# 1812598631/Amos-slam

Hardware: AMD Instinct MI355X
Metric: front-end frames/sec (ORB extract+match+mask) at 640x480 (higher is better)
Workload: dtype u8 (ORB, gate, matcher) + fp32 (mask network); 1 GPU; configs[2]: 640x480 L8 N1000 full front-end: YOLACT-R50 fp32 mask + ORB detect + gate + describe + match; lanes_per_gpu=2, frames_per_launch=64, width=640, height=480, n_features=1000, n_levels=8, ini_th_fast=20, min_th_fast=7, match=frame k vs k-1, N x N best-2, synthetic_stream_seed=stream = rank, frame k seeded 1000*rank+k (amos-slam_amd/synth.py), parallelism=frames sharded 1 ways, one process per GPU, no data-path collective

## Files before the change

### amos-slam_amd/__init__.py

```python
import ctypes as C
import os

import numpy as np

_HERE = os.path.dirname(os.path.abspath(__file__))
LIB_PATH = os.environ.get("AMOS_FRONTEND_LIB", os.path.join(_HERE, "csrc", "libamos_frontend.so"))

KP_DTYPE = np.dtype([("x", "<f4"), ("y", "<f4"), ("size", "<f4"), ("angle", "<f4"),
                     ("response", "<f4"), ("octave", "<i4"), ("class_id", "<i4")])
BEST2_DTYPE = np.dtype([("best_idx", "<i4"), ("best_dist", "<i4"), ("second_idx", "<i4"),
                        ("second_dist", "<i4")])

TH_HIGH, TH_LOW, HISTO_LENGTH = 100, 50, 30

_v, _i, _z, _f, _d, _q, _u = C.c_void_p, C.c_int, C.c_size_t, C.c_float, C.c_double, C.c_longlong, C.c_uint32
PROTOTYPES = {
    "amos_last_error": (C.c_char_p, ()),
    "amos_device_count": (_i, ()),
    "amos_current_device": (_i, ()),
    "amos_build_variant": (C.c_char_p, ()),
    "amos_orb_create": (_i, (_v, _i, _i, _i, _i, _v, _v)),
    "amos_orb_destroy": (None, (_v,)),
    "amos_orb_geometry_probe": (_i, (_v, _i, _i, _i, _i, _v, _v)),
    "amos_orb_tables": (_i, (_v, _v, _v, _v, _v, _v, _v)),
    "amos_orb_tables_host": (_i, (_v, _v, _v, _v, _v, _v, _v)),
    "amos_orb_level_sizes": (_i, (_v, _i, _i, _v, _v)),
    "amos_orb_detect": (_i, (_v, _v, _z, _i, _i)),
    "amos_orb_level_count": (_i, (_v, _i, _i)),
    "amos_orb_level_keypoints": (_i, (_v, _i, _i, _v, _i)),
    "amos_orb_set_level_keypoints": (_i, (_v, _i, _i, _v, _i)),
    "amos_orb_level_layout": (_i, (_v, _v, _v, _v)),
    "amos_orb_fetch_levels": (_i, (_v, _i, _v, _v, _i)),
    "amos_orb_store_levels": (_i, (_v, _i, _v, _v, _i)),
    "amos_orb_gate": (_i, (_v, _v, _z, _v, _z, _v, _i, _v, _i, _v, _i, _v)),
    "amos_orb_closed_mask": (_i, (_v, _v, _z)),
    "amos_orb_describe": (_i, (_v, _v, _v, _i, _v)),
    "amos_orb_extract": (_i, (_v, _v, _z, _i, _i, _v, _v, _i, _v)),
    "amos_orb_level_image": (_i, (_v, _i, _i, _v, _z, _i)),
    "amos_orb_pyramid_images": (_i, (_v, _i, _v, _v, _i)),
    "amos_orb_blurred_image": (_i, (_v, _i, _i, _v, _z)),
    "amos_orb_level_candidates": (_i, (_v, _i, _i, _v, _i)),
    "amos_orb_extract_batch_device": (_i, (_v, _v, _z, _z, _i, _i, _i)),
    "amos_orb_detect_batch_device": (_i, (_v, _v, _z, _z, _i, _i, _i)),
    "amos_orb_gate_batch_device": (_i, (_v, _v, _z, _z)),
    "amos_orb_gate_labels_batch_device": (_i, (_v, _v, _z, _z, _v, _z, _z, _v, _z, _i, _v, _z, _i, _v)),
    "amos_orb_describe_batch_device": (_i, (_v,)),
    "amos_orb_extract_batch_device_color": (_i, (_v, _v, _z, _z, _i, _i, _i, _i, _i)),
    "amos_frame_rgbd_glue_batch_device": (_i, (_v, _v, _i, _f, _z, _z, _f, _f, _f, _f, _f, _v, _v, _v, _v)),
    "amos_frame_stereo_match": (_i, (_v, _v, _f, _f, _v, _v, _i)),
    "amos_frame_stereo_match_batch_device": (_i, (_v, _v, _i, _f, _f, _v, _v, _v, _v)),
    "amos_frame_stereo_match_arrays_device": (_i, (_v, _v, _i, _v, _v, _v, _i, _v, _v, _v, _i, _f, _f, _v, _v, _v, _v)),
    "amos_frame_undistort_batch_device": (_i, (_v, _f, _f, _f, _f, _v, _i, _v)),
    "amos_frame_image_bounds": (_i, (_i, _i, _f, _f, _f, _f, _v, _i, _v)),
    "amos_orb_batch_results_device": (_i, (_v, _v, _v, _v, _v)),
    "amos_orb_batch_fetch": (_i, (_v, _i, _v, _v, _i, _v)),
    "amos_orb_sync": (_i, (_v,)),
    "amos_orb_timing_enable": (_i, (_v, _i)),
    "amos_orb_timing_collect": (_i, (_v, _v, _v)),
    "amos_orb_stream": (_v, (_v,)),
    "amos_match_create": (_i, (_i, _v, _v)),
    "amos_match_destroy": (None, (_v,)),
    "amos_match_sync": (_i, (_v,)),
    "amos_match_stream": (_v, (_v,)),
    "amos_match_distances": (_i, (_v, _v, _i, _v, _i, _v)),
    "amos_match_list_distances": (_i, (_v, _v, _i, _v, _i, _v, _v, _v)),
    "amos_match_list_best2": (_i, (_v, _v, _i, _v, _i, _v, _v, _i, _v)),
    "amos_match_bruteforce_best2": (_i, (_v, _v, _i, _v, _i, _i, _v)),
    "amos_match_set_bruteforce_kernel": (_i, (_v, _i)),
    "amos_match_bruteforce_best2_batch_device": (_i, (_v, _v, _z, _v, _v, _v, _i, _i, _i, _v)),
    "amos_frame_grid_build_batch_device": (_i, (_v, _v, _v, _i, _i, _v, _v)),
    "amos_match_window_best2_batch_device": (_i, (_v, _v, _v)),
    "amos_match_local_points_batch_device": (_i, (_v, _v)),
    "amos_match_local_points": (_i, (_v, _v, _v, _v, _i, _v, _i, _v, _v, _v, _i, _f, _f, _f, _f, _v, _v, _v, _v)),
    "amos_match_motion_model_batch_device": (_i, (_v, _v)),
    "amos_match_motion_model": (_i, (_v, _v, _v, _v, _i, _v, _i, _v, _v, _i, _f, _f, _f, _f, _v, _v, _v, _v)),
    "amos_bow_create": (_i, (_i, _v, _i, _i, _i, _i, _i, _v, _v, _v, _v, _v)),
    "amos_bow_destroy": (None, (_v,)),
    "amos_bow_sync": (_i, (_v,)),
    "amos_bow_stream": (_v, (_v,)),
    "amos_bow_check": (_i, (_i, _i, _i, _i, _i, _v, _v, _v)),
    "amos_bow_transform_batch_device": (_i, (_v, _v, _v, _i, _i, _i, _v, _v, _v, _v, _v, _v, _v, _v, _v, _v)),
    "amos_bow_transform": (_i, (_v, _v, _i, _i, _v, _v, _v, _v, _v, _v, _v, _v)),
    "amos_match_bow_batch_device": (_i, (_v, _v)),
    "amos_match_bow": (_i, (_v, _v, _v, _f, _i, _v, _v)),
    "amos_match_bow_kf_batch_device": (_i, (_v, _v, _f, _i)),
    "amos_match_triangulation_batch_device": (_i, (_v, _v, _v, _v, _v, _i, _i, _i)),
    "amos_match_bow_kf": (_i, (_v, _v, _v, _f, _i, _v, _v)),
    "amos_match_triangulation": (_i, (_v, _v, _v, _i, _v, _v, _v, _i, _i, _i, _v, _v)),
    "amos_mask_pre_create": (_i, (_i, _v, _i, _i, _i, _v)),
    "amos_mask_pre_destroy": (None, (_v,)),
    "amos_mask_pre_stream": (_v, (_v,)),
    "amos_mask_preprocess_batch_device": (_i, (_v, _v, _i, _v)),
    "amos_orb_detect_color_with_mask_pre_batch_device": (_i, (_v, _v, _v, _z, _z, _i, _i, _i, _i, _i, _v)),
    "amos_mask_bias_act_device": (_i, (_v, _v, _v, _v, _z, _i, _i)),
    "amos_mask_bias_relu_maxpool_device": (_i, (_v, _v, _v, _v, _i, _i, _i, _i)),
    "amos_mask_stem_weight_floats": (_i, ()),
    "amos_mask_stem_weights_device": (_i, (_v, _v, _q, _q, _q, _q, _v)),
    "amos_mask_stem_device": (_i, (_v, _v, _q, _q, _q, _q, _v, _v, _v, _i, _i, _i)),
    "amos_mask_conv_supported": (_i, (_i, _i, _i, _i, _i, _i)),
    "amos_mask_conv_device": (_i, (_v, _v, _v, _v, _v, _v, _i, _i, _i, _i, _i, _i, _i, _i, _i, _i)),
    "amos_mask_conv_workspace_bytes": (_z, (_i, _i, _i, _i, _i, _i, _i, _i, _i)),
    "amos_mask_conv_ws_device": (_i, (_v, _v, _v, _v, _v, _v, _i, _i, _i, _i, _i, _i, _i, _i, _i, _i, _v, _z)),
    "amos_mask_conv_tile_mode": (_i, (_i,)),
    "amos_mask_conv_kernel_name": (_i, (_i, _i, _i, _i, _i, _i, _i, _i, _i, _v, _i)),
    "amos_mask_conv_chain_supported": (_i, (_i, _i, _i, _i, _i, _i, _i)),
    "amos_mask_conv_chain_device": (_i, (_v, _v, _v, _v, _v, _v, _v, _v, _i, _i, _i, _i, _i, _i, _i)),
    "amos_mask_conv1x1_supported": (_i, (_i, _i, _i)),
    "amos_mask_winograd_supported": (_i, (_i, _i)),
    "amos_mask_winograd_weight_floats": (_z, (_i, _i)),
    "amos_mask_winograd_weights_device": (_i, (_v, _v, _v, _i, _i)),
    "amos_mask_winograd_conv_device": (_i, (_v, _v, _v, _v, _v, _v, _i, _i, _i, _i, _i, _i)),
    "amos_mask_winograd24_weight_floats": (_z, (_i, _i)),
    "amos_mask_winograd24_weights_device": (_i, (_v, _v, _v, _i, _i)),
    "amos_mask_winograd24_conv_device": (_i, (_v, _v, _v, _v, _v, _v, _i, _i, _i, _i, _i, _i)),
    "amos_mask_winograd24_conv_layout_device": (_i, (_v, _v, _v, _v, _v, _v, _i, _i, _i, _i, _i, _i, _i, _i)),
    "amos_mask_winograd24_persistent_mode": (_i, (_i,)),
    "amos_mask_winograd24_narrow_mode": (_i, (_i,)),
    "amos_mask_conv1x1_device": (_i, (_v, _v, _v, _v, _v, _v, _i, _i, _i, _i, _i, _i, _i)),
    "amos_mask_bilinear_nhwc_device": (_i, (_v, _v, _v, _i, _i, _i, _i, _i, _i, _f, _f)),
    "amos_mask_bilinear_nhwc_act_device": (_i, (_v, _v, _v, _i, _i, _i, _i, _i, _i, _f, _f, _i)),
    "amos_mask_bilinear_x2_mode": (_i, (_i,)),
    "amos_mask_nms_column_max_device": (_i, (_v, _v, _v, _i, _i)),
    "amos_mask_class_scores_device": (_i, (_v, _v, _v, _i, _i, _i, _f)),
    "amos_mask_person_mask_device": (_i, (_v, _v, _v, _v, _i, _i, _i, _i, _i, _i)),
    "amos_mask_head_outputs_device": (_i, (_v, _v, _v, _v, _v, _v, _i, _i, _i, _i, _i, _i, _i, _i)),
    "amos_mask_head_outputs_scores_device": (_i, (_v, _v, _v, _v, _v, _v, _v, _f, _i, _i, _i, _i, _i, _i, _i, _i)),
    "amos_mask_topk_rows_device": (_i, (_v, _v, _v, _v, _i, _i, _i)),
    "amos_mask_topk_rows_sparse_device": (_i, (_v, _v, _v, _v, _i, _i, _i, _f)),
    "amos_mask_post_workspace_bytes": (_z, (_i, _i, _i, _i, _i, _i)),
    "amos_mask_person_masks_device": (_i, (_v, _v, _v, _v, _v, _v, _i, _i, _i, _i, _i, _i, _i, _i, _v, _z, _v, _v)),
    "amos_mask_person_masks_scores_device": (_i, (_v, _v, _v, _v, _v, _v, _i, _i, _i, _i, _i, _i, _i, _i, _v, _z, _v, _v)),
    "amos_mask_coef_at_priors_device": (_i, (_v, _v, _v, _v, _v, _v, _i, _i, _v, _v, _v, _i, _i, _i, _i, _v)),
    "amos_mask_person_masks_at_priors_device": (_i, (_v, _v, _v, _v, _v, _v, _v, _v, _i, _i, _i, _v, _v, _v, _v, _i, _i, _i, _i, _i, _i, _i, _i, _v, _z, _v, _v)),
    "amos_mask_person_masks_scores_at_priors_device": (_i, (_v, _v, _v, _v, _v, _v, _v, _v, _i, _i, _i, _v, _v, _v, _v, _i, _i, _i, _i, _i, _i, _i, _i, _v, _z, _v, _v)),
    "amos_slic_center_count": (_i, (_i, _i, _i, _v, _v)),
    "amos_slic_create": (_i, (_i, _v, _i, _i, _i, _v)),
    "amos_slic_destroy": (None, (_v,)),
    "amos_slic_stream": (_v, (_v,)),
    "amos_slic_run": (_i, (_v, _v, _v, _i, _i, _i, _i, _i, _v, _v, _v)),
    "amos_slic_batch_device": (_i, (_v, _v, _v, _i, _i, _i, _i, _i, _i, _v, _v)),
    "amos_cluster_bgr2lab_batch_device": (_i, (_v, _v, _z, _i, _v)),
    "amos_cluster_kmeans_batch_device": (_i, (_v, _v, _i, _i, _i, _u, _i, _v)),
    "amos_cluster_kmeans": (_i, (_v, _v, _i, _i, _u, _i, _v)),
    "amos_flow_check_device": (_i, (_v, _v, _z, _v, _z, _i, _i, _v, _v, _v, _i, _v)),
    "amos_flow_epipolar_device": (_i, (_v, _v, _v, _v, _v, _i, _v)),
    "amos_flow_scene_flow_device": (_i, (_v, _v, _z, _v, _z, _v, _v, _i, _v, _v)),
    "amos_flow_fundamental_score_device": (_i, (_v, _v, _i, _v, _v, _i, _d, _v, _v, _v)),
    "amos_flow_pnp_score_device": (_i, (_v, _v, _i, _v, _v, _i, _d, _d, _d, _d, _d, _v, _v, _v)),
    "amos_lk_create": (_i, (_i, _v, _i, _i, _i, _i, _v)),
    "amos_lk_destroy": (None, (_v,)),
    "amos_lk_stream": (_v, (_v,)),
    "amos_lk_levels": (_i, (_v,)),
    "amos_lk_track_device": (_i, (_v, _v, _z, _v, _z, _v, _i, _i, _d, _f, _v, _v, _v)),
    "amos_corners_create": (_i, (_i, _v, _i, _i, _v)),
    "amos_corners_destroy": (None, (_v,)),
    "amos_corners_stream": (_v, (_v,)),
    "amos_corners_good_features_device": (_i, (_v, _v, _z, _i, _i, _i, _d, _d, _d, _v, _i, _v, _v)),
    "amos_corners_candidate_count": (_i, (_v, _v)),
    "amos_corners_subpix_device": (_i, (_v, _v, _z, _i, _i, _v, _v, _i, _i, _i, _d)),
    "amos_fmat_create": (_i, (_i, _v, _i, _i, _v)),
    "amos_fmat_destroy": (None, (_v,)),
    "amos_fmat_stream": (_v, (_v,)),
    "amos_fmat_ransac_device": (_i, (_v, _i, _v, _v, _v, _v, _v, _d, _d, _i, _v, _v, _v)),
    "amos_fmat_scene_flow_pair_device": (_i, (_v, _v, _v, _v, _v, _v, _v, _v, _v)),
    "amos_fmat_ransac": (_i, (_v, _i, _v, _v, _d, _d, _i, _v, _v, _v)),
    "amos_pnp_create": (_i, (_i, _v, _i, _i, _v)),
    "amos_pnp_destroy": (None, (_v,)),
    "amos_pnp_stream": (_v, (_v,)),
    "amos_pnp_ransac_device": (_i, (_v, _i, _v, _v, _v, _v, _v, _d, _d, _d, _d, _d, _d, _i, _v, _v, _v)),
    "amos_pnp_scene_flow_device": (_i, (_v, _v, _v, _v, _v, _v, _z, _v, _z, _i, _i, _v, _d, _d, _v, _v, _v)),
    "amos_pnp_ransac": (_i, (_v, _i, _v, _v, _d, _d, _d, _d, _d, _d, _i, _v, _v, _v)),
    "amos_dyna_create": (_i, (_i, _v, _i, _i, _v)),
    "amos_dyna_destroy": (None, (_v,)),
    "amos_dyna_stream": (_v, (_v,)),
    "amos_dyna_results_device": (_i, (_v, _v)),
    "amos_dyna_copy_to_host": (_i, (_v, _v, _v, _z)),
    "amos_dyna_tail_device": (_i, (_v, _i, _v, _v, _v, _v, _v, _v, _v, _v, _v, _z, _v, _z, _i, _i, _v, _d, _d, _v)),
    "amos_dyna_reset_frame_device": (_i, (_v, _i)),
    "amos_dyna_decide_batch_device": (_i, (_v, _i, _v, _z, _z, _i, _i, _v, _z, _i, _i, _v, _z)),
    "amos_dyna_scene_flow_obj_device": (_i, (_v, _i, _v, _v, _v, _v, _v, _z, _v, _z, _i, _i, _v, _z, _v, _z, _v, _d, _d, _v)),
}
EXPORTS = list(PROTOTYPES)


class AmosError(RuntimeError):
    pass


class OrbParams(C.Structure):
    _fields_ = [("n_features", C.c_int32), ("scale_factor", C.c_float), ("n_levels", C.c_int32),
                ("ini_th_fast", C.c_int32), ("min_th_fast", C.c_int32)]


_lib = None


def lib():
    global _lib
    if _lib is None:
        if not os.path.exists(LIB_PATH):
            raise AmosError(f"{LIB_PATH} is missing: build it with `make -C amos-slam_amd/csrc` "
                            "(or __graft_entry__.build()); there is no CPU fallback")
        try:
            import torch
        except ImportError:
            pass
        L = C.CDLL(LIB_PATH)

        def declare(name):
            f = getattr(L, name)
            f.restype, f.argtypes = PROTOTYPES[name]

        declare("amos_build_variant")
        variant = L.amos_build_variant().decode()
        if variant != "default" and os.environ.get("AMOS_ALLOW_EXPERIMENT_BUILD") != "1":
            raise AmosError(f"{LIB_PATH} is an experiment build ({variant}): its results are wrong; unset AMOS_FRONTEND_LIB "
                            "or set AMOS_ALLOW_EXPERIMENT_BUILD=1 for a timing run")
        for name in PROTOTYPES:
            declare(name)
        _lib = L
    return _lib


def _check(rc, what):
    if rc < 0:
        raise AmosError(f"{what} failed (rc={rc}): {lib().amos_last_error().decode()}")
    return rc


def _p(a):
    return a.ctypes.data_as(C.c_void_p) if a is not None else None


def geometry_probe(max_width, max_height, width, height, n_features=1000, scale_factor=1.2, n_levels=8, ini_th=20, min_th=7):
    params = OrbParams(n_features, scale_factor, n_levels, ini_th, min_th)
    need, cap = np.zeros(6, np.int32), np.zeros(6, np.int32)
    rc = lib().amos_orb_geometry_probe(C.byref(params), max_width, max_height, width, height, _p(need), _p(cap))
    return rc, need, cap


def device_count():
    return _check(lib().amos_device_count(), "amos_device_count")


class _Handle:
    _kind = None

    def _open(self, *args):
        self.L = lib()
        h = C.c_void_p()
        _check(getattr(self.L, f"amos_{self._kind}_create")(*args, C.byref(h)), f"amos_{self._kind}_create")
        self.h = h

    def close(self):
        if getattr(self, "h", None):
            getattr(self.L, f"amos_{self._kind}_destroy")(self.h)
            self.h = None

    __del__ = close

    @property
    def stream(self):
        return getattr(self.L, f"amos_{self._kind}_stream")(self.h)


class OrbExtractor(_Handle):

    _kind = "orb"

    def __init__(self, n_features=1000, scale_factor=1.2, n_levels=8, ini_th=20, min_th=7,
                 max_width=640, max_height=480, max_batch=1, device=0, stream=None):
        self.params = OrbParams(n_features, scale_factor, n_levels, ini_th, min_th)
        self.n_levels, self.n_features = n_levels, n_features
        self.max_batch = max_batch
        self._open(C.byref(self.params), max_width, max_height, max_batch, device, stream)
        self.shape = None
        cap = C.c_int(0)
        self.L.amos_orb_batch_results_device(self.h, None, None, None, C.byref(cap))
        self.capacity = cap.value

    def tables(self):
        n = self.n_levels
        sc, isc, s2, is2 = (np.zeros(n, np.float32) for _ in range(4))
        fpl, umax = np.zeros(n, np.int32), np.zeros(16, np.int32)
        _check(self.L.amos_orb_tables(self.h, _p(sc), _p(isc), _p(s2), _p(is2), _p(fpl), _p(umax)), "amos_orb_tables")
        return dict(scale=sc, inv_scale=isc, sigma2=s2, inv_sigma2=is2, features_per_level=fpl, umax=umax)

# ... 278 lines not shown
    return int(lib().amos_mask_bilinear_x2_mode(mode))


def mask_conv1x1_supported(cin, cout, stride):
    return lib().amos_mask_conv1x1_supported(cin, cout, stride) == 0


def mask_conv1x1(stream_ptr, x_ptr, w_ptr, bias_ptr, residual_ptr, y_ptr, batch, in_h, in_w, cin, cout, stride, relu):
    _check(lib().amos_mask_conv1x1_device(stream_ptr, x_ptr, w_ptr, bias_ptr, residual_ptr, y_ptr, batch, in_h, in_w, cin, cout, stride, int(relu)),
           "amos_mask_conv1x1_device")


def mask_conv_supported(cin, cout, kh, kw, stride, pad):
    return lib().amos_mask_conv_supported(cin, cout, kh, kw, stride, pad) == 0


def mask_winograd_supported(cin, cout):
    return lib().amos_mask_winograd_supported(cin, cout) == 0


def mask_winograd_weights(stream_ptr, w_ptr, u_ptr, cin, cout):
    _check(lib().amos_mask_winograd_weights_device(stream_ptr, w_ptr, u_ptr, cin, cout), "amos_mask_winograd_weights_device")


def mask_winograd_conv(stream_ptr, x_ptr, u_ptr, bias_ptr, residual_ptr, y_ptr, batch, h, w, cin, cout, relu):
    _check(lib().amos_mask_winograd_conv_device(stream_ptr, x_ptr, u_ptr, bias_ptr, residual_ptr, y_ptr, batch, h, w, cin, cout, int(relu)),
           "amos_mask_winograd_conv_device")


def mask_winograd24_weights(stream_ptr, w_ptr, u_ptr, cin, cout):
    _check(lib().amos_mask_winograd24_weights_device(stream_ptr, w_ptr, u_ptr, cin, cout), "amos_mask_winograd24_weights_device")


def mask_winograd24_conv(stream_ptr, x_ptr, u_ptr, bias_ptr, residual_ptr, y_ptr, batch, h, w, cin, cout, relu):
    _check(lib().amos_mask_winograd24_conv_device(stream_ptr, x_ptr, u_ptr, bias_ptr, residual_ptr, y_ptr, batch, h, w, cin, cout, int(relu)),
           "amos_mask_winograd24_conv_device")


def mask_winograd24_conv_layout(stream_ptr, x_ptr, u_ptr, bias_ptr, residual_ptr, y_ptr, batch, h, w, cin, cout, relu, in_blocked, out_blocked):
    _check(lib().amos_mask_winograd24_conv_layout_device(stream_ptr, x_ptr, u_ptr, bias_ptr, residual_ptr, y_ptr, batch, h, w, cin, cout, int(relu), int(in_blocked),
                                                         int(out_blocked)), "amos_mask_winograd24_conv_layout_device")


def mask_winograd24_persistent_mode(mode=-2):
    return int(lib().amos_mask_winograd24_persistent_mode(mode))


def mask_winograd24_narrow_mode(mode=-2):
    return int(lib().amos_mask_winograd24_narrow_mode(mode))


def mask_conv_tile_mode(mode=-2):
    return int(lib().amos_mask_conv_tile_mode(mode))


def mask_conv_kernel_name(batch, in_h, in_w, cin, cout, kh, kw, stride, pad):
    buf = C.create_string_buffer(96)
    _check(lib().amos_mask_conv_kernel_name(batch, in_h, in_w, cin, cout, kh, kw, stride, pad, buf, 96), "amos_mask_conv_kernel_name")
    return buf.value.decode()


def mask_conv(stream_ptr, x_ptr, w_ptr, bias_ptr, residual_ptr, y_ptr, batch, in_h, in_w, cin, cout, kh, kw, stride, pad, relu):
    _check(lib().amos_mask_conv_device(stream_ptr, x_ptr, w_ptr, bias_ptr, residual_ptr, y_ptr, batch, in_h, in_w, cin, cout, kh, kw, stride, pad, int(relu)),
           "amos_mask_conv_device")


def mask_conv_chain_supported(batch, in_h, in_w, cin, planes, cout, stride):
    return lib().amos_mask_conv_chain_supported(batch, in_h, in_w, cin, planes, cout, stride) == 0


def mask_conv_chain(stream_ptr, x_ptr, wd_ptr, bd_ptr, yc_ptr, w3_ptr, b3_ptr, y_ptr, batch, in_h, in_w, cin, planes, cout, stride):
    _check(lib().amos_mask_conv_chain_device(stream_ptr, x_ptr, wd_ptr, bd_ptr, yc_ptr, w3_ptr, b3_ptr, y_ptr, batch, in_h, in_w, cin, planes, cout, stride),
           "amos_mask_conv_chain_device")


def mask_conv_workspace_bytes(batch, in_h, in_w, cin, cout, kh, kw, stride, pad):
    return int(lib().amos_mask_conv_workspace_bytes(batch, in_h, in_w, cin, cout, kh, kw, stride, pad))


def mask_conv_ws(stream_ptr, x_ptr, w_ptr, bias_ptr, residual_ptr, y_ptr, batch, in_h, in_w, cin, cout, kh, kw, stride, pad, relu, workspace_ptr, workspace_bytes):
    _check(lib().amos_mask_conv_ws_device(stream_ptr, x_ptr, w_ptr, bias_ptr, residual_ptr, y_ptr, batch, in_h, in_w, cin, cout, kh, kw, stride, pad, int(relu),
                                          workspace_ptr, workspace_bytes), "amos_mask_conv_ws_device")


def mask_bilinear_nhwc(stream_ptr, x_ptr, y_ptr, n, in_h, in_w, out_h, out_w, channels, scale_h, scale_w, relu=False):
    _check(lib().amos_mask_bilinear_nhwc_act_device(stream_ptr, x_ptr, y_ptr, n, in_h, in_w, out_h, out_w, channels, scale_h, scale_w, int(relu)),
           "amos_mask_bilinear_nhwc_act_device")


def mask_class_scores(stream_ptr, conf_ptr, scores_ptr, batch, n_priors, n_classes_with_background, threshold):
    _check(lib().amos_mask_class_scores_device(stream_ptr, conf_ptr, scores_ptr, batch, n_priors, n_classes_with_background, threshold),
           "amos_mask_class_scores_device")


def mask_person_mask(stream_ptr, masks_ptr, flags_ptr, out_ptr, batch, n_det, mask_h, mask_w, out_h, out_w):
    _check(lib().amos_mask_person_mask_device(stream_ptr, masks_ptr, flags_ptr, out_ptr, batch, n_det, mask_h, mask_w, out_h, out_w), "amos_mask_person_mask_device")


def mask_head_outputs(stream_ptr, raw_ptr, bias_ptr, loc_ptr, conf_ptr, coef_ptr, batch, cells, channels_padded, anchors, n_classes_with_background, mask_dim,
                      n_priors_total, prior_offset):
    _check(lib().amos_mask_head_outputs_device(stream_ptr, raw_ptr, bias_ptr, loc_ptr, conf_ptr, coef_ptr, batch, cells, channels_padded, anchors,
                                               n_classes_with_background, mask_dim, n_priors_total, prior_offset), "amos_mask_head_outputs_device")


def mask_head_outputs_scores(stream_ptr, raw_ptr, bias_ptr, loc_ptr, conf_ptr, coef_ptr, scores_ptr, threshold, batch, cells, channels_padded, anchors,
                             n_classes_with_background, mask_dim, n_priors_total, prior_offset):
    _check(lib().amos_mask_head_outputs_scores_device(stream_ptr, raw_ptr, bias_ptr, loc_ptr, conf_ptr, coef_ptr, scores_ptr, threshold, batch, cells,
                                                      channels_padded, anchors, n_classes_with_background, mask_dim, n_priors_total, prior_offset),
           "amos_mask_head_outputs_scores_device")


def mask_person_masks_scores(stream_ptr, loc_ptr, scores_ptr, coef_ptr, priors_ptr, proto_ptr, batch, n_priors, n_classes_with_background, mask_dim, proto_h, proto_w,
                             out_h, out_w, workspace_ptr, workspace_bytes, masks_ptr, found_ptr):
    _check(lib().amos_mask_person_masks_scores_device(stream_ptr, loc_ptr, scores_ptr, coef_ptr, priors_ptr, proto_ptr, batch, n_priors, n_classes_with_background,
                                                      mask_dim, proto_h, proto_w, out_h, out_w, workspace_ptr, workspace_bytes, masks_ptr, found_ptr),
           "amos_mask_person_masks_scores_device")


def mask_topk_rows(stream_ptr, x_ptr, values_ptr, indices_ptr, rows, n, k):
    _check(lib().amos_mask_topk_rows_device(stream_ptr, x_ptr, values_ptr, indices_ptr, rows, n, k), "amos_mask_topk_rows_device")


def mask_topk_rows_sparse(stream_ptr, x_ptr, values_ptr, indices_ptr, rows, n, k, fill):
    _check(lib().amos_mask_topk_rows_sparse_device(stream_ptr, x_ptr, values_ptr, indices_ptr, rows, n, k, fill), "amos_mask_topk_rows_sparse_device")


def mask_post_workspace_bytes(batch, n_priors, n_classes_with_background, mask_dim, proto_h, proto_w):
    return int(lib().amos_mask_post_workspace_bytes(batch, n_priors, n_classes_with_background, mask_dim, proto_h, proto_w))


def mask_person_masks(stream_ptr, loc_ptr, conf_ptr, coef_ptr, priors_ptr, proto_ptr, batch, n_priors, n_classes_with_background, mask_dim, proto_h, proto_w,
                      out_h, out_w, workspace_ptr, workspace_bytes, masks_ptr, found_ptr):
    _check(lib().amos_mask_person_masks_device(stream_ptr, loc_ptr, conf_ptr, coef_ptr, priors_ptr, proto_ptr, batch, n_priors, n_classes_with_background, mask_dim,
                                               proto_h, proto_w, out_h, out_w, workspace_ptr, workspace_bytes, masks_ptr, found_ptr),
           "amos_mask_person_masks_device")


def _coef_levels(level_ptrs, level_hw, level_blocked, anchors):
    n = len(level_ptrs)
    offs, off = [], 0
    for h, w in level_hw:
        offs.append(off)
        off += h * w * anchors
    ints = C.c_int * n
    return ((C.c_void_p * n)(*level_ptrs), ints(*[h for h, _ in level_hw]), ints(*[w for _, w in level_hw]), ints(*[int(bool(f)) for f in level_blocked]),
            ints(*offs), n)


def mask_coef_at_priors(stream_ptr, level_ptrs, level_hw, level_blocked, cin, weight_ptr, bias_ptr, prior_idx_ptr, batch, n_slots, anchors, mask_dim, out_ptr):
    _check(lib().amos_mask_coef_at_priors_device(stream_ptr, *_coef_levels(level_ptrs, level_hw, level_blocked, anchors), cin, weight_ptr, bias_ptr, prior_idx_ptr,
                                                 batch, n_slots, anchors, mask_dim, out_ptr), "amos_mask_coef_at_priors_device")


def mask_person_masks_at_priors(stream_ptr, loc_ptr, scores_ptr, scores_are_class_scores, level_ptrs, level_hw, level_blocked, cin, anchors, mask_weight_ptr,
                                mask_bias_ptr, priors_ptr, proto_ptr, batch, n_priors, n_classes_with_background, mask_dim, proto_h, proto_w, out_h, out_w,
                                workspace_ptr, workspace_bytes, masks_ptr, found_ptr):
    name = "amos_mask_person_masks_scores_at_priors_device" if scores_are_class_scores else "amos_mask_person_masks_at_priors_device"
    _check(getattr(lib(), name)(stream_ptr, loc_ptr, scores_ptr, *_coef_levels(level_ptrs, level_hw, level_blocked, anchors), cin, anchors, mask_weight_ptr,
                                mask_bias_ptr, priors_ptr, proto_ptr, batch, n_priors, n_classes_with_background, mask_dim, proto_h, proto_w, out_h, out_w,
                                workspace_ptr, workspace_bytes, masks_ptr, found_ptr), name)


def mask_nms_column_max(stream_ptr, boxes_ptr, out_ptr, n_lists, k):
    _check(lib().amos_mask_nms_column_max_device(stream_ptr, boxes_ptr, out_ptr, n_lists, k), "amos_mask_nms_column_max_device")


class LkTracker(_Handle):

    _kind = "lk"

    def __init__(self, width=640, height=480, win_size=22, max_level=5, device=0, stream=None):
        self._open(device, stream, width, height, win_size, max_level)
        self.levels = self.L.amos_lk_levels(self.h)

    def track_device(self, d_prev, prev_stride, d_next, next_stride, d_prev_xy, n, d_next_xy, d_status, d_err=None, max_count=20, epsilon=0.01,
                     min_eig=1e-4):
        _check(self.L.amos_lk_track_device(self.h, d_prev, prev_stride, d_next, next_stride, d_prev_xy, n, max_count, epsilon, min_eig, d_next_xy, d_status,
                                           d_err), "amos_lk_track_device")


def image_bounds(width, height, fx, fy, cx, cy, dist_coef):
    dc = np.ascontiguousarray(dist_coef, np.float32)
    out = np.zeros(4, np.float32)
    _check(lib().amos_frame_image_bounds(width, height, fx, fy, cx, cy, _p(dc), len(dc), _p(out)), "amos_frame_image_bounds")
    return tuple(float(v) for v in out)


class WindowSearch(C.Structure):
    _fields_ = [("d_kps", C.c_void_p), ("d_desc", C.c_void_p), ("d_counts", C.c_void_p), ("d_cell_start", C.c_void_p),
                ("d_items", C.c_void_p), ("d_query_uv", C.c_void_p), ("d_query_invz", C.c_void_p), ("d_u_right", C.c_void_p),
                ("d_pairs_q", C.c_void_p), ("d_pairs_t", C.c_void_p), ("scale_factors", C.c_void_p), ("n_pairs", C.c_int32),
                ("capacity", C.c_int32), ("n_levels", C.c_int32), ("mode", C.c_int32), ("init_dist", C.c_int32), ("th", C.c_float),
                ("mbf", C.c_float), ("min_x", C.c_float), ("max_x", C.c_float), ("min_y", C.c_float), ("max_y", C.c_float)]


class MapPoint(C.Structure):
    _fields_ = [("pos", C.c_float * 3), ("normal", C.c_float * 3), ("min_distance", C.c_float), ("max_distance", C.c_float),
                ("flags", C.c_int32), ("desc", C.c_uint8 * 32), ("pad", C.c_uint8 * 12)]


class LocalCamera(C.Structure):
    _fields_ = [("Rcw", C.c_float * 9), ("tcw", C.c_float * 3), ("Ow", C.c_float * 3), ("fx", C.c_float), ("fy", C.c_float),
                ("cx", C.c_float), ("cy", C.c_float), ("mbf", C.c_float), ("view_cos_limit", C.c_float), ("th", C.c_float),
                ("nn_ratio", C.c_float)]


class LocalStats(C.Structure):
    _fields_ = [("n_in_view", C.c_int32), ("n_matches", C.c_int32), ("n_researched", C.c_int32), ("status", C.c_int32)]


MAP_POINT_SKIP, MAP_POINT_HAS_OBS = 1, 2
MAP_POINT_DTYPE = np.dtype([("pos", "<f4", (3,)), ("normal", "<f4", (3,)), ("min_distance", "<f4"), ("max_distance", "<f4"),
                            ("flags", "<i4"), ("desc", "u1", (32,)), ("pad", "u1", (12,))])
LOCAL_CAMERA_DTYPE = np.dtype([("Rcw", "<f4", (9,)), ("tcw", "<f4", (3,)), ("Ow", "<f4", (3,)), ("fx", "<f4"), ("fy", "<f4"), ("cx", "<f4"),
                               ("cy", "<f4"), ("mbf", "<f4"), ("view_cos_limit", "<f4"), ("th", "<f4"), ("nn_ratio", "<f4")])
LOCAL_STATS_DTYPE = np.dtype([("n_in_view", "<i4"), ("n_matches", "<i4"), ("n_researched", "<i4"), ("status", "<i4")])
MAP_QUERY_DTYPE = np.dtype([("proj_x", "<f4"), ("proj_y", "<f4"), ("proj_xr", "<f4"), ("view_cos", "<f4"), ("level", "<i4"),
                            ("has_obs", "<i4"), ("desc", "u1", (32,))])
assert (C.sizeof(MapPoint), C.sizeof(LocalCamera), C.sizeof(LocalStats)) == (MAP_POINT_DTYPE.itemsize, LOCAL_CAMERA_DTYPE.itemsize,
                                                                            LOCAL_STATS_DTYPE.itemsize) == (80, 92, 16)


class LocalSearch(C.Structure):
    _fields_ = [("d_kps", C.c_void_p), ("d_desc", C.c_void_p), ("d_counts", C.c_void_p), ("d_cell_start", C.c_void_p), ("d_items", C.c_void_p),
                ("d_u_right", C.c_void_p), ("d_points", C.c_void_p), ("point_off", C.c_void_p), ("cameras", C.c_void_p),
                ("d_occupied", C.c_void_p), ("scale_factors", C.c_void_p), ("d_query", C.c_void_p), ("d_in_view", C.c_void_p),
                ("d_match", C.c_void_p), ("d_stats", C.c_void_p), ("n_frames", C.c_int32), ("capacity", C.c_int32), ("n_levels", C.c_int32),
                ("min_x", C.c_float), ("max_x", C.c_float), ("min_y", C.c_float), ("max_y", C.c_float)]


class LastPoint(C.Structure):
    _fields_ = [("pos", C.c_float * 3), ("angle", C.c_float), ("octave", C.c_int32), ("flags", C.c_int32), ("desc", C.c_uint8 * 32),
                ("pad", C.c_uint8 * 8)]


class MotionCamera(C.Structure):
    _fields_ = [("Rcw", C.c_float * 9), ("tcw", C.c_float * 3), ("Rlw", C.c_float * 9), ("tlw", C.c_float * 3), ("fx", C.c_float),
                ("fy", C.c_float), ("cx", C.c_float), ("cy", C.c_float), ("mbf", C.c_float), ("mb", C.c_float), ("th", C.c_float),
                ("th_retry", C.c_float), ("retry_below", C.c_int32), ("mono", C.c_int32), ("check_orientation", C.c_int32)]


class MotionStats(C.Structure):
    _fields_ = [("n_projected", C.c_int32), ("n_matches", C.c_int32), ("n_first", C.c_int32), ("pass_", C.c_int32),
                ("n_researched", C.c_int32), ("flags", C.c_int32), ("status", C.c_int32), ("pad", C.c_int32)]


LAST_POINT_SKIP, LAST_POINT_HAS_OBS = 1, 2
MOTION_FORWARD, MOTION_BACKWARD = 1, 2
LAST_POINT_DTYPE = np.dtype([("pos", "<f4", (3,)), ("angle", "<f4"), ("octave", "<i4"), ("flags", "<i4"), ("desc", "u1", (32,)),
                             ("pad", "u1", (8,))])
MOTION_CAMERA_DTYPE = np.dtype([("Rcw", "<f4", (9,)), ("tcw", "<f4", (3,)), ("Rlw", "<f4", (9,)), ("tlw", "<f4", (3,)), ("fx", "<f4"),
                                ("fy", "<f4"), ("cx", "<f4"), ("cy", "<f4"), ("mbf", "<f4"), ("mb", "<f4"), ("th", "<f4"),
                                ("th_retry", "<f4"), ("retry_below", "<i4"), ("mono", "<i4"), ("check_orientation", "<i4")])
MOTION_STATS_DTYPE = np.dtype([("n_projected", "<i4"), ("n_matches", "<i4"), ("n_first", "<i4"), ("pass", "<i4"), ("n_researched", "<i4"),
                               ("flags", "<i4"), ("status", "<i4"), ("pad", "<i4")])
PROJ_QUERY_DTYPE = np.dtype([("u", "<f4"), ("v", "<f4"), ("invz", "<f4"), ("octave", "<i4"), ("angle", "<f4"), ("has_obs", "<i4"),
                             ("desc", "u1", (32,))])
assert (C.sizeof(LastPoint), C.sizeof(MotionCamera), C.sizeof(MotionStats)) == (LAST_POINT_DTYPE.itemsize, MOTION_CAMERA_DTYPE.itemsize,
                                                                                MOTION_STATS_DTYPE.itemsize) == (64, 140, 32)


class MotionSearch(C.Structure):
    _fields_ = [("d_kps", C.c_void_p), ("d_desc", C.c_void_p), ("d_counts", C.c_void_p), ("d_cell_start", C.c_void_p), ("d_items", C.c_void_p),
                ("d_u_right", C.c_void_p), ("d_points", C.c_void_p), ("point_off", C.c_void_p), ("cameras", C.c_void_p),
                ("scale_factors", C.c_void_p), ("d_query", C.c_void_p), ("d_projected", C.c_void_p), ("d_match", C.c_void_p),
                ("d_stats", C.c_void_p), ("n_frames", C.c_int32), ("capacity", C.c_int32), ("n_levels", C.c_int32), ("min_x", C.c_float),
                ("max_x", C.c_float), ("min_y", C.c_float), ("max_y", C.c_float)]


BOW_L1_NORM, BOW_TF_IDF = 0, 0
BOW_MAX_CHILDREN, BOW_MAX_CAPACITY, BOW_NO_WORD, BOW_STATUS_EARLY_LEAF = 32, 16384, 0xFFFFFFFF, 1
BOW_STATS_DTYPE = np.dtype([("n_words", "<i4"), ("n_nodes", "<i4"), ("n_stopped", "<i4"), ("status", "<i4")])
BOW_SEARCH_STATS_DTYPE = np.dtype([("n_queries", "<i4"), ("n_matches", "<i4"), ("n_researched", "<i4"), ("status", "<i4")])
assert BOW_STATS_DTYPE.itemsize == BOW_SEARCH_STATS_DTYPE.itemsize == 16


class BowSearch(C.Structure):
    _fields_ = [("d_kps", C.c_void_p), ("d_desc", C.c_void_p), ("d_counts", C.c_void_p), ("d_n_nodes", C.c_void_p), ("d_node_ids", C.c_void_p),
                ("d_node_off", C.c_void_p), ("d_node_idx", C.c_void_p), ("d_has_point", C.c_void_p), ("d_pairs_kf", C.c_void_p),
                ("d_pairs_f", C.c_void_p), ("d_match", C.c_void_p), ("d_stats", C.c_void_p), ("n_pairs", C.c_int32), ("capacity", C.c_int32),
                ("nn_ratio", C.c_float), ("check_orientation", C.c_int32)]


class KfPairSearch(C.Structure):
    _fields_ = [("d_kps", C.c_void_p), ("d_desc", C.c_void_p), ("d_counts", C.c_void_p), ("d_n_nodes", C.c_void_p), ("d_node_ids", C.c_void_p),
                ("d_node_off", C.c_void_p), ("d_node_idx", C.c_void_p), ("d_has_point", C.c_void_p), ("d_u_right", C.c_void_p),
                ("d_pairs_1", C.c_void_p), ("d_pairs_2", C.c_void_p), ("d_match12", C.c_void_p), ("d_stats", C.c_void_p), ("n_pairs", C.c_int32),
                ("capacity", C.c_int32)]


KF_GEOMETRY_DTYPE = np.dtype([("f12", "<f4", (9,)), ("ex", "<f4"), ("ey", "<f4")])
assert KF_GEOMETRY_DTYPE.itemsize == 44
KF_STATUS_BAD_INDEX, KF_STATUS_BAD_OCTAVE = 1, 2


class BowView(C.Structure):
    _fields_ = [("n", C.c_int32), ("keys", C.c_void_p), ("descriptors", C.c_void_p), ("has_point", C.c_void_p), ("u_right", C.c_void_p),
                ("n_nodes", C.c_int32), ("node_ids", C.c_void_p), ("node_off", C.c_void_p), ("node_idx", C.c_void_p)]


def bow_vocabulary_arrays(parent, is_leaf, desc, weight):
    parent = np.ascontiguousarray(parent, np.int32)
    is_leaf = np.ascontiguousarray(is_leaf, np.uint8)
    desc = np.ascontiguousarray(desc, np.uint8).reshape(-1, 32)
    weight = np.ascontiguousarray(weight, np.float64)
    if not (len(parent) == len(is_leaf) == len(desc) == len(weight)):
        raise ValueError("parent, is_leaf, desc and weight hold one entry per node")
    return parent, is_leaf, desc, weight


# ... 372 lines not shown
```

### amos-slam_amd/csrc/amos_mask_post.hip

```cpp
#include <hip/hip_runtime.h>
#include <stdint.h>

#include "../../include/amos_frontend.h"
#include "amos_common.h"

namespace amos {

constexpr int kScoreTile = 64;
__global__ __launch_bounds__(256) void k_class_scores(const float *__restrict__ conf, float *__restrict__ scores, int P, int C1, float thresh)
{
    extern __shared__ float tile[];
    __shared__ float best[kScoreTile];
    const int b = blockIdx.y, p0 = blockIdx.x * kScoreTile, np = min(kScoreTile, P - p0), pitch = C1 + 1;
    const float *src = conf + ((size_t)b * P + p0) * C1;
    for (int e = threadIdx.x; e < np * C1; e += 256) {
        const int r = e / C1, c = e - r * C1;
        tile[r * pitch + c] = src[e];
    }
    __syncthreads();
    if (threadIdx.x < np) {
        const float *row = tile + threadIdx.x * pitch;
        float m = row[1];
        bool nan = m != m;
        for (int c = 2; c < C1; c++) {
            const float v = row[c];
            nan = nan || v != v;
            m = v > m ? v : m;
        }
        best[threadIdx.x] = nan ? __builtin_nanf("") : m;
    }
    __syncthreads();
    const int C = C1 - 1;
    for (int e = threadIdx.x; e < C * kScoreTile; e += 256) {
        const int c = e / kScoreTile, r = e - c * kScoreTile;
        if (r < np) scores[((size_t)b * C + c) * P + p0 + r] = best[r] > thresh ? tile[r * pitch + c + 1] : -1.f;
    }
}

constexpr int kPmCols = 20, kPmRows = 6, kPmDet = 16, kPmTileH = 16;
__global__ __launch_bounds__(256) void k_person_mask(const float *__restrict__ masks, const uint8_t *__restrict__ flags, uint8_t *__restrict__ out, int n,
                                                    int ph, int pw, int H, int W, float scaleH, float scaleW)
{
    __shared__ float win[kPmDet][kPmRows][kPmCols];
    __shared__ int sList[kPmDet], sCount;
    const int ox = blockIdx.x * 64 + threadIdx.x, b = blockIdx.z, t = threadIdx.y * 64 + threadIdx.x;
    auto src = [](float scale, int o) {
        const float f = __fsub_rn(__fmul_rn(scale, __fadd_rn((float)o, 0.5f)), 0.5f);
        return f < 0.f ? 0.f : f;
    };
    const int ox0 = blockIdx.x * 64, ox1 = min(ox0 + 63, W - 1), oy0 = blockIdx.y * kPmTileH, oy1 = min(oy0 + kPmTileH - 1, H - 1);
    const int wx0 = (int)src(scaleW, ox0), wx1 = min((int)src(scaleW, ox1) + 1, pw - 1), wy0 = (int)src(scaleH, oy0), wy1 = min((int)src(scaleH, oy1) + 1, ph - 1);
    const int wc = wx1 - wx0 + 1, wr = wy1 - wy0 + 1;
    const bool staged = wc <= kPmCols && wr <= kPmRows && n <= kPmDet;
    if (staged) {
        if (t < 64) {
            const bool f = t < n && flags[b * n + t] != 0;
            const unsigned long long m = __ballot(f);
            if (f) sList[__popcll(m & ((1ull << t) - 1ull))] = t;
            if (t == 0) sCount = (int)__popcll(m);
        }
        __syncthreads();
        const int cnt = sCount, per = wr * wc;
        for (int e = t; e < cnt * per; e += 256) {
            const int d = e / per, rem = e - d * per, r = rem / wc, c = rem - r * wc;
            win[d][r][c] = masks[((size_t)b * n + sList[d]) * ph * pw + (size_t)(wy0 + r) * pw + wx0 + c];
        }
        __syncthreads();
    }
    if (ox >= W) return;
    const float fx = src(scaleW, ox);
    const int x0 = (int)fx, x1 = x0 + (x0 < pw - 1 ? 1 : 0);
    const float lx = __fsub_rn(fx, (float)x0), hx = __fsub_rn(1.f, lx);
    for (int ry = threadIdx.y; ry < kPmTileH; ry += 4) {
        const int oy = oy0 + ry;
        if (oy >= H) break;
        const float fy = src(scaleH, oy);
        const int y0 = (int)fy, y1 = y0 + (y0 < ph - 1 ? 1 : 0);
        const float ly = __fsub_rn(fy, (float)y0), hy = __fsub_rn(1.f, ly);
        unsigned count = 0;
        if (staged) {
            const int cnt = sCount, ry0 = y0 - wy0, ry1 = y1 - wy0, cx0 = x0 - wx0, cx1 = x1 - wx0;
            for (int d = 0; d < cnt; d++) {
                const float p = win[d][ry0][cx0], r = win[d][ry0][cx1], s2 = win[d][ry1][cx0], u = win[d][ry1][cx1];
                const float v = __fadd_rn(__fmul_rn(hy, __fadd_rn(__fmul_rn(hx, p), __fmul_rn(lx, r))), __fmul_rn(ly, __fadd_rn(__fmul_rn(hx, s2), __fmul_rn(lx, u))));
                count += v > 0.5f ? 1u : 0u;
            }
        } else {
            for (int i = 0; i < n; i++) {
                if (!flags[b * n + i]) continue;
                const float *m = masks + ((size_t)b * n + i) * ph * pw;
                const float p = m[y0 * pw + x0], r = m[y0 * pw + x1], s2 = m[y1 * pw + x0], u = m[y1 * pw + x1];
                const float v = __fadd_rn(__fmul_rn(hy, __fadd_rn(__fmul_rn(hx, p), __fmul_rn(lx, r))), __fmul_rn(ly, __fadd_rn(__fmul_rn(hx, s2), __fmul_rn(lx, u))));
                count += v > 0.5f ? 1u : 0u;
            }
        }
        out[((size_t)b * H + oy) * W + ox] = (uint8_t)((count * 255u) & 0xffu);
    }
}

constexpr int kHeadCells = 16;
__global__ __launch_bounds__(256) void k_head_outputs(const float *__restrict__ raw, const float *__restrict__ bias, float *__restrict__ loc, float *__restrict__ conf,
                                                     float *__restrict__ coef, int cells, int cpad, int A, int C1, int D, int P, int pOff,
                                                     float *__restrict__ scores, float thresh)
{
    extern __shared__ float sh[];
    const int b = blockIdx.y, c0 = blockIdx.x * kHeadCells, nc = min(kHeadCells, cells - c0);
    const int nLoc = A * 4, nConf = A * C1, nCoef = coef ? A * D : 0;
    const float *src = raw + ((size_t)b * cells + c0) * cpad;
    for (int e = threadIdx.x * 4; e < nc * cpad; e += 256 * 4) {
        float4 v = *reinterpret_cast<const float4 *>(src + e);
        const float4 bb = *reinterpret_cast<const float4 *>(bias + e % cpad);
        v.x = __fadd_rn(v.x, bb.x); v.y = __fadd_rn(v.y, bb.y); v.z = __fadd_rn(v.z, bb.z); v.w = __fadd_rn(v.w, bb.w);
        *reinterpret_cast<float4 *>(sh + e) = v;
    }
    __syncthreads();
    __shared__ float sMax[256], sSum[256];
#define AMOS_HEAD_FOREACH(n, body)                                                             \
    {                                                                                          \
        const int stepCell = 256 / (n), stepR = 256 % (n);                                     \
        int cell = (int)threadIdx.x / (n), r = (int)threadIdx.x - cell * (n);                  \
        for (int e = threadIdx.x; e < nc * (n); e += 256) {                                    \
            body;                                                                              \
            cell += stepCell;                                                                  \
            r += stepR;                                                                        \
            if (r >= (n)) { r -= (n); cell++; }                                                \
        }                                                                                      \
    }
    if ((int)threadIdx.x < nc * A) {
        const int cell = threadIdx.x / A, a = threadIdx.x - cell * A;
        const float *v = sh + cell * cpad + nLoc + a * C1;
        float m = v[0];
        for (int c = 1; c < C1; c++) m = fmaxf(m, v[c]);
        sMax[threadIdx.x] = m;
    }
    __syncthreads();
    const float invC1 = 1.f / (float)C1;
    AMOS_HEAD_FOREACH(nConf, {
        float *v = sh + cell * cpad + nLoc + r;
        int a = (int)((float)r * invC1);
        a -= a * C1 > r ? 1 : 0;
        a += (a + 1) * C1 <= r ? 1 : 0;
        *v = expf(__fsub_rn(*v, sMax[cell * A + a]));
    })
    if (nCoef) AMOS_HEAD_FOREACH(nCoef, {
        float *v = sh + cell * cpad + nLoc + nConf + r;
        *v = tanhf(*v);
    })
    __syncthreads();
    if ((int)threadIdx.x < nc * A) {
        const int cell = threadIdx.x / A, a = threadIdx.x - cell * A;
        const float *v = sh + cell * cpad + nLoc + a * C1;
        float sum = 0.f;
        for (int c = 0; c < C1; c++) sum = __fadd_rn(sum, v[c]);
        sSum[threadIdx.x] = sum;
    }
    __syncthreads();
    const size_t prior0 = (size_t)b * P + pOff + (size_t)c0 * A;
    AMOS_HEAD_FOREACH(nLoc, loc[prior0 * 4 + e] = sh[cell * cpad + r])
    if (nCoef) AMOS_HEAD_FOREACH(nCoef, coef[prior0 * D + e] = sh[cell * cpad + nLoc + nConf + r])
    if (!scores) {
        AMOS_HEAD_FOREACH(nConf, {
            int a = (int)((float)r * invC1);
            a -= a * C1 > r ? 1 : 0;
            a += (a + 1) * C1 <= r ? 1 : 0;
            conf[prior0 * C1 + e] = sh[cell * cpad + nLoc + r] / sSum[cell * A + a];
        })
        return;
    }
    AMOS_HEAD_FOREACH(nConf, {
        int a = (int)((float)r * invC1);
        a -= a * C1 > r ? 1 : 0;
        a += (a + 1) * C1 <= r ? 1 : 0;
        float *v = sh + cell * cpad + nLoc + r;
        *v = *v / sSum[cell * A + a];
    })
    __syncthreads();
    if ((int)threadIdx.x < nc * A) {
        const int cell = threadIdx.x / A, a = threadIdx.x - cell * A;
        const float *v = sh + cell * cpad + nLoc + a * C1;
        float m = v[1];
        bool nan = m != m;
        for (int c = 2; c < C1; c++) {
            const float q = v[c];
            nan = nan || q != q;
            m = q > m ? q : m;
        }
        sMax[threadIdx.x] = nan ? __builtin_nanf("") : m;
    }
    __syncthreads();
    if (conf) AMOS_HEAD_FOREACH(nConf, conf[prior0 * C1 + e] = sh[cell * cpad + nLoc + r])
    {
        const int C = C1 - 1, np = nc * A;
        float *dst = scores + (size_t)b * C * P + pOff + (size_t)c0 * A;
        int c = (int)threadIdx.x / np, pl = (int)threadIdx.x - c * np;
        const int stepC = 256 / np, stepP = 256 % np;
        for (int e = threadIdx.x; e < C * np; e += 256) {
            const int cell = pl / A, a = pl - cell * A;
            dst[(size_t)c * P + pl] = sMax[pl] > thresh ? sh[cell * cpad + nLoc + a * C1 + c + 1] : -1.f;
            c += stepC;
            pl += stepP;
            if (pl >= np) { pl -= np; c++; }
        }
    }
#undef AMOS_HEAD_FOREACH
}


constexpr int kTopkBins = 2048;
__device__ __forceinline__ unsigned topk_key(float f)
{
    const unsigned u = __float_as_uint(f);
    return (u & 0x80000000u) ? ~u : (u | 0x80000000u);
}
__device__ __forceinline__ float topk_value(unsigned key) { return __uint_as_float((key & 0x80000000u) ? (key & 0x7fffffffu) : ~key); }

constexpr int kTopkList = 1024;
__global__ __launch_bounds__(256) void k_topk_rows(const float *__restrict__ x, float *__restrict__ values, long long *__restrict__ indices, int n, int k, float fill)
{
    __shared__ unsigned hist[kTopkBins];
    __shared__ unsigned part[256];
    __shared__ unsigned long long sel[256];
    __shared__ unsigned sPrefix, sMask, sNeed, sCountAbove, sWaveEq[4];
    __shared__ unsigned long long list[kTopkList];
    __shared__ unsigned sLive, sBelow;
    const int t = threadIdx.x, lane = t & 63, wave = t >> 6;
    const float *row = x + (size_t)blockIdx.x * n;
    if (fill == fill) {
        const unsigned fk = topk_key(fill);
        if (t == 0) { sLive = 0; sBelow = 0; }
        __syncthreads();
        const bool vec = (n & 3) == 0 && ((uintptr_t)row & 15) == 0;
        const int nVec = vec ? n : 0;
#define AMOS_TOPK_TAKE(have, v, i)                                                                                        \
        {                                                                                                                 \
            const unsigned key = topk_key(v);                                                                             \
            const bool up = (have) && key > fk;                                                                           \
            const unsigned long long m = __ballot(up);                                                                    \
            if (m) {                                                                                                      \
                unsigned base = 0;                                                                                        \
                if (lane == (int)__builtin_ctzll(m)) base = atomicAdd(&sLive, (unsigned)__popcll(m));                     \
                base = __shfl(base, (int)__builtin_ctzll(m), 64);                                                         \
                const unsigned slot = base + (unsigned)__popcll(m & ((1ull << lane) - 1ull));                             \
                if (up && slot < (unsigned)kTopkList) list[slot] = ((unsigned long long)key << 32) | (unsigned)(0xffffffffu - (unsigned)(i)); \
            }                                                                                                             \
            if ((have) && key < fk) sBelow = 1u;                                                                          \
        }
        for (int i0 = 0; i0 < nVec; i0 += 1024) {
            if (*reinterpret_cast<volatile unsigned *>(&sLive) > (unsigned)kTopkList) break;
            const int i = i0 + 4 * t;
            const bool have = i < n;
            const float4 v = have ? *reinterpret_cast<const float4 *>(row + i) : make_float4(0.f, 0.f, 0.f, 0.f);
            AMOS_TOPK_TAKE(have, v.x, i)
            AMOS_TOPK_TAKE(have, v.y, i + 1)
            AMOS_TOPK_TAKE(have, v.z, i + 2)
            AMOS_TOPK_TAKE(have, v.w, i + 3)
        }
        for (int i0 = nVec; i0 < n; i0 += 256) {
            const int i = i0 + t;
            const bool have = i < n;
            const float v = have ? row[i] : 0.f;
            AMOS_TOPK_TAKE(have, v, i)
        }
#undef AMOS_TOPK_TAKE
        __syncthreads();
        const unsigned live = sLive;
        if (live <= (unsigned)kTopkList && (live >= (unsigned)k || !sBelow)) {
            unsigned n2 = 256;
            while (n2 < live) n2 <<= 1;
            for (unsigned i = live + t; i < n2; i += 256) list[i] = 0ull;
            __syncthreads();
            for (unsigned size = 2; size <= n2; size <<= 1)
                for (unsigned stride = size >> 1; stride > 0; stride >>= 1) {
                    for (unsigned i = t; i < n2 / 2; i += 256) {
                        const unsigned lo = ((i / stride) * stride * 2) + (i % stride), hi = lo + stride;
                        const unsigned long long a = list[lo], b = list[hi];
                        const bool descending = (lo & size) == 0;
                        if (descending ? a < b : a > b) { list[lo] = b; list[hi] = a; }
                    }
                    __syncthreads();
                }
            const unsigned take = live < (unsigned)k ? live : (unsigned)k;
            if ((unsigned)t < take) {
                const unsigned long long v = list[t];
                values[(size_t)blockIdx.x * k + t] = topk_value((unsigned)(v >> 32));
                indices[(size_t)blockIdx.x * k + t] = (long long)(0xffffffffu - (unsigned)(v & 0xffffffffu));
            }
            unsigned have = take;
            for (int i0 = 0; i0 < n && have < (unsigned)k; i0 += 256) {
                const int i = i0 + t;
                const bool eq = i < n && topk_key(row[i]) == fk;
                const unsigned long long m = __ballot(eq);
                if (lane == 0) sWaveEq[wave] = (unsigned)__popcll(m);
                __syncthreads();
                unsigned base = have, total = 0;
                for (int w = 0; w < 4; w++) {
                    const unsigned c = sWaveEq[w];
                    if (w < wave) base += c;
                    total += c;
                }
                const unsigned rank = base + (unsigned)__popcll(m & ((1ull << lane) - 1ull));
                if (eq && rank < (unsigned)k) {
                    values[(size_t)blockIdx.x * k + rank] = fill;
                    indices[(size_t)blockIdx.x * k + rank] = (long long)i;
                }
                have += total;
                __syncthreads();
            }
            return;
        }
        __syncthreads();
// ... 188 lines not shown
        __syncthreads();
        for (unsigned size = 2; size <= n2; size <<= 1)
            for (unsigned stride = size >> 1; stride > 0; stride >>= 1) {
                for (unsigned i = t; i < n2 / 2; i += kTopkLdsThreads) {
                    const unsigned lo = ((i / stride) * stride * 2) + (i % stride), hi = lo + stride;
                    const unsigned long long a = list[lo], b = list[hi];
                    const bool descending = (lo & size) == 0;
                    if (descending ? a < b : a > b) { list[lo] = b; list[hi] = a; }
                }
                __syncthreads();
            }
        const unsigned take = live < (unsigned)k ? live : (unsigned)k;
        if ((unsigned)t < take) {
            const unsigned long long v = list[t];
            values[(size_t)blockIdx.x * k + t] = topk_value((unsigned)(v >> 32));
            indices[(size_t)blockIdx.x * k + t] = (long long)(0xffffffffu - (unsigned)(v & 0xffffffffu));
        }
        unsigned have = take;
        for (int i0 = 0; i0 < n && have < (unsigned)k; i0 += kTopkLdsThreads) {
            const int i = i0 + t;
            const bool eq = i < n && keys[i] == fk;
            const unsigned long long m = __ballot(eq);
            if (lane == 0) sWave[wave] = (unsigned)__popcll(m);
            __syncthreads();
            unsigned base = have, total = 0;
            for (int w = 0; w < kTopkLdsThreads / 64; w++) {
                const unsigned c = sWave[w];
                if (w < wave) base += c;
                total += c;
            }
            const unsigned rank = base + (unsigned)__popcll(m & ((1ull << lane) - 1ull));
            if (eq && rank < (unsigned)k) {
                values[(size_t)blockIdx.x * k + rank] = fill;
                indices[(size_t)blockIdx.x * k + rank] = (long long)i;
            }
            have += total;
            __syncthreads();
        }
        return;
    }
    const int shifts[3] = {21, 10, 0}, widths[3] = {11, 11, 10};
    for (int pass = 0; pass < 3; pass++) {
        const int shift = shifts[pass], bins = 1 << widths[pass];
        for (int b = t; b < kTopkBins; b += kTopkLdsThreads) hist[b] = 0;
        __syncthreads();
        const unsigned prefix = sPrefix, mask = sMask, need = sNeed;
#define AMOS_TOPK_COUNT(in, bin)                                                                                          \
        {     \
            const unsigned long long m = __ballot(in);                                                                    \
            if (m) {                                                                                                      \
                const unsigned b0 = __builtin_amdgcn_readlane((bin), (int)__builtin_ctzll(m));  \
                const bool same = __ballot((in) && (bin) != b0) == 0ull;                                                  \
                if (same) {                                                                                               \
                    if (lane == (int)__builtin_ctzll(m)) atomicAdd(&hist[b0], (unsigned)__popcll(m));                     \
                } else if (in) {                                                                                          \
                    atomicAdd(&hist[(bin)], 1u);                                                                          \
                }                                                                                                         \
            }                                                                                                             \
        }
        for (int i0 = 0; i0 < n; i0 += 4 * kTopkLdsThreads) {
            const int i = i0 + 4 * t;
            const uint4 kk = i < n ? *reinterpret_cast<const uint4 *>(&keys[i]) : make_uint4(0u, 0u, 0u, 0u);
            const bool in0 = i < n && (kk.x & mask) == prefix, in1 = i + 1 < n && (kk.y & mask) == prefix;
            const bool in2 = i + 2 < n && (kk.z & mask) == prefix, in3 = i + 3 < n && (kk.w & mask) == prefix;
            const unsigned b0_ = (kk.x >> shift) & (bins - 1), b1_ = (kk.y >> shift) & (bins - 1), b2_ = (kk.z >> shift) & (bins - 1), b3_ = (kk.w >> shift) & (bins - 1);
            AMOS_TOPK_COUNT(in0, b0_)
            AMOS_TOPK_COUNT(in1, b1_)
            AMOS_TOPK_COUNT(in2, b2_)
            AMOS_TOPK_COUNT(in3, b3_)
        }
#undef AMOS_TOPK_COUNT
        __syncthreads();
        {
            unsigned p = 0;
            for (int b = 0; b < kTopkBins / kTopkLdsThreads; b++) p += hist[(kTopkBins / kTopkLdsThreads) * t + b];
            part[t] = p;
        }
        __syncthreads();
        if (t < 64) {
            unsigned q = 0;
            for (int j = 0; j < kTopkLdsThreads / 64; j++) q += part[(kTopkLdsThreads / 64) * lane + j];
            unsigned suffix = q;
            for (int d = 1; d < 64; d <<= 1) {
                const unsigned o = __shfl_down(suffix, d, 64);
                if (lane + d < 64) suffix += o;
            }
            const unsigned above = suffix - q;
            if (above < need && suffix >= need) {
                unsigned acc = above;
                int bin = 32 * lane + 31;
                for (; bin > 32 * lane; bin--) {
                    const unsigned c = hist[bin];
                    if (acc + c >= need) break;
                    acc += c;
                }
                sPrefix = prefix | ((unsigned)bin << shift);
                sMask = mask | ((unsigned)(bins - 1) << shift);
                sNeed = need - acc;
            }
        }
        __syncthreads();
    }
    const unsigned T = sPrefix, needEq = sNeed, nAbove = (unsigned)k - needEq;
    for (int i0 = 0; i0 < n; i0 += 4 * kTopkLdsThreads) {
        const int i = i0 + 4 * t;
        if (i < n) {
            const uint4 kk = *reinterpret_cast<const uint4 *>(&keys[i]);
            const unsigned key[4] = {kk.x, kk.y, kk.z, kk.w};
#pragma unroll
            for (int e = 0; e < 4; e++)
                if (i + e < n && key[e] > T) sel[atomicAdd(&sCountAbove, 1u)] = ((unsigned long long)key[e] << 32) | (unsigned)(0xffffffffu - (unsigned)(i + e));
        }
    }
    {
        const int chunk = (n + kTopkLdsThreads - 1) / kTopkLdsThreads, lo = min(t * chunk, n), hi = min(lo + chunk, n);
        unsigned cnt = 0;
        for (int i = lo; i < hi; i++) cnt += keys[i] == T ? 1u : 0u;
        unsigned incl = cnt;
        for (int d = 1; d < 64; d <<= 1) {
            const unsigned o = __shfl_up(incl, d, 64);
            if (lane >= d) incl += o;
        }
        if (lane == 63) sWave[wave] = incl;
        __syncthreads();
        unsigned rank = incl - cnt;
        for (int w = 0; w < wave; w++) rank += sWave[w];
        for (int i = lo; i < hi && rank < needEq; i++)
            if (keys[i] == T) {
                sel[nAbove + rank] = ((unsigned long long)T << 32) | (unsigned)(0xffffffffu - (unsigned)i);
                rank++;
            }
    }
    if (t >= k && t < 256) sel[t] = 0ull;
    __syncthreads();
    for (int size = 2; size <= 256; size <<= 1)
        for (int stride = size >> 1; stride > 0; stride >>= 1) {
            unsigned long long a = 0, b = 0;
            if (t < 256) { a = sel[t]; b = sel[t ^ stride]; }
            __syncthreads();
            if (t < 256) {
                const bool descending = (t & size) == 0, lower = (t & stride) == 0;
                const unsigned long long hi = a > b ? a : b, lo = a > b ? b : a;
                sel[t] = (descending == lower) ? hi : lo;
            }
            __syncthreads();
        }
    if (t < k) {
        const unsigned long long v = sel[t];
        values[(size_t)blockIdx.x * k + t] = topk_value((unsigned)(v >> 32));
        indices[(size_t)blockIdx.x * k + t] = (long long)(0xffffffffu - (unsigned)(v & 0xffffffffu));
    }
}



__global__ __launch_bounds__(256) void k_decode_boxes(const float4 *__restrict__ loc, const float4 *__restrict__ priors, float4 *__restrict__ boxes, int P, int total)
{
    const int e = blockIdx.x * 256 + threadIdx.x;
    if (e >= total) return;
    const float4 l = loc[e], p = priors[e % P];
    const float cx = __fadd_rn(p.x, __fmul_rn(__fmul_rn(l.x, 0.1f), p.z)), cy = __fadd_rn(p.y, __fmul_rn(__fmul_rn(l.y, 0.1f), p.w));
    const float sw = __fmul_rn(p.z, expf(__fmul_rn(l.z, 0.2f))), sh = __fmul_rn(p.w, expf(__fmul_rn(l.w, 0.2f)));
    const float x1 = __fsub_rn(cx, __fmul_rn(sw, 0.5f)), y1 = __fsub_rn(cy, __fmul_rn(sh, 0.5f));
    boxes[e] = make_float4(x1, y1, __fadd_rn(x1, sw), __fadd_rn(y1, sh));
}

__global__ __launch_bounds__(256) void k_nms_alive(const float4 *__restrict__ boxes, const long long *__restrict__ idx, const float *__restrict__ scores,
                                                  float *__restrict__ out, int k, int P, int C, float thresh)
{
    __shared__ float4 sb[256];
    __shared__ float sarea[256];
    const int j = threadIdx.x, list = blockIdx.x, b = list / C;
    float4 me = {0.f, 0.f, 0.f, 0.f};
    float myArea = 0.f;
    if (j < k) {
        me = boxes[(size_t)b * P + (size_t)idx[(size_t)list * k + j]];
        myArea = __fmul_rn(__fsub_rn(me.z, me.x), __fsub_rn(me.w, me.y));
        sb[j] = me;
        sarea[j] = myArea;
    }
    __syncthreads();
    if (j >= k) return;
    float best = 0.f;
    bool nan = false;
    for (int i = 0; i < j; i++) {
        const float4 o = sb[i];
        float w = __fsub_rn(fminf(o.z, me.z), fmaxf(o.x, me.x)), h = __fsub_rn(fminf(o.w, me.w), fmaxf(o.y, me.y));
        w = w < 0.f ? 0.f : w;
        h = h < 0.f ? 0.f : h;
        const float inter = __fmul_rn(w, h);
        const float uni = __fsub_rn(__fadd_rn(sarea[i], myArea), inter);
        const float iou = (float)((double)inter / (double)uni);
        nan = nan || iou != iou;
        best = iou > best ? iou : best;
    }
    const float sc = scores[(size_t)list * k + j];
    out[(size_t)list * k + j] = (!nan && best <= thresh && sc > 0.f) ? sc : -1.f;
}

__global__ __launch_bounds__(256) void k_select_display(const float *__restrict__ alive, const long long *__restrict__ idx, const float4 *__restrict__ boxes,
                                                       const float *__restrict__ coef, float *__restrict__ selCoef, float4 *__restrict__ selRect,
                                                       uint8_t *__restrict__ flags, uint8_t *__restrict__ found, int n, int k, int P, int D, int nDisplay,
                                                       float scoreThresh, int personClass, int pw, int ph, int *__restrict__ selPrior)
{
    constexpr int kSelectList = 4096;
    __shared__ unsigned long long list[kSelectList];
    __shared__ unsigned long long sWave[4], sSel[32];
    __shared__ unsigned sCount;
    const int t = threadIdx.x, lane = t & 63, wave = t >> 6, b = blockIdx.x;
    const float *row = alive + (size_t)b * n;
    if (t == 0) sCount = 0;
    __syncthreads();
    for (int i = t; i < n; i += 256) {
        const float v = row[i];
        if (v > scoreThresh) {
            const unsigned slot = atomicAdd(&sCount, 1u);
            if (slot < (unsigned)kSelectList) list[slot] = ((unsigned long long)topk_key(v) << 32) | (unsigned)(0xffffffffu - (unsigned)i);
        }
    }
    __syncthreads();
    const unsigned count = sCount;
    const bool listed = count <= (unsigned)kSelectList;
    unsigned long long prev = ~0ull;
    for (int r = 0; r < nDisplay; r++) {
        unsigned long long best = 0ull;
        if (listed) {
            for (unsigned i = t; i < count; i += 256) {
                const unsigned long long key = list[i];
                best = (key < prev && key > best) ? key : best;
            }
        } else {
            for (int i = t; i < n; i += 256) {
                const float v = row[i];
                const unsigned long long key = v > scoreThresh ? (((unsigned long long)topk_key(v) << 32) | (unsigned)(0xffffffffu - (unsigned)i)) : 0ull;
                best = (key < prev && key > best) ? key : best;
            }
        }
        for (int d = 32; d > 0; d >>= 1) {
            const unsigned long long o = __shfl_xor(best, d, 64);
            best = o > best ? o : best;
        }
        if (lane == 0) sWave[wave] = best;
        __syncthreads();
        unsigned long long m = sWave[0];
        for (int w = 1; w < 4; w++) m = sWave[w] > m ? sWave[w] : m;
        if (t == 0) sSel[r] = m;
        prev = m ? m : 1ull;
        __syncthreads();
    }
    if (t < nDisplay) {
        const unsigned long long key = sSel[t];
        const float score = topk_value((unsigned)(key >> 32));
        const int flat = (int)(0xffffffffu - (unsigned)(key & 0xffffffffu));
        const bool valid = key != 0ull && score > scoreThresh;
        const int cls = valid ? flat / k : 0;
        const long long prior = valid ? idx[(size_t)b * n + flat] : 0;
        const float4 bx = boxes[(size_t)b * P + (size_t)prior];
        const float ax = __fmul_rn(bx.x, (float)pw), bxx = __fmul_rn(bx.z, (float)pw), ay = __fmul_rn(bx.y, (float)ph), by = __fmul_rn(bx.w, (float)ph);
        float4 rc;
        rc.x = fmaxf(__fsub_rn(fminf(ax, bxx), 1.f), 0.f);
        rc.y = fminf(__fadd_rn(fmaxf(ax, bxx), 1.f), (float)pw);
        rc.z = fmaxf(__fsub_rn(fminf(ay, by), 1.f), 0.f);
        rc.w = fminf(__fadd_rn(fmaxf(ay, by), 1.f), (float)ph);
        selRect[(size_t)b * nDisplay + t] = rc;
        flags[(size_t)b * nDisplay + t] = (valid && cls == personClass) ? 1 : 0;
        if (t == 0) found[b] = valid ? 1 : 0;
        if (selPrior) selPrior[(size_t)b * nDisplay + t] = valid ? (int)prior : -1;
        sSel[t] = (unsigned long long)prior;
    }
    if (selPrior) return;
    __syncthreads();
    for (int e = t; e < nDisplay * D; e += 256) {
        const int r = e / D, c = e - r * D;
        selCoef[((size_t)b * nDisplay + r) * D + c] = coef[((size_t)b * P + (size_t)sSel[r]) * D + c];
    }
}

__global__ __launch_bounds__(256) void k_assemble_masks(const float *__restrict__ proto, const float *__restrict__ selCoef, const float4 *__restrict__ selRect,
                                                       const uint8_t *__restrict__ flags, float *__restrict__ masks, int ph, int pw, int D, int nDisplay)
{
    const int n = blockIdx.y, b = blockIdx.z, pix = blockIdx.x * 256 + threadIdx.x;
    if (!flags[(size_t)b * nDisplay + n] || pix >= ph * pw) return;
    const int y = pix / pw, x = pix - y * pw;
    const float4 rc = selRect[(size_t)b * nDisplay + n];
    float v = 0.f;
    if ((float)x >= rc.x && (float)x < rc.y && (float)y >= rc.z && (float)y < rc.w) {
        const float4 *pp = reinterpret_cast<const float4 *>(proto + ((size_t)b * ph * pw + pix) * D);
        const float4 *cc = reinterpret_cast<const float4 *>(selCoef + ((size_t)b * nDisplay + n) * D);
        float acc = 0.f;
        for (int q = 0; q < D / 4; q++) {
            const float4 a = pp[q], c = cc[q];
            acc = __fmaf_rn(a.x, c.x, acc); acc = __fmaf_rn(a.y, c.y, acc); acc = __fmaf_rn(a.z, c.z, acc); acc = __fmaf_rn(a.w, c.w, acc);
        }
        v = 1.f / (1.f + expf(-acc));
    }
    masks[((size_t)b * nDisplay + n) * ph * pw + pix] = v;
}

constexpr int kCoefLevels = 8, kCoefParts = 8;
struct CoefLevels {
    const float *x[kCoefLevels];
    int h[kCoefLevels], w[kCoefLevels], blocked[kCoefLevels], off[kCoefLevels];
    int n;
};
__global__ __launch_bounds__(256) void k_coef_at_priors(CoefLevels lv, int cin, const float *__restrict__ weight, const float *__restrict__ bias,
                                                       const int *__restrict__ idx, int n, int A, int D, float *__restrict__ out)
{
    extern __shared__ __align__(16) float patch[];
    const int slot = blockIdx.x, b = blockIdx.y, t = threadIdx.x;
    const int p = idx[(size_t)b * n + slot];
    float *dst = out + ((size_t)b * n + slot) * D;
    int l = -1;
    for (int i = 0; i < lv.n; i++) l = p >= lv.off[i] ? i : l;
    const int rel = l >= 0 ? p - lv.off[l] : 0, cell = rel / A, a = rel - cell * A;
    if (p < 0 || l < 0 || cell >= lv.h[l] * lv.w[l]) {
        if (t < D) dst[t] = 0.f;
        return;
    }
    const int h = lv.h[l], w = lv.w[l], cy = cell / w, cx = cell - cy * w;
    const float *x = lv.x[l];
    const bool blocked = lv.blocked[l] != 0;
    for (int e = t; e < 9 * cin; e += blockDim.x) {
        const int tap = e / cin, c = e - tap * cin, y = cy + tap / 3 - 1, xx = cx + tap % 3 - 1;
        float v = 0.f;
        if (y >= 0 && y < h && xx >= 0 && xx < w)
            v = blocked ? x[((((size_t)b * (cin / 8) + c / 8) * h + y) * w + xx) * 8 + (c & 7)] : x[(((size_t)b * h + y) * w + xx) * cin + c];
        patch[e] = v;
    }
    __syncthreads();
    const int d = t / kCoefParts, s = t - d * kCoefParts;
    const float4 *wv = reinterpret_cast<const float4 *>(weight + (size_t)(a * D + d) * 9 * cin);
    const float4 *pv = reinterpret_cast<const float4 *>(patch);
    float acc = 0.f;
    for (int q = s; q < 9 * cin / 4; q += kCoefParts) {
        const float4 u = wv[q], v = pv[q];
        acc = __fmaf_rn(u.x, v.x, acc); acc = __fmaf_rn(u.y, v.y, acc); acc = __fmaf_rn(u.z, v.z, acc); acc = __fmaf_rn(u.w, v.w, acc);
    }
    for (int m = 1; m < kCoefParts; m <<= 1) acc = __fadd_rn(acc, __shfl_xor(acc, m, 64));
    if (s == 0) dst[d] = tanhf(__fadd_rn(acc, bias[a * D + d]));
}

}

using namespace amos;

extern "C" {

int amos_mask_class_scores_device(void *stream, const float *d_conf, float *d_scores, int batch, int n_priors, int n_classes_with_background, float threshold)
{
    if (!d_conf || !d_scores || batch < 0 || n_priors < 1 || n_classes_with_background < 2 || n_classes_with_background > 200 || batch > 65535) {
        set_error("amos_mask_class_scores_device: invalid argument (2 <= classes incl. background <= 200)");
        return AMOS_ERR_INVALID;
    }
    if (batch == 0) return AMOS_OK;
    const size_t lds = (size_t)kScoreTile * (n_classes_with_background + 1) * sizeof(float);
    hipLaunchKernelGGL(k_class_scores, dim3((n_priors + kScoreTile - 1) / kScoreTile, batch), dim3(256), lds, (hipStream_t)stream, d_conf, d_scores, n_priors,
                       n_classes_with_background, threshold);
    AMOS_HIP_CHECK(hipGetLastError());
    return AMOS_OK;
}

int amos_mask_person_mask_device(void *stream, const float *d_masks, const uint8_t *d_flags, uint8_t *d_out, int batch, int n_det, int mask_h, int mask_w,
                                 int out_h, int out_w)
{
    if (!d_masks || !d_flags || !d_out || batch < 0 || n_det < 0 || mask_h < 1 || mask_w < 1 || out_h < 1 || out_w < 1 || batch > 65535 || out_h > 16 * 65535) {
        set_error("amos_mask_person_mask_device: invalid argument");
        return AMOS_ERR_INVALID;
    }
    if (batch == 0) return AMOS_OK;
    const float sh = (float)mask_h / (float)out_h, sw = (float)mask_w / (float)out_w;
    hipLaunchKernelGGL(k_person_mask, dim3((out_w + 63) / 64, (out_h + kPmTileH - 1) / kPmTileH, batch), dim3(64, 4), 0, (hipStream_t)stream, d_masks, d_flags, d_out, n_det, mask_h,
                       mask_w, out_h, out_w, sh, sw);
    AMOS_HIP_CHECK(hipGetLastError());
    return AMOS_OK;
}

int amos_mask_head_outputs_device(void *stream, const float *d_raw, const float *d_bias, float *d_loc, float *d_conf, float *d_coef, int batch, int cells,
                                  int channels_padded, int anchors, int n_classes_with_background, int mask_dim, int n_priors_total, int prior_offset)
{
    if (!d_conf) { set_error("amos_mask_head_outputs_device: invalid argument"); return AMOS_ERR_INVALID; }
    return amos_mask_head_outputs_scores_device(stream, d_raw, d_bias, d_loc, d_conf, d_coef, nullptr, 0.f, batch, cells, channels_padded, anchors,
                                                n_classes_with_background, mask_dim, n_priors_total, prior_offset);
}

int amos_mask_head_outputs_scores_device(void *stream, const float *d_raw, const float *d_bias, float *d_loc, float *d_conf, float *d_coef, float *d_scores,
                                         float threshold, int batch, int cells, int channels_padded, int anchors, int n_classes_with_background, int mask_dim,
                                         int n_priors_total, int prior_offset)
{
    const long long used = (long long)anchors * (4 + n_classes_with_background + (d_coef ? mask_dim : 0));
    if (!d_raw || !d_bias || !d_loc || (!d_conf && !d_scores) || (d_scores && n_classes_with_background < 2) || batch < 0 || cells < 1 || anchors < 1 || n_classes_with_background < 1 || mask_dim < 1 ||
        channels_padded % 4 != 0 || used > channels_padded || channels_padded > 1000 || prior_offset < 0 ||
       
        (long long)prior_offset + (long long)cells * anchors > n_priors_total || batch > 65535 || kHeadCells * anchors > 256 ||
        ((uintptr_t)d_raw | (uintptr_t)d_bias) % 16 != 0) {
        set_error("amos_mask_head_outputs_scores_device: invalid argument");
        return AMOS_ERR_INVALID;
    }
    if (batch == 0) return AMOS_OK;
    hipLaunchKernelGGL(k_head_outputs, dim3((cells + kHeadCells - 1) / kHeadCells, batch), dim3(256), (size_t)kHeadCells * channels_padded * sizeof(float),
                       (hipStream_t)stream, d_raw, d_bias, d_loc, d_conf, d_coef, cells, channels_padded, anchors, n_classes_with_background, mask_dim,
                       n_priors_total, prior_offset, d_scores, threshold);
    AMOS_HIP_CHECK(hipGetLastError());
    return AMOS_OK;
}

static DeviceOnce g_topk_lds_once;
static int launch_topk(hipStream_t stream, const float *d_x, float *d_values, long long *d_indices, int rows, int n, int k, float fill)
{
    static const bool ldsAllowed = [] { const char *e = getenv("AMOS_TOPK_LDS"); return !(e && e[0] == '0'); }();
    if (ldsAllowed && n <= kTopkLdsMax && rows <= 256) {
        const int ldsBytes = ((n + 3) & ~3) * (int)sizeof(unsigned);
        AMOS_HIP_CHECK(set_max_dynamic_lds(g_topk_lds_once, reinterpret_cast<const void *>(k_topk_rows_lds), kTopkLdsMax * (int)sizeof(unsigned), stream));
        hipLaunchKernelGGL(k_topk_rows_lds, dim3(rows), dim3(kTopkLdsThreads), ldsBytes, stream, d_x, d_values, d_indices, n, k, fill);
    } else {
        hipLaunchKernelGGL(k_topk_rows, dim3(rows), dim3(256), 0, stream, d_x, d_values, d_indices, n, k, fill);
    }
    AMOS_HIP_CHECK(hipGetLastError());
    return AMOS_OK;
}

int amos_mask_topk_rows_device(void *stream, const float *d_x, float *d_values, long long *d_indices, int rows, int n, int k)
{
    if (!d_x || !d_values || !d_indices || rows < 0 || n < 1 || k < 1 || k > 256 || k > n) {
        set_error("amos_mask_topk_rows_device: invalid argument (1 <= k <= min(256, n))");
        return AMOS_ERR_INVALID;
    }
    if (rows == 0) return AMOS_OK;
    return launch_topk((hipStream_t)stream, d_x, d_values, d_indices, rows, n, k, __builtin_nanf(""));
}

int amos_mask_topk_rows_sparse_device(void *stream, const float *d_x, float *d_values, long long *d_indices, int rows, int n, int k, float fill)
{
    if (!d_x || !d_values || !d_indices || rows < 0 || n < 1 || k < 1 || k > 256 || k > n) {
        set_error("amos_mask_topk_rows_sparse_device: invalid argument (1 <= k <= min(256, n))");
        return AMOS_ERR_INVALID;
    }
    if (rows == 0) return AMOS_OK;
    return launch_topk((hipStream_t)stream, d_x, d_values, d_indices, rows, n, k, fill);
}


namespace {
struct PostLayout {
    size_t boxes, cls, topv, topi, alive, selCoef, selRect, flags, masks, selPrior, total;
};
inline size_t post_align(size_t v) { return (v + 255) & ~(size_t)255; }
PostLayout post_layout(int B, int P, int C1, int D, int ph, int pw)
{
    const size_t C = (size_t)C1 - 1, k = AMOS_MASK_NMS_TOP_K, nd = AMOS_MASK_TOP_K_DISPLAY;
    PostLayout l;
    size_t o = 0;
    l.boxes = o; o += post_align((size_t)B * P * 16);
    l.cls = o; o += post_align((size_t)B * C * P * 4);
    l.topv = o; o += post_align((size_t)B * C * k * 4);
    l.topi = o; o += post_align((size_t)B * C * k * 8);
    l.alive = o; o += post_align((size_t)B * C * k * 4);
    l.selCoef = o; o += post_align((size_t)B * nd * D * 4);
    l.selRect = o; o += post_align((size_t)B * nd * 16);
    l.flags = o; o += post_align((size_t)B * nd);
    l.masks = o; o += post_align((size_t)B * nd * ph * pw * 4);
    l.selPrior = o; o += post_align((size_t)B * nd * 4);
    l.total = o;
    return l;
}
}

size_t amos_mask_post_workspace_bytes(int batch, int n_priors, int n_classes_with_background, int mask_dim, int proto_h, int proto_w)
{
    if (batch < 1 || n_priors < AMOS_MASK_NMS_TOP_K || n_classes_with_background < 2 || mask_dim < 4 || proto_h < 1 || proto_w < 1) return 0;
    return post_layout(batch, n_priors, n_classes_with_background, mask_dim, proto_h, proto_w).total;
}

struct LazyCoef {
    CoefLevels lv;
    int cin, anchors;
    const float *weight, *bias;
};
static int fill_coef_levels(const char *who, CoefLevels &lv, const float *const *d_levels, const int *level_h, const int *level_w, const int *level_blocked,
                            const int *level_offsets, int n_levels, int batch, int cin, int anchors, int mask_dim, const float *d_weight, const float *d_bias);
static int launch_coef_at_priors(hipStream_t st, const CoefLevels &lv, int cin, const float *d_weight, const float *d_bias, const int *d_idx, int batch, int n,
                                 int anchors, int mask_dim, float *d_out);
static int person_masks(void *stream, const float *d_loc, const float *d_conf, const float *d_scores, const float *d_coef, const LazyCoef *lazy, const float *d_priors,
                        const float *d_proto, int batch, int n_priors, int n_classes_with_background, int mask_dim, int proto_h, int proto_w, int out_h, int out_w,
                        void *d_workspace, size_t workspace_bytes, uint8_t *d_masks, uint8_t *d_found);

int amos_mask_person_masks_device(void *stream, const float *d_loc, const float *d_conf, const float *d_coef, const float *d_priors, const float *d_proto,
                                  int batch, int n_priors, int n_classes_with_background, int mask_dim, int proto_h, int proto_w, int out_h, int out_w,
                                  void *d_workspace, size_t workspace_bytes, uint8_t *d_masks, uint8_t *d_found)
{
    if (!d_conf) { set_error("amos_mask_person_masks_device: invalid argument"); return AMOS_ERR_INVALID; }
    return person_masks(stream, d_loc, d_conf, nullptr, d_coef, nullptr, d_priors, d_proto, batch, n_priors, n_classes_with_background, mask_dim, proto_h, proto_w, out_h, out_w,
                        d_workspace, workspace_bytes, d_masks, d_found);
}

int amos_mask_person_masks_scores_device(void *stream, const float *d_loc, const float *d_scores, const float *d_coef, const float *d_priors, const float *d_proto,
                                         int batch, int n_priors, int n_classes_with_background, int mask_dim, int proto_h, int proto_w, int out_h, int out_w,
                                         void *d_workspace, size_t workspace_bytes, uint8_t *d_masks, uint8_t *d_found)
{
    if (!d_scores) { set_error("amos_mask_person_masks_scores_device: invalid argument"); return AMOS_ERR_INVALID; }
    return person_masks(stream, d_loc, nullptr, d_scores, d_coef, nullptr, d_priors, d_proto, batch, n_priors, n_classes_with_background, mask_dim, proto_h, proto_w, out_h, out_w,
                        d_workspace, workspace_bytes, d_masks, d_found);
}

static int fill_coef_levels(const char *who, CoefLevels &lv, const float *const *d_levels, const int *level_h, const int *level_w, const int *level_blocked,
                            const int *level_offsets, int n_levels, int batch, int cin, int anchors, int mask_dim, const float *d_weight, const float *d_bias)
{
    bool ok = d_levels && level_h && level_w && level_blocked && level_offsets && d_weight && d_bias && n_levels >= 1 && n_levels <= kCoefLevels && batch >= 0 &&
              batch <= 65535 && cin >= 8 && cin % 8 == 0 && cin <= 1024 && anchors >= 1 && mask_dim >= 1 && mask_dim * kCoefParts <= 256 &&
              (mask_dim * kCoefParts) % 64 == 0 && (uintptr_t)d_weight % 16 == 0;
    long long next = 0;
    for (int i = 0; ok && i < n_levels; i++) {
        ok = d_levels[i] && level_h[i] >= 1 && level_w[i] >= 1 && level_offsets[i] == next &&
             (long long)batch * level_h[i] * level_w[i] * cin < (1ll << 40);
        next += (long long)level_h[i] * level_w[i] * anchors;
        ok = ok && next < (1ll << 31);
    }
    if (!ok) {
        set_error("%s: invalid argument (1 - %d levels, offsets = the running sum of h x w x anchors, cin %% 8 == 0 and <= 1024, mask_dim x %d a multiple of 64 up to 256)",
                  who, kCoefLevels, kCoefParts);
        return AMOS_ERR_INVALID;
    }
    lv = CoefLevels{};
    lv.n = n_levels;
    for (int i = 0; i < n_levels; i++) {
        lv.x[i] = d_levels[i]; lv.h[i] = level_h[i]; lv.w[i] = level_w[i]; lv.blocked[i] = level_blocked[i]; lv.off[i] = level_offsets[i];
    }
    return AMOS_OK;
}

static int launch_coef_at_priors(hipStream_t st, const CoefLevels &lv, int cin, const float *d_weight, const float *d_bias, const int *d_idx, int batch, int n,
                                 int anchors, int mask_dim, float *d_out)
{
    hipLaunchKernelGGL(k_coef_at_priors, dim3(n, batch), dim3(mask_dim * kCoefParts), (size_t)9 * cin * sizeof(float), st, lv, cin, d_weight, d_bias, d_idx, n, anchors,
                       mask_dim, d_out);
    AMOS_HIP_CHECK(hipGetLastError());
    return AMOS_OK;
}

int amos_mask_coef_at_priors_device(void *stream, const float *const *d_levels, const int *level_h, const int *level_w, const int *level_blocked,
                                    const int *level_offsets, int n_levels, int cin, const float *d_weight, const float *d_bias, const int *d_prior_idx, int batch,
                                    int n_slots, int anchors, int mask_dim, float *d_out)
{
    CoefLevels lv;
    if (!d_prior_idx || !d_out || n_slots < 0 || n_slots > 65535) { set_error("amos_mask_coef_at_priors_device: invalid argument"); return AMOS_ERR_INVALID; }
    const int rc = fill_coef_levels("amos_mask_coef_at_priors_device", lv, d_levels, level_h, level_w, level_blocked, level_offsets, n_levels, batch, cin, anchors,
                                    mask_dim, d_weight, d_bias);
    if (rc != AMOS_OK) return rc;
    if (batch == 0 || n_slots == 0) return AMOS_OK;
    return launch_coef_at_priors((hipStream_t)stream, lv, cin, d_weight, d_bias, d_prior_idx, batch, n_slots, anchors, mask_dim, d_out);
}

int amos_mask_person_masks_at_priors_device(void *stream, const float *d_loc, const float *d_conf, const float *const *d_levels, const int *level_h,
                                            const int *level_w, const int *level_blocked, const int *level_offsets, int n_levels, int cin, int anchors,
                                            const float *d_mask_weight, const float *d_mask_bias, const float *d_priors, const float *d_proto, int batch,
                                            int n_priors, int n_classes_with_background, int mask_dim, int proto_h, int proto_w, int out_h, int out_w,
                                            void *d_workspace, size_t workspace_bytes, uint8_t *d_masks, uint8_t *d_found)
{
    LazyCoef lazy;
    if (!d_conf) { set_error("amos_mask_person_masks_at_priors_device: invalid argument"); return AMOS_ERR_INVALID; }
    const int rc = fill_coef_levels("amos_mask_person_masks_at_priors_device", lazy.lv, d_levels, level_h, level_w, level_blocked, level_offsets, n_levels, batch, cin,
                                    anchors, mask_dim, d_mask_weight, d_mask_bias);
    if (rc != AMOS_OK) return rc;
    lazy.cin = cin; lazy.anchors = anchors; lazy.weight = d_mask_weight; lazy.bias = d_mask_bias;
    return person_masks(stream, d_loc, d_conf, nullptr, nullptr, &lazy, d_priors, d_proto, batch, n_priors, n_classes_with_background, mask_dim, proto_h, proto_w, out_h,
                        out_w, d_workspace, workspace_bytes, d_masks, d_found);
}

int amos_mask_person_masks_scores_at_priors_device(void *stream, const float *d_loc, const float *d_scores, const float *const *d_levels, const int *level_h,
                                                   const int *level_w, const int *level_blocked, const int *level_offsets, int n_levels, int cin, int anchors,
                                                   const float *d_mask_weight, const float *d_mask_bias, const float *d_priors, const float *d_proto, int batch,
                                                   int n_priors, int n_classes_with_background, int mask_dim, int proto_h, int proto_w, int out_h, int out_w,
                                                   void *d_workspace, size_t workspace_bytes, uint8_t *d_masks, uint8_t *d_found)
{
    LazyCoef lazy;
    if (!d_scores) { set_error("amos_mask_person_masks_scores_at_priors_device: invalid argument"); return AMOS_ERR_INVALID; }
    const int rc = fill_coef_levels("amos_mask_person_masks_scores_at_priors_device", lazy.lv, d_levels, level_h, level_w, level_blocked, level_offsets, n_levels, batch,
                                    cin, anchors, mask_dim, d_mask_weight, d_mask_bias);
    if (rc != AMOS_OK) return rc;
    lazy.cin = cin; lazy.anchors = anchors; lazy.weight = d_mask_weight; lazy.bias = d_mask_bias;
    return person_masks(stream, d_loc, nullptr, d_scores, nullptr, &lazy, d_priors, d_proto, batch, n_priors, n_classes_with_background, mask_dim, proto_h, proto_w, out_h,
                        out_w, d_workspace, workspace_bytes, d_masks, d_found);
}

static int person_masks(void *stream, const float *d_loc, const float *d_conf, const float *d_scores, const float *d_coef, const LazyCoef *lazy, const float *d_priors,
                        const float *d_proto, int batch, int n_priors, int n_classes_with_background, int mask_dim, int proto_h, int proto_w, int out_h, int out_w,
                        void *d_workspace, size_t workspace_bytes, uint8_t *d_masks, uint8_t *d_found)
{
    const int B = batch, P = n_priors, C1 = n_classes_with_background, C = C1 - 1, D = mask_dim, k = AMOS_MASK_NMS_TOP_K, nd = AMOS_MASK_TOP_K_DISPLAY;
    if (!d_loc || (!d_conf && !d_scores) || (!d_coef && !lazy) || !d_priors || !d_proto || !d_workspace || !d_masks || !d_found || B < 1 || B > 65535 || P < k || C1 < 2 || C1 > 200 ||
        D < 4 || D % 4 != 0 || proto_h < 1 || proto_w < 1 || out_h < 1 || out_w < 1 || (size_t)C * k * 4 > 64 * 1024 ||
        ((uintptr_t)d_loc | (uintptr_t)d_priors | (uintptr_t)d_proto | (uintptr_t)d_coef | (uintptr_t)d_workspace) % 16 != 0) {
        set_error("amos_mask_person_masks_device: invalid argument (16-byte aligned tensors, mask_dim %% 4 == 0, at most %d class lists of %d)", 16384 / k, k);
        return AMOS_ERR_INVALID;
    }
    if (lazy) {
        const CoefLevels &lv = lazy->lv;
        const long long last = (long long)lv.off[lv.n - 1] + (long long)lv.h[lv.n - 1] * lv.w[lv.n - 1] * lazy->anchors;
        if (last != P) { set_error("amos_mask_person_masks_at_priors_device: the levels hold %lld priors, n_priors is %d", last, P); return AMOS_ERR_INVALID; }
    }
    const PostLayout l = post_layout(B, P, C1, D, proto_h, proto_w);
    if (workspace_bytes < l.total) { set_error("amos_mask_person_masks_device: workspace of %zu bytes, %zu needed", workspace_bytes, l.total); return AMOS_ERR_CAPACITY; }
    uint8_t *ws = (uint8_t *)d_workspace;
    float4 *boxes = (float4 *)(ws + l.boxes);
    const float *cls = d_scores ? d_scores : (const float *)(ws + l.cls);
    float *topv = (float *)(ws + l.topv), *alive = (float *)(ws + l.alive), *selCoef = (float *)(ws + l.selCoef);
    long long *topi = (long long *)(ws + l.topi);
    float4 *selRect = (float4 *)(ws + l.selRect);
    uint8_t *flags = ws + l.flags;
    float *masks = (float *)(ws + l.masks);
    hipStream_t st = (hipStream_t)stream;
    const int total = B * P;
    hipLaunchKernelGGL(k_decode_boxes, dim3((total + 255) / 256), dim3(256), 0, st, (const float4 *)d_loc, (const float4 *)d_priors, boxes, P, total);
    int rc = d_scores ? AMOS_OK : amos_mask_class_scores_device(stream, d_conf, (float *)(ws + l.cls), B, P, C1, AMOS_MASK_CONF_THRESH);
    if (rc != AMOS_OK) return rc;
    rc = amos_mask_topk_rows_sparse_device(stream, cls, topv, topi, B * C, P, k, -1.f);
    if (rc != AMOS_OK) return rc;
    hipLaunchKernelGGL(k_nms_alive, dim3(B * C), dim3(256), 0, st, boxes, topi, topv, alive, k, P, C, AMOS_MASK_NMS_THRESH);
    int *selPrior = lazy ? (int *)(ws + l.selPrior) : nullptr;
    hipLaunchKernelGGL(k_select_display, dim3(B), dim3(256), 0, st, alive, topi, boxes, d_coef, selCoef, selRect, flags, d_found, C * k, k,
                       P, D, nd, AMOS_MASK_SCORE_THRESHOLD, AMOS_MASK_PERSON_CLASS, proto_w, proto_h, selPrior);
    if (lazy) {
        rc = launch_coef_at_priors(st, lazy->lv, lazy->cin, lazy->weight, lazy->bias, selPrior, B, nd, lazy->anchors, D, selCoef);
        if (rc != AMOS_OK) return rc;
    }
    hipLaunchKernelGGL(k_assemble_masks, dim3((proto_h * proto_w + 255) / 256, nd, B), dim3(256), 0, st, d_proto, selCoef, selRect, flags, masks, proto_h, proto_w, D, nd);
    AMOS_HIP_CHECK(hipGetLastError());
    return amos_mask_person_mask_device(stream, masks, flags, d_masks, B, nd, proto_h, proto_w, out_h, out_w);
}

}
```

### amos-slam_amd/mask/interface.py

```python
import os

import torch

from .detect import detect, detect_batch
from .net import YolactR50, _stem_eligible, lazy_coef_enabled, stem_kernel_enabled
from .post import person_mask, person_mask_batch, person_masks_fused
from .pre import cxx_marshalling, fast_base_transform, resize_f32_cv


class MaskEngine:
    def __init__(self, weight_path=None, device=None, seed=0, conv_dtype=None):
        if device is None:
            if not torch.cuda.is_available():
                raise RuntimeError("MaskEngine needs a GPU (PyTorch-ROCm); pass device='cpu' explicitly for CPU tests")
            device = "cuda:0"
        self.device = torch.device(device)
        torch.manual_seed(seed)
        self.net = YolactR50()
        self.has_weights = False
        if weight_path:
            self.net.load_weights(weight_path)
            self.has_weights = True
        self.net.eval().to(self.device)
        self.conv_dtype = conv_dtype
        self.use_hip_pre = True
        self.channels_last = self.device.type == "cuda"
        if self.channels_last:
            self.net.to(memory_format=torch.channels_last)
            torch.backends.cudnn.benchmark = True
        self._hip_pre = {}

    def prepare(self):
        self.net.fold_batch_norms()
        if self.device.type == "cuda" and os.environ.get("AMOS_MASK_MERGE_HEADS", "1") != "0":
            self.net.merge_head_outputs()
        if self.channels_last:
            self.net.to(memory_format=torch.channels_last)
        if self.device.type == "cuda" and os.environ.get("AMOS_MASK_WINOGRAD", "1") != "0":
            from .net import prepare_winograd_weights
            with torch.cuda.device(self.device):
                prepare_winograd_weights(self.net)
        if self.device.type == "cuda":
            from .net import prepare_stem_weight
            with torch.cuda.device(self.device):
                prepare_stem_weight(self.net)
        return self

    def _preprocess_hip(self, frames):
        from .. import MaskPreprocessor
        b, h, w = frames.shape[:3]
        pre = self._hip_pre.get((h, w))
        if pre is None or pre.max_batch < b:
            pre = MaskPreprocessor(w, h, max(b, 16), device=self.device.index or 0, stream=None)
            self._hip_pre[(h, w)] = pre
        out = torch.empty((b, 3, 550, 550), dtype=torch.float32, device=self.device)
        frames = frames.contiguous()
        cur = torch.cuda.current_stream(self.device)
        ev_in = torch.cuda.Event()
        ev_in.record(cur)
        ext = torch.cuda.ExternalStream(pre.stream, device=self.device)
        ext.wait_event(ev_in)
        pre.run(frames.data_ptr(), b, out.data_ptr())
        ev_out = torch.cuda.Event()
        ev_out.record(ext)
        cur.wait_event(ev_out)
        return out

    def _masks_of(self, x, width, height):
        fused_post = (self.device.type == "cuda" and self.conv_dtype is None and x.dtype == torch.float32 and x.is_cuda
                      and not torch.is_autocast_enabled() and os.environ.get("AMOS_MASK_FUSED_POST", "1") != "0")
        scores_only = fused_post and os.environ.get("AMOS_MASK_HEAD_SCORES", "0") == "1"
        before, self.net.lazy_coef = getattr(self.net, "lazy_coef", False), fused_post and lazy_coef_enabled()
        try:
            pred = self._forward(x, scores_only)
        finally:
            self.net.lazy_coef = before
        return self._person_masks(pred, width, height)

    def _forward(self, x, scores_only=False):
        if self.channels_last and not (self.conv_dtype is None and x.dtype == torch.float32 and stem_kernel_enabled() and _stem_eligible(self.net.backbone.conv1)):
            x = x.contiguous(memory_format=torch.channels_last)
        if self.conv_dtype is None:
            return self.net(x, scores_only) if scores_only else self.net(x)
        with torch.autocast(self.device.type, dtype=self.conv_dtype):
            pred = self.net(x)
        return {k: (v.float() if torch.is_tensor(v) and v.is_floating_point() else v) for k, v in pred.items()}

    @torch.no_grad()
    def network_outputs(self, image_chw):
        x = torch.as_tensor(image_chw, dtype=torch.float32, device=self.device)
        img = x.permute(1, 2, 0) * 255
        img = resize_f32_cv(img, 640, 480)
        return self._forward(fast_base_transform(img)), img

    @torch.no_grad()
    def eval_chw(self, image_chw):
        pred, img = self.network_outputs(image_chw)
        h, w = img.shape[:2]
        mask = person_mask(detect(pred), w, h)
        if mask is None:
            return None
        return mask

    @torch.no_grad()
    def eval_bgr(self, bgr_u8):
        frame = torch.as_tensor(bgr_u8, dtype=torch.uint8, device=self.device)
        return self.eval_chw(cxx_marshalling(frame))

    @staticmethod
    def _person_masks(pred, width, height):
        fused = person_masks_fused(pred, width, height)
        if fused is None and ("conf" not in pred or "mask" not in pred):
            raise RuntimeError("the pass was run for the fused post-processing (class scores only, or no coefficient tensor), which does not apply to its outputs")
        return fused if fused is not None else person_mask_batch(detect_batch(pred), width, height)

    @torch.no_grad()
    def eval_net_input_batch(self, x, chunk=16, height=480, width=640):
        B = x.shape[0]
        out = torch.zeros((B, height, width), dtype=torch.uint8, device=self.device)
        for b0 in range(0, B, chunk):
            masks, _found = self._masks_of(x[b0:b0 + chunk], width, height)
            out[b0:b0 + masks.shape[0]] = masks
        return out

    @torch.no_grad()
    def capture_graph(self, batch=1):
        if self.device.type != "cuda":
            raise RuntimeError("capture_graph needs the GPU")
        self._g_in = torch.zeros((batch, 3, 550, 550), dtype=torch.float32, device=self.device)

        def body():
            return self._masks_of(self._g_in, 640, 480)

        side = torch.cuda.Stream(device=self.device)
        side.wait_stream(torch.cuda.current_stream(self.device))
        with torch.cuda.stream(side):
            for _ in range(3):
                body()
        torch.cuda.current_stream(self.device).wait_stream(side)
        torch.cuda.synchronize(self.device)
        graph = torch.cuda.CUDAGraph()
        with torch.cuda.graph(graph):
            self._g_masks, self._g_found = body()
        self._graph, self._g_batch = graph, batch
        return self

    @torch.no_grad()
    def eval_net_input_graph(self, x):
        if getattr(self, "_graph", None) is None or x.shape[0] != self._g_batch:
            raise RuntimeError("eval_net_input_graph: call capture_graph(batch=%d) first" % x.shape[0])
        self._g_in.copy_(x)
        self._graph.replay()
        return self._g_masks, self._g_found

    @torch.no_grad()
    def eval_bgr_graph(self, frames_u8):
        frames = torch.as_tensor(frames_u8, dtype=torch.uint8, device=self.device)
        return self.eval_net_input_graph(self._preprocess_hip(frames))

    @torch.no_grad()
    def frame_session(self, height, width):
        key = (int(height), int(width))
        sessions = self.__dict__.setdefault("_sessions", {})
        if key not in sessions:
            sessions[key] = FrameSession(self, *key)
        return sessions[key]

    @torch.no_grad()
    def eval_bgr_batch(self, frames_u8, chunk=16):
        frames = torch.as_tensor(frames_u8, dtype=torch.uint8, device=self.device)
        B = frames.shape[0]
        out = torch.zeros((B, 480, 640), dtype=torch.uint8, device=self.device)
        for b0 in range(0, B, chunk):
            part = frames[b0:b0 + chunk]
            if self.device.type == "cuda" and self.use_hip_pre:
                x = self._preprocess_hip(part)
            else:
                chw = cxx_marshalling(part)
                imgs = resize_f32_cv(chw.permute(0, 2, 3, 1) * 255, 640, 480)
                x = fast_base_transform(imgs)
            masks, _found = self._masks_of(x, 640, 480)
            out[b0:b0 + part.shape[0]] = masks
        return out


class FrameSession:

    def __init__(self, engine, height, width):
        if engine.device.type != "cuda":
            raise RuntimeError("FrameSession needs the GPU")
        from .. import MaskPreprocessor
        dev = engine.device
        self.engine, self.height, self.width = engine, height, width
        self.stream = torch.cuda.Stream(device=dev)
        self.frame_in = torch.zeros((height, width, 3), dtype=torch.uint8).pin_memory()
        self.mask_out = torch.zeros((480, 640), dtype=torch.uint8).pin_memory()
        self._found_host = torch.zeros(1, dtype=torch.bool).pin_memory()
        self._d_frame = torch.zeros((1, height, width, 3), dtype=torch.uint8, device=dev)
        self._net_in = torch.zeros((1, 3, 550, 550), dtype=torch.float32, device=dev)
        self._pre = MaskPreprocessor(width, height, 1, device=dev.index or 0, stream=self.stream.cuda_stream)

        def body():
            self._pre.run(self._d_frame.data_ptr(), 1, self._net_in.data_ptr())
            return engine._masks_of(self._net_in, 640, 480)

        self.stream.wait_stream(torch.cuda.current_stream(dev))
        with torch.cuda.stream(self.stream):
            for _ in range(3):
                body()
        self.stream.synchronize()
        self._graph = torch.cuda.CUDAGraph()
        with torch.cuda.graph(self._graph, stream=self.stream):
            self._masks, self._found = body()
        self.stream.synchronize()

    @property
    def in_ptr(self):
        return self.frame_in.data_ptr()

    @property
    def out_ptr(self):
        return self.mask_out.data_ptr()

    @torch.no_grad()
    def run(self):
        with torch.cuda.stream(self.stream):
            self._d_frame[0].copy_(self.frame_in, non_blocking=True)
            self._graph.replay()
            self.mask_out.copy_(self._masks[0], non_blocking=True)
# ... 4 lines not shown
```

### amos-slam_amd/mask/net.py

```python
import math
import os

import torch
import torch.nn as nn
import torch.nn.functional as F

NUM_CLASSES = 81
MASK_DIM = 32
FPN_FEATURES = 256
CONF_THRESH = 0.05
MAX_SIZE = 550
PRED_SCALES = (24, 48, 96, 192, 384)
ASPECT_RATIOS = (1.0, 0.5, 2.0)


def _gemm_conv(conv, x):
    k = conv.kernel_size
    if k[0] != k[1] or conv.padding[0] != conv.padding[1] or conv.dilation != (1, 1) or conv.groups != 1 or conv.stride[0] != conv.stride[1]:
        return False
    from .. import mask_conv_supported
    if not mask_conv_supported(conv.in_channels, conv.out_channels, k[0], k[1], conv.stride[0], conv.padding[0]):
        return False
    s = conv.stride[0]
    m = x.shape[0] * ((x.shape[2] + 2 * conv.padding[0] - k[0]) // s + 1) * ((x.shape[3] + 2 * conv.padding[1] - k[1]) // s + 1)
# ... 361 lines not shown
            ch, cw = (h - 1) // 2 + 1, (w - 1) // 2 + 1
            y = torch.empty((b, 64, (ch - 1) // 2 + 1, (cw - 1) // 2 + 1), dtype=torch.float32, device=x.device, memory_format=cl)
            mask_stem(torch.cuda.current_stream(x.device).cuda_stream, x.data_ptr(), x.stride(), _stem_weight(self.conv1).data_ptr(), self.conv1.bias.data_ptr(),
                      y.data_ptr(), b, h, w)
            x = y
        elif self.conv1.bias is not None and x.is_cuda and x.dtype == torch.float32 and not torch.is_autocast_enabled():
            raw = F.conv2d(x, self.conv1.weight, None, self.conv1.stride, self.conv1.padding)
            if raw.is_contiguous(memory_format=cl) and raw.shape[1] % 4 == 0:
                from .. import mask_bias_relu_maxpool
                b, c, h, w = raw.shape
                y = torch.empty((b, c, (h - 1) // 2 + 1, (w - 1) // 2 + 1), dtype=torch.float32, device=x.device, memory_format=cl)
                mask_bias_relu_maxpool(torch.cuda.current_stream(x.device).cuda_stream, raw.data_ptr(), self.conv1.bias.data_ptr(), y.data_ptr(), b, h, w, c)
                x = y
            else:
                x = F.max_pool2d(F.relu(raw + self.conv1.bias.view(1, -1, 1, 1)), 3, stride=2, padding=1)
        else:
            x = conv_bias_act(self.conv1, x, True) if self.conv1.bias is not None else F.relu(self.bn1(self.conv1(x)))
            x = F.max_pool2d(x, 3, stride=2, padding=1)
        outs = []
        for layer in self.layers:
            x = layer(x)
            outs.append(x)
        return outs


_SIDE_STREAMS = {}


class Branches:

    def __init__(self, device, n=1):
        self.device = device
        self.main = torch.cuda.current_stream(device)
        key = (str(device), self.main.cuda_stream)
        if key not in _SIDE_STREAMS:
            if len(_SIDE_STREAMS) >= 64:
                _SIDE_STREAMS.clear()
            _SIDE_STREAMS[key] = []
        while len(_SIDE_STREAMS[key]) < n:
            _SIDE_STREAMS[key].append(torch.cuda.Stream(device))
        self.streams = _SIDE_STREAMS[key][:n]
        self.used = set()
        self.keep = []

    def side(self, i, fork=True):
        if i is None:
            return torch.cuda.stream(self.main)
        i %= len(self.streams)
        s = self.streams[i]
        if fork or i not in self.used:
            s.wait_stream(self.main)
        self.used.add(i)
        return torch.cuda.stream(s)

    def hold(self, *tensors):
        self.keep.extend(tensors)

    def join(self):
        for i in sorted(self.used):
            self.main.wait_stream(self.streams[i])
        self.used.clear()
        self.keep = []


def branches_for(x):
    mode = os.environ.get("AMOS_MASK_BRANCHES", "auto")
    if mode == "0" or not x.is_cuda:
        return None
    if mode != "1" and x.shape[0] > int(os.environ.get("AMOS_MASK_BRANCH_MAX_BATCH", "16")):
        return None
    return Branches(x.device, int(os.environ.get("AMOS_MASK_BRANCH_STREAMS", "1")))


class FeaturePyramid(nn.Module):

    def __init__(self, in_channels):
        super().__init__()
        self.lat_layers = nn.ModuleList([nn.Conv2d(c, FPN_FEATURES, 1) for c in reversed(in_channels)])
        self.pred_layers = nn.ModuleList([nn.Conv2d(FPN_FEATURES, FPN_FEATURES, 3, padding=1) for _ in in_channels])
        self.downsample_layers = nn.ModuleList([nn.Conv2d(FPN_FEATURES, FPN_FEATURES, 3, padding=1, stride=2) for _ in range(2)])

    def forward(self, feats, br=None, p3_blocked=False):
        n = len(feats)
        merged = [None] * n
        top = None
        for k, lat in enumerate(self.lat_layers):
            j = n - 1 - k
            up = bilinear(top, size=feats[j].shape[2:]) if top is not None else None
            merged[j] = top = conv_bias_act(lat, feats[j], False, residual=up)
        outs = [None] * n
        if br is not None and n == 3:
            br.hold(*merged)
            with br.side(0):
                outs[2] = conv_bias_act(self.pred_layers[0], merged[2], True)
                extra = []
                for down in self.downsample_layers:
                    extra.append(down(extra[-1] if extra else outs[2]))
            with br.side(1, fork=len(br.streams) > 1):
                outs[1] = conv_bias_act(self.pred_layers[1], merged[1], True)
            outs[0] = conv_bias_act(self.pred_layers[2], merged[0], True, out_blocked=p3_blocked)
            outs += extra
            br.hold(*outs)
            return outs
        for k, pred in enumerate(self.pred_layers):
            j = n - 1 - k
            outs[j] = conv_bias_act(pred, merged[j], True, out_blocked=p3_blocked and j == 0)
        for down in self.downsample_layers:
            outs.append(down(outs[-1]))
        return outs


class SharedHead(nn.Module):

    def __init__(self, num_priors=len(ASPECT_RATIOS)):
        super().__init__()
        self.upfeature = nn.Sequential(nn.Conv2d(FPN_FEATURES, FPN_FEATURES, 3, padding=1), nn.ReLU(inplace=True))
        self.bbox_layer = nn.Conv2d(FPN_FEATURES, num_priors * 4, 3, padding=1)
        self.conf_layer = nn.Conv2d(FPN_FEATURES, num_priors * NUM_CLASSES, 3, padding=1)
        self.mask_layer = nn.Conv2d(FPN_FEATURES, num_priors * MASK_DIM, 3, padding=1)

    def merge_output_layers(self):
        if getattr(self, "merged", None) is None:
            layers = (self.bbox_layer, self.conf_layer, self.mask_layer)
            n = sum(l.out_channels for l in layers)
            pad = (-n) % 64
            merged = nn.Conv2d(FPN_FEATURES, n + pad, 3, padding=1).to(device=self.bbox_layer.weight.device, dtype=self.bbox_layer.weight.dtype)
            with torch.no_grad():
                merged.weight.zero_()
                merged.bias.zero_()
                merged.weight[:n].copy_(torch.cat([l.weight for l in layers], 0))
                merged.bias[:n].copy_(torch.cat([l.bias for l in layers], 0))
            object.__setattr__(self, "merged", merged.requires_grad_(False))
        if getattr(self, "scores_boxes", None) is None:
            layers = (self.bbox_layer, self.conf_layer)
            n = sum(l.out_channels for l in layers)
            lean = nn.Conv2d(FPN_FEATURES, n + (-n) % 64, 3, padding=1).to(device=self.bbox_layer.weight.device, dtype=self.bbox_layer.weight.dtype)
            with torch.no_grad():
                lean.weight.zero_()
                lean.bias.zero_()
                lean.weight[:n].copy_(torch.cat([l.weight for l in layers], 0))
                lean.bias[:n].copy_(torch.cat([l.bias for l in layers], 0))
            object.__setattr__(lean, "rule_like", self.merged)
            object.__setattr__(self, "scores_boxes", lean.requires_grad_(False))
        return self

    def lazy_applies(self, x0):
        return self.fused_applies(x0) and getattr(self, "scores_boxes", None) is not None and self.mask_layer.weight.dtype == torch.float32 and (
            self.mask_layer.in_channels % 8 == 0 and MASK_DIM % 8 == 0 and MASK_DIM <= 32)

    def fused_applies(self, x0):
        merged = getattr(self, "merged", None)
        return not (merged is None or not x0.is_cuda or x0.dtype != torch.float32 or torch.is_autocast_enabled() or os.environ.get("AMOS_MASK_FUSED_HEAD", "1") == "0")

    def fused_outputs(self, pyramid, n_priors, br=None, out=None, scores=None, lazy=False):
        x0 = pyramid[0]
        if not self.fused_applies(x0):
            return None
        merged = self.scores_boxes if lazy else self.merged
        ups = [None] * len(pyramid)
        from .. import mask_head_outputs_scores
        b, dev = x0.shape[0], x0.device
        n_anchor = self.bbox_layer.out_channels // 4
        if out is None:
            if br is not None:
                raise ValueError("fused_outputs: with side streams the caller allocates the outputs")
            out = self.alloc_outputs(b, n_priors, dev)
        loc, conf, coef = out
        offs, off = [], 0
        for x in pyramid:
            offs.append(off)
            off += x.shape[2] * x.shape[3] * n_anchor
        if off != n_priors:
            raise ValueError("fused_outputs: %d priors written, %d expected" % (off, n_priors))

        def level(i):
            x = pyramid[i]
            u = conv_bias_act(self.upfeature[0], x, True, out_blocked=isinstance(x, Blocked))
            if lazy:
                ups[i] = u if isinstance(u, Blocked) or u.is_contiguous(memory_format=torch.channels_last) else u.contiguous(memory_format=torch.channels_last)
                if br is not None:
                    br.hold(ups[i].data if isinstance(u, Blocked) else ups[i])
            raw = conv_raw(merged, u)
            if not raw.is_contiguous(memory_format=torch.channels_last):
                raw = raw.contiguous(memory_format=torch.channels_last)
            cells = raw.shape[2] * raw.shape[3]
            mask_head_outputs_scores(torch.cuda.current_stream(dev).cuda_stream, raw.data_ptr(), merged.bias.data_ptr(), loc.data_ptr(),
                                     conf.data_ptr() if conf is not None else None, coef.data_ptr() if coef is not None else None,
                                     scores.data_ptr() if scores is not None else None,
                                     CONF_THRESH, b, cells, raw.shape[1], n_anchor, NUM_CLASSES, MASK_DIM, n_priors, offs[i])

        if br is not None and len(pyramid) == 5:
            with br.side(2 if len(br.streams) >= 3 else None):
                level(0)
            with br.side(1, fork=False):
                level(1)
            with br.side(0, fork=False):
                for i in (2, 3, 4):
                    level(i)
        else:
            for i in range(len(pyramid)):
                level(i)
        return loc, conf, (ups if lazy else coef)

    def alloc_outputs(self, b, n_priors, dev, conf=True, coef=True):
        return (torch.empty((b, n_priors, 4), dtype=torch.float32, device=dev),
                torch.empty((b, n_priors, NUM_CLASSES), dtype=torch.float32, device=dev) if conf else None,
                torch.empty((b, n_priors, MASK_DIM), dtype=torch.float32, device=dev) if coef else None)

    def alloc_scores(self, b, n_priors, dev):
        return torch.empty((b, NUM_CLASSES - 1, n_priors), dtype=torch.float32, device=dev)

    def forward(self, x):
        b = x.shape[0]
        x = conv_bias_act(self.upfeature[0], x, True)
        merged = getattr(self, "merged", None)
        if merged is not None:
            y = conv_bias_act(merged, x, False).permute(0, 2, 3, 1)
            n0, n1, n2 = self.bbox_layer.out_channels, self.conf_layer.out_channels, self.mask_layer.out_channels
            loc = y[..., :n0].reshape(b, -1, 4)
            conf = y[..., n0:n0 + n1].reshape(b, -1, NUM_CLASSES)
            coef = torch.tanh(y[..., n0 + n1:n0 + n1 + n2].reshape(b, -1, MASK_DIM))
            return loc, conf, coef
        loc = self.bbox_layer(x).permute(0, 2, 3, 1).reshape(b, -1, 4)
        conf = self.conf_layer(x).permute(0, 2, 3, 1).reshape(b, -1, NUM_CLASSES)
        coef = torch.tanh(self.mask_layer(x).permute(0, 2, 3, 1).reshape(b, -1, MASK_DIM))
        return loc, conf, coef


class _NoParams(nn.Module):
    """Levels 1..4 own no weights (they point at level 0): keeps the ModuleList length of the reference."""


class _Upsample2x(nn.Module):
    def forward(self, x):
        return bilinear(x, scale_factor=2)


def build_priors(conv_sizes, device="cpu"):
    rows = []
    for (h, w), scale in zip(conv_sizes, PRED_SCALES):
        for j in range(h):
            for i in range(w):
                x, y = (i + 0.5) / w, (j + 0.5) / h
                for ar in ASPECT_RATIOS:
                    side = scale * math.sqrt(ar) / MAX_SIZE
                    rows.append((x, y, side, side))
    return torch.tensor(rows, dtype=torch.float32, device=device)


def lazy_coef_enabled():
    return os.environ.get("AMOS_MASK_LAZY_COEF", "1") != "0"


def _outputs(loc, conf, cls, coef, priors, proto, head=None):
    out = {"loc": loc, "priors": priors, "proto": proto}
    if head is None:
        out["mask"] = coef
    else:
        out["upfeature"], out["mask_layer"] = coef, head.mask_layer
    if conf is not None:
        out["conf"] = conf
    if cls is not None:
        out["cls"] = cls
    return out


class YolactR50(nn.Module):
    def __init__(self):
        super().__init__()
        self.backbone = ResNet50Trunk()
        self.fpn = FeaturePyramid(self.backbone.channels[1:])
        c = FPN_FEATURES
        self.proto_net = nn.Sequential(
            nn.Conv2d(c, c, 3, padding=1), nn.ReLU(inplace=True), nn.Conv2d(c, c, 3, padding=1), nn.ReLU(inplace=True),
            nn.Conv2d(c, c, 3, padding=1), nn.ReLU(inplace=True), _Upsample2x(), nn.ReLU(inplace=True),
            nn.Conv2d(c, c, 3, padding=1), nn.ReLU(inplace=True), nn.Conv2d(c, MASK_DIM, 1))
        self.prediction_layers = nn.ModuleList([SharedHead()] + [_NoParams() for _ in range(4)])
        self.semantic_seg_conv = nn.Conv2d(c, NUM_CLASSES - 1, 1)
        self._prior_cache = {}

    def load_weights(self, path, map_location="cpu"):
        sd = torch.load(path, map_location=map_location)
        for key in list(sd.keys()):
            if key.startswith("backbone.layer") and not key.startswith("backbone.layers"):
                del sd[key]
            elif key.startswith("fpn.downsample_layers.") and int(key.split(".")[2]) >= 2:
                del sd[key]
        return self.load_state_dict(sd, strict=False)

    def fold_batch_norms(self):
        if not getattr(self, "_folded", False):
            self.backbone.fold_batch_norms()
            self._folded = True
        return self

    def merge_head_outputs(self):
        self.prediction_layers[0].merge_output_layers()
        return self

    def _apply(self, fn, *args, **kwargs):
        super()._apply(fn, *args, **kwargs)
        for name in ("merged", "scores_boxes"):
            layer = getattr(self.prediction_layers[0], name, None)
            if layer is not None:
                layer._apply(fn, *args, **kwargs)
        return self

    def forward(self, x, scores_only=False):
        feats = self.backbone(x)[1:]
        head = self.prediction_layers[0]
        lazy = bool(getattr(self, "lazy_coef", False)) and len(feats) == 3 and head.lazy_applies(feats[0])
        pn = self.proto_net

        def prototypes(p3):
            blk = isinstance(p3, Blocked)
            p = conv_bias_act(pn[4], conv_bias_act(pn[2], conv_bias_act(pn[0], p3, True, out_blocked=blk), True, out_blocked=blk), True, out_blocked=blk)
            p = conv_bias_act(pn[10], conv_bias_act(pn[8], bilinear(p, scale_factor=2, relu=True), True), True)
            return p.permute(0, 2, 3, 1).contiguous()

        def priors_of(pyramid):
            sizes = tuple(tuple(p.shape[2:]) for p in pyramid)
            key = (sizes, str(x.device))
            if key not in self._prior_cache:
                self._prior_cache[key] = build_priors(sizes, x.device)
            return self._prior_cache[key]

        chain = (len(feats) == 3 and head.fused_applies(feats[0]) and getattr(head, "merged", None) is not None and
                 blocked_chain_for(feats[0], (self.fpn.pred_layers[2], pn[0], pn[2], pn[4], head.upfeature[0], head.merged), (pn[8],)))
        br = branches_for(x) if head.fused_applies(feats[0]) and len(feats) == 3 else None
        if br is not None:
            sizes = [tuple(f.shape[2:]) for f in feats]
            for _ in range(2):
                sizes.append(((sizes[-1][0] - 1) // 2 + 1, (sizes[-1][1] - 1) // 2 + 1))
            n_priors = sum(h * w for h, w in sizes) * (head.bbox_layer.out_channels // 4)
            out = head.alloc_outputs(x.shape[0], n_priors, x.device, conf=not scores_only, coef=not lazy)
            cls = head.alloc_scores(x.shape[0], n_priors, x.device) if scores_only else None
            pyramid = self.fpn(feats, br, chain)
            priors = priors_of(pyramid)
            loc, conf, coef = head.fused_outputs(pyramid, priors.shape[0], br, out, cls, lazy)
            proto = prototypes(pyramid[0])
            br.join()
            return _outputs(loc, conf, cls, coef, priors, proto, head if lazy else None)
        pyramid = self.fpn(feats, None, chain)
        proto = prototypes(pyramid[0])
        priors = priors_of(pyramid)
        if head.fused_applies(pyramid[0]):
            out = head.alloc_outputs(x.shape[0], priors.shape[0], x.device, conf=not scores_only, coef=not lazy)
            cls = head.alloc_scores(x.shape[0], priors.shape[0], x.device) if scores_only else None
            loc, conf, coef = head.fused_outputs(pyramid, priors.shape[0], None, out, cls, lazy)
            return _outputs(loc, conf, cls, coef, priors, proto, head if lazy else None)
        locs, confs, coefs = zip(*(head(p) for p in pyramid))
        return {"loc": torch.cat(locs, 1), "conf": F.softmax(torch.cat(confs, 1), -1), "mask": torch.cat(coefs, 1),
                "priors": priors, "proto": proto}
```

### amos-slam_amd/mask/post.py

```python
import torch
import torch.nn.functional as F

SCORE_THRESHOLD = 0.15
TOP_K_DISPLAY = 15
PERSON_CLASS = 0


def _sanitize(a, b, size, padding):
    a, b = a * size, b * size
    lo, hi = torch.min(a, b), torch.max(a, b)
    return torch.clamp(lo - padding, min=0), torch.clamp(hi + padding, max=size)


def _crop(masks, boxes, padding=1):
    h, w, n = masks.shape
    x1, x2 = _sanitize(boxes[:, 0], boxes[:, 2], w, padding)
    y1, y2 = _sanitize(boxes[:, 1], boxes[:, 3], h, padding)
    cols = torch.arange(w, device=masks.device, dtype=x1.dtype).view(1, -1, 1)
    rows = torch.arange(h, device=masks.device, dtype=x1.dtype).view(-1, 1, 1)
    inside = (cols >= x1.view(1, 1, -1)) & (cols < x2.view(1, 1, -1)) & (rows >= y1.view(1, 1, -1)) & (rows < y2.view(1, 1, -1))
    return masks * inside.to(masks.dtype)


def postprocess_masks(det, w, h, score_threshold=SCORE_THRESHOLD):
    if det is None:
        return None
    keep = det["score"] > score_threshold
    if int(keep.sum()) == 0:
        return None
    classes, scores, boxes, coefs = det["class"][keep], det["score"][keep], det["box"][keep], det["mask"][keep]
    masks = torch.sigmoid(det["proto"] @ coefs.t())
    masks = _crop(masks, boxes).permute(2, 0, 1).contiguous()
    masks = F.interpolate(masks.unsqueeze(0), (h, w), mode="bilinear", align_corners=False).squeeze(0)
    return classes, scores, (masks > 0.5).to(torch.float32)


def person_mask(det, w, h):
    out = postprocess_masks(det, w, h)
    if out is None:
        return None
    classes, scores, masks = out
    order = scores.argsort(0, descending=True)[:TOP_K_DISPLAY]
    classes, masks = classes[order], masks[order]
    total = masks[classes == PERSON_CLASS].sum(0)
    return ((total.to(torch.int64) * 255) & 0xFF).to(torch.uint8)


def person_mask_batch(det, w, h):
    scores, classes, boxes, coefs, proto = det["score"], det["class"], det["box"], det["mask"], det["proto"]
    B = scores.shape[0]
    valid = scores > SCORE_THRESHOLD
    found = valid.any(dim=1)
    top_scores, order = torch.where(valid, scores, torch.full_like(scores, -1.0)).topk(TOP_K_DISPLAY, dim=1)
    sel_valid = top_scores > SCORE_THRESHOLD
    sel_cls = torch.gather(classes, 1, order)
    sel_box = torch.gather(boxes, 1, order[..., None].expand(-1, -1, 4))
    sel_coef = torch.gather(coefs, 1, order[..., None].expand(-1, -1, coefs.shape[-1]))
    masks = torch.sigmoid(torch.einsum("bhwk,bnk->bnhw", proto, sel_coef))
    ph, pw = masks.shape[2:]
    x1, x2 = _sanitize(sel_box[..., 0], sel_box[..., 2], pw, 1)
    y1, y2 = _sanitize(sel_box[..., 1], sel_box[..., 3], ph, 1)
    cols = torch.arange(pw, device=masks.device, dtype=x1.dtype).view(1, 1, 1, -1)
    rows = torch.arange(ph, device=masks.device, dtype=x1.dtype).view(1, 1, -1, 1)
    inside = (cols >= x1[..., None, None]) & (cols < x2[..., None, None]) & (rows >= y1[..., None, None]) & (rows < y2[..., None, None])
    masks = masks * inside.to(masks.dtype)
    person = sel_valid & (sel_cls == PERSON_CLASS)
    if masks.is_cuda and masks.dtype == torch.float32:
        from .. import mask_person_mask
        masks, flags = masks.contiguous(), person.to(torch.uint8).contiguous()
        out = torch.empty((B, h, w), dtype=torch.uint8, device=masks.device)
        mask_person_mask(torch.cuda.current_stream(masks.device).cuda_stream, masks.data_ptr(), flags.data_ptr(), out.data_ptr(), B, masks.shape[1], ph, pw, h, w)
        return out, found
    masks = F.interpolate(masks, (h, w), mode="bilinear", align_corners=False) > 0.5
    total = (masks & person[..., None, None]).sum(dim=1)
    return ((total.to(torch.int64) * 255) & 0xFF).to(torch.uint8), found


def person_masks_fused(pred, w, h):
    ups = pred.get("upfeature")
    loc, coef, priors, proto = pred["loc"], pred.get("mask"), pred["priors"], pred["proto"]
    if ups is not None:
        layer = pred["mask_layer"]
        coef = layer.weight
    cls = pred.get("cls")
    conf = pred.get("conf")
    scores = cls if cls is not None else conf
    if scores is None or not (loc.is_cuda and all(t.dtype == torch.float32 for t in (loc, scores, coef, priors, proto))) or proto.dim() != 4:
        return None
    import os
    if os.environ.get("AMOS_MASK_FUSED_POST", "1") == "0":
        return None
    from .. import mask_person_masks, mask_person_masks_scores, mask_post_workspace_bytes
    loc, scores, priors, proto = (t.contiguous() for t in (loc, scores, priors, proto))
    B, P = loc.shape[:2]
    ph, pw, D = proto.shape[1:]
    c1 = cls.shape[1] + 1 if cls is not None else conf.shape[2]
    if P < 200 or (c1 - 1) * 200 * 4 > 64 * 1024 or D % 4 != 0:
        return None
    nbytes = mask_post_workspace_bytes(B, P, c1, D, ph, pw)
    ws = torch.empty(nbytes, dtype=torch.uint8, device=loc.device)
    out = torch.empty((B, h, w), dtype=torch.uint8, device=loc.device)
    found = torch.empty(B, dtype=torch.uint8, device=loc.device)
    stream = torch.cuda.current_stream(loc.device).cuda_stream
    if ups is not None:
        from .. import mask_person_masks_at_priors
        from .net import Blocked
        weight = layer.weight.contiguous(memory_format=torch.channels_last)
        anchors = layer.out_channels // D
        if layer.kernel_size != (3, 3) or layer.padding != (1, 1) or layer.stride != (1, 1) or layer.out_channels != anchors * D or layer.bias is None:
            raise RuntimeError("person_masks_fused: the mask layer is not the 3 x 3, padding 1 convolution the lazy pass evaluates")
        blocked = [isinstance(u, Blocked) for u in ups]
        if any(tuple(u.shape[:2]) != (B, layer.in_channels) or u.dtype != torch.float32 for u in ups):
            raise RuntimeError("person_masks_fused: upfeature tensors of another batch, width or type than the pass")
        data = [u.data if f else u for u, f in zip(ups, blocked)]
        if not all(d.is_contiguous() if f else d.is_contiguous(memory_format=torch.channels_last) for d, f in zip(data, blocked)):
            raise RuntimeError("person_masks_fused: an upfeature tensor is neither channels-last nor channel-blocked")
        mask_person_masks_at_priors(stream, loc.data_ptr(), scores.data_ptr(), cls is not None, [d.data_ptr() for d in data], [tuple(u.shape[2:]) for u in ups], blocked,
                                    layer.in_channels, anchors, weight.data_ptr(), layer.bias.data_ptr(), priors.data_ptr(), proto.data_ptr(), B, P, c1, D, ph, pw,
                                    h, w, ws.data_ptr(), nbytes, out.data_ptr(), found.data_ptr())
        return out, found.bool()
    coef = coef.contiguous()
    (mask_person_masks_scores if cls is not None else mask_person_masks)(
        stream, loc.data_ptr(), scores.data_ptr(), coef.data_ptr(), priors.data_ptr(), proto.data_ptr(),
        B, P, c1, D, ph, pw, h, w, ws.data_ptr(), nbytes, out.data_ptr(), found.data_ptr())
    return out, found.bool()
```

### include/amos_frontend.h

```cpp
#ifndef AMOS_FRONTEND_H
#define AMOS_FRONTEND_H

#include <stddef.h>
#include <stdint.h>

#ifdef __cplusplus
extern "C" {
#endif

#define AMOS_OK 0
#define AMOS_ERR_INVALID (-1)
#define AMOS_ERR_DEVICE (-2)
#define AMOS_ERR_CAPACITY (-3)
#define AMOS_ERR_STATE (-4)

#define AMOS_EDGE_THRESHOLD 19
#define AMOS_MAX_LEVELS 16
#define AMOS_FRAME_GRID_ROWS 48
#define AMOS_FRAME_GRID_COLS 64
#define AMOS_TH_HIGH 100
#define AMOS_TH_LOW 50
#define AMOS_HISTO_LENGTH 30

typedef struct amos_keypoint {
// ... 317 lines not shown
    const uint8_t *d_has_point;
    const int32_t *d_pairs_kf, *d_pairs_f;
    int32_t *d_match;
    amos_bow_search_stats *d_stats;
    int32_t n_pairs, capacity;
    float nn_ratio;
    int32_t check_orientation;
} amos_bow_search;
int amos_match_bow_batch_device(amos_match *m, const amos_bow_search *s);
struct amos_bow_view;
int amos_match_bow(amos_match *m, const struct amos_bow_view *kf, const struct amos_bow_view *f, float nn_ratio, int check_orientation,
                   int32_t *matches_f, amos_bow_search_stats *stats);

typedef struct amos_kf_pair_search {
    const amos_keypoint *d_kps;
    const uint8_t *d_desc;
    const int32_t *d_counts;
    const int32_t *d_n_nodes;
    const uint32_t *d_node_ids;
    const int32_t *d_node_off;
    const int32_t *d_node_idx;
    const uint8_t *d_has_point;
    const float *d_u_right;
    const int32_t *d_pairs_1, *d_pairs_2;
    int32_t *d_match12;
    amos_bow_search_stats *d_stats;
    int32_t n_pairs, capacity;
} amos_kf_pair_search;
typedef struct amos_kf_geometry {
    float f12[9];
    float ex, ey;
} amos_kf_geometry;
int amos_match_bow_kf_batch_device(amos_match *m, const amos_kf_pair_search *s, float nn_ratio, int check_orientation);
int amos_match_triangulation_batch_device(amos_match *m, const amos_kf_pair_search *s, const amos_kf_geometry *d_geometry,
                                          const float *d_scale_factors, const float *d_level_sigma2, int n_levels, int only_stereo,
                                          int check_orientation);
int amos_match_bow_kf(amos_match *m, const struct amos_bow_view *k1, const struct amos_bow_view *k2, float nn_ratio, int check_orientation,
                      int32_t *match12, amos_bow_search_stats *stats);
int amos_match_triangulation(amos_match *m, const struct amos_bow_view *k1, const struct amos_bow_view *const *k2s, int n2,
                             const amos_kf_geometry *geometry, const float *scale_factors, const float *level_sigma2, int n_levels,
                             int only_stereo, int check_orientation, int32_t *match12, amos_bow_search_stats *stats);


int amos_mask_pre_create(int device, void *stream, int width, int height, int max_batch, amos_mask_pre **out);
void amos_mask_pre_destroy(amos_mask_pre *p);
void *amos_mask_pre_stream(amos_mask_pre *p);
int amos_mask_preprocess_batch_device(amos_mask_pre *p, const uint8_t *d_bgr, int n_frames, float *d_out);

int amos_orb_detect_color_with_mask_pre_batch_device(amos_orb *h, amos_mask_pre *pre, const uint8_t *d_color,
                                                     size_t frame_stride, size_t row_stride, int width, int height,
                                                     int n_frames, int channels, int rgb_order, float *d_net_input);

int amos_mask_bias_act_device(void *stream, float *d_y, const float *d_bias, const float *d_residual, size_t n,
                              int channels, int relu);

int amos_mask_bias_relu_maxpool_device(void *stream, const float *d_x, const float *d_bias, float *d_y, int n, int in_h, int in_w,
                                       int channels);

int amos_mask_stem_weight_floats(void);
int amos_mask_stem_weights_device(void *stream, const float *d_w, long long stride_n, long long stride_c, long long stride_y, long long stride_x,
                                  float *d_packed);
int amos_mask_stem_device(void *stream, const float *d_x, long long stride_b, long long stride_c, long long stride_y, long long stride_x,
                          const float *d_packed, const float *d_bias, float *d_y, int batch, int height, int width);

int amos_mask_conv_supported(int cin, int cout, int kh, int kw, int stride, int pad);
int amos_mask_conv_device(void *stream, const float *d_x, const float *d_w, const float *d_bias, const float *d_residual,
                          float *d_y, int batch, int in_h, int in_w, int cin, int cout, int kh, int kw, int stride, int pad,
                          int relu);
size_t amos_mask_conv_workspace_bytes(int batch, int in_h, int in_w, int cin, int cout, int kh, int kw, int stride, int pad);
int amos_mask_conv_ws_device(void *stream, const float *d_x, const float *d_w, const float *d_bias, const float *d_residual, float *d_y,
                             int batch, int in_h, int in_w, int cin, int cout, int kh, int kw, int stride, int pad, int relu,
                             void *d_workspace, size_t workspace_bytes);
int amos_mask_conv_tile_mode(int mode);
int amos_mask_conv_kernel_name(int batch, int in_h, int in_w, int cin, int cout, int kh, int kw, int stride, int pad, char *name,
                               int name_len);
int amos_mask_conv_chain_supported(int batch, int in_h, int in_w, int cin, int planes, int cout, int stride);
int amos_mask_conv_chain_device(void *stream, const float *d_x, const float *d_wd, const float *d_bd, const float *d_yc, const float *d_w3,
                                const float *d_b3, float *d_y, int batch, int in_h, int in_w, int cin, int planes, int cout, int stride);
int amos_mask_conv1x1_supported(int cin, int cout, int stride);

int amos_mask_winograd_supported(int cin, int cout);
size_t amos_mask_winograd_weight_floats(int cin, int cout);
int amos_mask_winograd_weights_device(void *stream, const float *d_w, float *d_u, int cin, int cout);
int amos_mask_winograd_conv_device(void *stream, const float *d_x, const float *d_u, const float *d_bias, const float *d_residual,
                                   float *d_y, int batch, int h, int w, int cin, int cout, int relu);
size_t amos_mask_winograd24_weight_floats(int cin, int cout);
int amos_mask_winograd24_weights_device(void *stream, const float *d_w, float *d_u, int cin, int cout);
int amos_mask_winograd24_conv_device(void *stream, const float *d_x, const float *d_u, const float *d_bias, const float *d_residual,
                                     float *d_y, int batch, int h, int w, int cin, int cout, int relu);
int amos_mask_winograd24_conv_layout_device(void *stream, const float *d_x, const float *d_u, const float *d_bias, const float *d_residual,
                                            float *d_y, int batch, int h, int w, int cin, int cout, int relu, int in_blocked, int out_blocked);
int amos_mask_winograd24_persistent_mode(int mode);
int amos_mask_winograd24_narrow_mode(int mode);
int amos_mask_conv1x1_device(void *stream, const float *d_x, const float *d_w, const float *d_bias, const float *d_residual,
                             float *d_y, int batch, int in_h, int in_w, int cin, int cout, int stride, int relu);

int amos_mask_bilinear_nhwc_device(void *stream, const float *d_x, float *d_y, int n, int in_h, int in_w, int out_h,
                                   int out_w, int channels, float scale_h, float scale_w);

int amos_mask_bilinear_nhwc_act_device(void *stream, const float *d_x, float *d_y, int n, int in_h, int in_w, int out_h,
                                       int out_w, int channels, float scale_h, float scale_w, int relu);

int amos_mask_bilinear_x2_mode(int mode);

int amos_mask_nms_column_max_device(void *stream, const float *d_boxes, float *d_out, int n_lists, int k);

int amos_mask_class_scores_device(void *stream, const float *d_conf, float *d_scores, int batch, int n_priors,
                                  int n_classes_with_background, float threshold);

int amos_mask_person_mask_device(void *stream, const float *d_masks, const uint8_t *d_flags, uint8_t *d_out, int batch, int n_det,
                                 int mask_h, int mask_w, int out_h, int out_w);

int amos_mask_head_outputs_device(void *stream, const float *d_raw, const float *d_bias, float *d_loc, float *d_conf, float *d_coef,
                                  int batch, int cells, int channels_padded, int anchors, int n_classes_with_background, int mask_dim,
                                  int n_priors_total, int prior_offset);
int amos_mask_head_outputs_scores_device(void *stream, const float *d_raw, const float *d_bias, float *d_loc, float *d_conf, float *d_coef, float *d_scores,
                                         float threshold, int batch, int cells, int channels_padded, int anchors, int n_classes_with_background,
                                         int mask_dim, int n_priors_total, int prior_offset);

int amos_mask_topk_rows_device(void *stream, const float *d_x, float *d_values, long long *d_indices, int rows, int n, int k);
int amos_mask_topk_rows_sparse_device(void *stream, const float *d_x, float *d_values, long long *d_indices, int rows, int n, int k, float fill);

#define AMOS_MASK_NMS_TOP_K 200
#define AMOS_MASK_NMS_THRESH 0.5f
#define AMOS_MASK_CONF_THRESH 0.05f
#define AMOS_MASK_SCORE_THRESHOLD 0.15f
#define AMOS_MASK_TOP_K_DISPLAY 15
#define AMOS_MASK_PERSON_CLASS 0
size_t amos_mask_post_workspace_bytes(int batch, int n_priors, int n_classes_with_background, int mask_dim, int proto_h, int proto_w);
int amos_mask_person_masks_device(void *stream, const float *d_loc, const float *d_conf, const float *d_coef, const float *d_priors,
                                  const float *d_proto, int batch, int n_priors, int n_classes_with_background, int mask_dim, int proto_h,
                                  int proto_w, int out_h, int out_w, void *d_workspace, size_t workspace_bytes, uint8_t *d_masks,
                                  uint8_t *d_found);
int amos_mask_person_masks_scores_device(void *stream, const float *d_loc, const float *d_scores, const float *d_coef, const float *d_priors,
                                         const float *d_proto, int batch, int n_priors, int n_classes_with_background, int mask_dim, int proto_h,
                                         int proto_w, int out_h, int out_w, void *d_workspace, size_t workspace_bytes, uint8_t *d_masks,
                                         uint8_t *d_found);

int amos_mask_coef_at_priors_device(void *stream, const float *const *d_levels, const int *level_h, const int *level_w, const int *level_blocked,
                                    const int *level_offsets, int n_levels, int cin, const float *d_weight, const float *d_bias,
                                    const int *d_prior_idx, int batch, int n_slots, int anchors, int mask_dim, float *d_out);
int amos_mask_person_masks_at_priors_device(void *stream, const float *d_loc, const float *d_conf, const float *const *d_levels, const int *level_h,
                                            const int *level_w, const int *level_blocked, const int *level_offsets, int n_levels, int cin,
                                            int anchors, const float *d_mask_weight, const float *d_mask_bias, const float *d_priors,
                                            const float *d_proto, int batch, int n_priors, int n_classes_with_background, int mask_dim, int proto_h,
                                            int proto_w, int out_h, int out_w, void *d_workspace, size_t workspace_bytes, uint8_t *d_masks,
                                            uint8_t *d_found);
int amos_mask_person_masks_scores_at_priors_device(void *stream, const float *d_loc, const float *d_scores, const float *const *d_levels,
                                                   const int *level_h, const int *level_w, const int *level_blocked, const int *level_offsets,
                                                   int n_levels, int cin, int anchors, const float *d_mask_weight, const float *d_mask_bias,
                                                   const float *d_priors, const float *d_proto, int batch, int n_priors,
                                                   int n_classes_with_background, int mask_dim, int proto_h, int proto_w, int out_h, int out_w,
                                                   void *d_workspace, size_t workspace_bytes, uint8_t *d_masks, uint8_t *d_found);



typedef struct amos_slic_center {
    int32_t x, y;
    int32_t L, A, B, D;
    int32_t label;
    int32_t id;
} amos_slic_center;

typedef struct amos_slic amos_slic;
int amos_slic_center_count(int width, int height, int len, int *nx, int *ny);
int amos_slic_create(int device, void *stream, int max_width, int max_height, int max_batch, amos_slic **out);
void amos_slic_destroy(amos_slic *s);
void *amos_slic_stream(amos_slic *s);
int amos_slic_run(amos_slic *s, const uint8_t *lab, const uint16_t *depth, int width, int height, int len, int m, int iterations,
              double *labels, amos_slic_center *centers, int *n_centers);
int amos_slic_batch_device(amos_slic *s, const uint8_t *d_lab, const uint16_t *d_depth, int width, int height, int n_frames,
                           int len, int m, int iterations, double *d_labels, amos_slic_center *d_centers);

int amos_cluster_bgr2lab_batch_device(amos_slic *s, const uint8_t *d_bgr, size_t n_pixels, int rgb_order, uint8_t *d_lab);

int amos_cluster_kmeans_batch_device(amos_slic *s, amos_slic_center *d_centers, int n_centers, int n_frames, int k,
                                     uint32_t seed, int max_iter, int32_t *d_passes );
int amos_cluster_kmeans(amos_slic *s, amos_slic_center *centers, int n_centers, int k, uint32_t seed, int max_iter,
                        int *passes);


int amos_flow_check_device(void *stream, const uint8_t *d_last_gray, size_t last_stride, const uint8_t *d_cur_gray,
                           size_t cur_stride, int cols, int rows, const float *d_pre_xy, const float *d_next_xy,
                           const uint8_t *d_state_in, int n, uint8_t *d_state_out);
int amos_flow_epipolar_device(void *stream, const double *d_F, const float *d_pre_xy, const float *d_next_xy,
                              const uint8_t *d_state, int n, double *d_dd);
typedef struct amos_scene_flow_camera {
    float cx, cy, invfx, invfy;
    float Tlw[12];
    float Rwc[9], Ow[3];
} amos_scene_flow_camera;
int amos_flow_scene_flow_device(void *stream, const float *d_depth_last, size_t last_stride, const float *d_depth_cur,
                                size_t cur_stride, const float *d_match_pre_xy, const float *d_match_cur_xy, int n,
                                const amos_scene_flow_camera *cam, float *d_out);
int amos_flow_fundamental_score_device(void *stream, const double *d_F, int n_hypotheses, const float *d_points1_xy, const float *d_points2_xy,
                                       int n, double threshold, float *d_err, int32_t *d_inliers, uint8_t *d_mask);
int amos_flow_pnp_score_device(void *stream, const double *d_Rt, int n_hypotheses, const float *d_object_xyz, const float *d_image_xy, int n,
                               double fx, double fy, double cx, double cy, double reprojection_error, float *d_err, int32_t *d_inliers,
                               uint8_t *d_mask);

typedef struct amos_lk amos_lk;
int amos_lk_create(int device, void *stream, int width, int height, int win_size, int max_level, amos_lk **out);
void amos_lk_destroy(amos_lk *k);
void *amos_lk_stream(amos_lk *k);
int amos_lk_levels(const amos_lk *k);
int amos_lk_track_device(amos_lk *k, const uint8_t *d_prev_gray, size_t prev_stride, const uint8_t *d_next_gray,
                         size_t next_stride, const float *d_prev_xy, int n, int max_count, double epsilon,
                         float min_eig_threshold, float *d_next_xy, uint8_t *d_status, float *d_err );

typedef struct amos_corners amos_corners;
int amos_corners_create(int device, void *stream, int max_width, int max_height, amos_corners **out);
void amos_corners_destroy(amos_corners *c);
void *amos_corners_stream(amos_corners *c);
int amos_corners_good_features_device(amos_corners *c, const uint8_t *d_gray, size_t stride, int width, int height, int max_corners,
                                      double quality_level, double min_distance, double harris_k, float *d_xy, int xy_capacity,
                                      int *d_count, float *d_response );
int amos_corners_candidate_count(amos_corners *c, int *count);
int amos_corners_subpix_device(amos_corners *c, const uint8_t *d_gray, size_t stride, int width, int height, float *d_xy,
                               const int *d_count , int n, int win, int max_count, double epsilon);

typedef struct amos_fmat amos_fmat;
int amos_fmat_create(int device, void *stream, int max_points , int max_problems, amos_fmat **out);
void amos_fmat_destroy(amos_fmat *h);
void *amos_fmat_stream(amos_fmat *h);
int amos_fmat_ransac_device(amos_fmat *h, int n_problems, const float *d_p1_xy, const float *d_p2_xy, const int32_t *d_offsets,
                            const int32_t *d_counts, const uint8_t *d_select, double threshold, double confidence, int max_iters,
                            double *d_F, int32_t *d_status, uint8_t *d_mask);
int amos_fmat_scene_flow_pair_device(amos_fmat *h, const float *d_pre_xy, const float *d_next_xy, const uint8_t *d_state,
                                     const int32_t *d_n, double *d_F1, double *d_F2, uint8_t *d_keep, int32_t *d_status);
int amos_fmat_ransac(amos_fmat *h, int n, const float *p1_xy, const float *p2_xy, double threshold, double confidence, int max_iters,
                     double *F, uint8_t *mask, int32_t *status);

typedef struct amos_pnp amos_pnp;
int amos_pnp_create(int device, void *stream, int max_points , int max_problems, amos_pnp **out);
void amos_pnp_destroy(amos_pnp *h);
void *amos_pnp_stream(amos_pnp *h);
int amos_pnp_ransac_device(amos_pnp *h, int n_problems, const float *d_object_xyz, const float *d_image_xy, const int32_t *d_offsets,
                           const int32_t *d_counts, const uint8_t *d_select, double fx, double fy, double cx, double cy,
                           double reprojection_error, double confidence, int max_iters, double *d_Rt, int32_t *d_status, uint8_t *d_mask);
int amos_pnp_scene_flow_device(amos_pnp *h, const float *d_pre_xy, const float *d_next_xy, const uint8_t *d_state, const int32_t *d_n,
                               const float *d_depth_last, size_t last_stride, const float *d_depth_cur, size_t cur_stride, int width,
                               int height, const amos_scene_flow_camera *cam, double fx, double fy, double *d_Rt, int32_t *d_status,
                               uint8_t *d_mask);
int amos_pnp_ransac(amos_pnp *h, int n, const float *object_xyz, const float *image_xy, double fx, double fy, double cx, double cy,
                    double reprojection_error, double confidence, int max_iters, double *Rt, uint8_t *mask, int32_t *status);

#define AMOS_DYNA_MAX_K 64
#define AMOS_DYNA_COUNTS 6
#define AMOS_DYNA_NO_PNP 1
#define AMOS_DYNA_NO_F2 2
#define AMOS_DYNA_BAD_N 4
#define AMOS_DYNA_RESET 8
#define AMOS_DYNA_BAD_MATCH_LABEL 1
#define AMOS_DYNA_BAD_TM_LABEL 2
#define AMOS_DYNA_BAD_ID 4
typedef struct amos_dyna amos_dyna;
typedef struct amos_dyna_poses {
    float motion[12];
    float lk[12];
    int32_t has_lk;
} amos_dyna_poses;
typedef struct amos_dyna_results {
    int32_t max_points, max_frames;
    float *pose;
    float *rwc, *ow;
    int32_t *choice;
    int32_t *counts;
    float *match_xy;
    float *rpe;
    double *epipolar;
    float *tm_xy;
    float *flow;
    int32_t *status;
    float *ave_rpe;
    int32_t *ep_num;
    int32_t *decide_status;
    float *pre_xy, *next_xy;
    uint8_t *state;
    int32_t *n;
    double *F1, *F2;
    int32_t *fmat_status;
    double *Rt;
    int32_t *pnp_status;
} amos_dyna_results;
int amos_dyna_create(int device, void *stream, int max_points , int max_frames, amos_dyna **out);
void amos_dyna_destroy(amos_dyna *h);
void *amos_dyna_stream(amos_dyna *h);
int amos_dyna_results_device(amos_dyna *h, amos_dyna_results *out);
int amos_dyna_copy_to_host(amos_dyna *h, void *dst, const void *d_src, size_t bytes);
int amos_dyna_tail_device(amos_dyna *h, int frame, const float *d_pre_xy, const float *d_next_xy, const uint8_t *d_state, const int32_t *d_n,
                          const double *d_F2, const int32_t *d_fmat_status, const double *d_Rt, const int32_t *d_pnp_status,
                          const float *d_depth_last, size_t last_stride, const float *d_depth_cur, size_t cur_stride, int width, int height,
                          const amos_scene_flow_camera *cam, double fx, double fy, const amos_dyna_poses *poses);
int amos_dyna_reset_frame_device(amos_dyna *h, int frame);
int amos_dyna_decide_batch_device(amos_dyna *h, int n_frames, const double *d_labels, size_t label_frame_stride, size_t label_row_stride,
                                  int width, int height, const amos_slic_center *d_centers, size_t centers_frame_stride, int n_centers, int k,
                                  int32_t *d_rm, size_t rm_frame_stride);
int amos_dyna_scene_flow_obj_device(amos_dyna *h, int frame, amos_corners *corners, amos_lk *lk, amos_fmat *fmat, amos_pnp *pnp,
                                    const uint8_t *d_imlast_gray, size_t last_gray_stride, const uint8_t *d_gray, size_t gray_stride, int width,
                                    int height, const float *d_depth_last, size_t last_stride, const float *d_depth_cur, size_t cur_stride,
                                    const amos_scene_flow_camera *cam, double fx, double fy, const amos_dyna_poses *poses);

#ifdef __cplusplus
}
#endif
#endif
// ... 1 lines not shown
```

Measured before the change: 1627 frames/s.

## Emit above-threshold class candidates from fused head and top-k from compact lists

The fused prediction-head kernel gains a candidate mode. In that mode it does the softmax thresholding in place and appends packed (score key, prior index) entries into per-class lists through shared-memory and global atomics, so the full conf tensor is never written. A new list top-k kernel takes the top k from these compact lists, using a bitonic sort for small lists and a radix select for large ones, and NMS skips empty lists early. This removes the dense per-class scoring and top-k over all priors, at the cost of atomics and more code paths. It depends on the model's candidates flag being set.

```diff
diff --git a/amos-slam_amd/__init__.py b/amos-slam_amd/__init__.py
--- a/amos-slam_amd/__init__.py
+++ b/amos-slam_amd/__init__.py
@@ -133,6 +133,12 @@
     "amos_mask_coef_at_priors_device": (_i, (_v, _v, _v, _v, _v, _v, _i, _i, _v, _v, _v, _i, _i, _i, _i, _v)),
     "amos_mask_person_masks_at_priors_device": (_i, (_v, _v, _v, _v, _v, _v, _v, _v, _i, _i, _i, _v, _v, _v, _v, _i, _i, _i, _i, _i, _i, _i, _i, _v, _z, _v, _v)),
     "amos_mask_person_masks_scores_at_priors_device": (_i, (_v, _v, _v, _v, _v, _v, _v, _v, _i, _i, _i, _v, _v, _v, _v, _i, _i, _i, _i, _i, _i, _i, _i, _v, _z, _v, _v)),
+    "amos_mask_candidates_bytes": (_z, (_i, _i, _i)),
+    "amos_mask_candidates_reset_device": (_i, (_v, _v, _i, _i)),
+    "amos_mask_head_candidates_device": (_i, (_v, _v, _v, _v, _v, _v, _f, _i, _i, _i, _i, _i, _i, _i, _i)),
+    "amos_mask_topk_lists_device": (_i, (_v, _v, _v, _i, _v, _v, _i, _i)),
+    "amos_mask_person_masks_candidates_device": (_i, (_v, _v, _v, _v, _v, _v, _i, _i, _i, _i, _i, _i, _i, _i, _v, _z, _v, _v)),
+    "amos_mask_person_masks_candidates_at_priors_device": (_i, (_v, _v, _v, _v, _v, _v, _v, _v, _i, _i, _i, _v, _v, _v, _v, _i, _i, _i, _i, _i, _i, _i, _i, _v, _z, _v, _v)),
     "amos_slic_center_count": (_i, (_i, _i, _i, _v, _v)),
     "amos_slic_create": (_i, (_i, _v, _i, _i, _i, _v)),
     "amos_slic_destroy": (None, (_v,)),
@@ -717,10 +723,36 @@
                                                  batch, n_slots, anchors, mask_dim, out_ptr), "amos_mask_coef_at_priors_device")
 
 
+def mask_candidates_bytes(batch, n_priors, n_classes_with_background):
+    return int(lib().amos_mask_candidates_bytes(batch, n_priors, n_classes_with_background))
+
+
+def mask_candidates_reset(stream_ptr, candidates_ptr, batch, n_classes_with_background):
+    _check(lib().amos_mask_candidates_reset_device(stream_ptr, candidates_ptr, batch, n_classes_with_background), "amos_mask_candidates_reset_device")
+
+
+def mask_head_candidates(stream_ptr, raw_ptr, bias_ptr, loc_ptr, coef_ptr, candidates_ptr, threshold, batch, cells, channels_padded, anchors,
+                         n_classes_with_background, mask_dim, n_priors_total, prior_offset):
+    _check(lib().amos_mask_head_candidates_device(stream_ptr, raw_ptr, bias_ptr, loc_ptr, coef_ptr, candidates_ptr, threshold, batch, cells, channels_padded,
+                                                  anchors, n_classes_with_background, mask_dim, n_priors_total, prior_offset), "amos_mask_head_candidates_device")
+
+
+def mask_topk_lists(stream_ptr, counts_ptr, entries_ptr, capacity, values_ptr, indices_ptr, rows, k):
+    _check(lib().amos_mask_topk_lists_device(stream_ptr, counts_ptr, entries_ptr, capacity, values_ptr, indices_ptr, rows, k), "amos_mask_topk_lists_device")
+
+
+def mask_person_masks_candidates(stream_ptr, loc_ptr, candidates_ptr, coef_ptr, priors_ptr, proto_ptr, batch, n_priors, n_classes_with_background, mask_dim,
+                                 proto_h, proto_w, out_h, out_w, workspace_ptr, workspace_bytes, masks_ptr, found_ptr):
+    _check(lib().amos_mask_person_masks_candidates_device(stream_ptr, loc_ptr, candidates_ptr, coef_ptr, priors_ptr, proto_ptr, batch, n_priors,
+                                                          n_classes_with_background, mask_dim, proto_h, proto_w, out_h, out_w, workspace_ptr, workspace_bytes,
+                                                          masks_ptr, found_ptr), "amos_mask_person_masks_candidates_device")
+
+
 def mask_person_masks_at_priors(stream_ptr, loc_ptr, scores_ptr, scores_are_class_scores, level_ptrs, level_hw, level_blocked, cin, anchors, mask_weight_ptr,
                                 mask_bias_ptr, priors_ptr, proto_ptr, batch, n_priors, n_classes_with_background, mask_dim, proto_h, proto_w, out_h, out_w,
                                 workspace_ptr, workspace_bytes, masks_ptr, found_ptr):
-    name = "amos_mask_person_masks_scores_at_priors_device" if scores_are_class_scores else "amos_mask_person_masks_at_priors_device"
+    name = ("amos_mask_person_masks_candidates_at_priors_device" if scores_are_class_scores == "candidates" else
+            "amos_mask_person_masks_scores_at_priors_device" if scores_are_class_scores else "amos_mask_person_masks_at_priors_device")
     _check(getattr(lib(), name)(stream_ptr, loc_ptr, scores_ptr, *_coef_levels(level_ptrs, level_hw, level_blocked, anchors), cin, anchors, mask_weight_ptr,
                                 mask_bias_ptr, priors_ptr, proto_ptr, batch, n_priors, n_classes_with_background, mask_dim, proto_h, proto_w, out_h, out_w,
                                 workspace_ptr, workspace_bytes, masks_ptr, found_ptr), name)
diff --git a/amos-slam_amd/csrc/amos_mask_post.hip b/amos-slam_amd/csrc/amos_mask_post.hip
--- a/amos-slam_amd/csrc/amos_mask_post.hip
+++ b/amos-slam_amd/csrc/amos_mask_post.hip
@@ -99,9 +99,12 @@
 }
 
 constexpr int kHeadCells = 16;
+__device__ __forceinline__ unsigned topk_key(float f);
+template <bool kCand>
 __global__ __launch_bounds__(256) void k_head_outputs(const float *__restrict__ raw, const float *__restrict__ bias, float *__restrict__ loc, float *__restrict__ conf,
                                                      float *__restrict__ coef, int cells, int cpad, int A, int C1, int D, int P, int pOff,
-                                                     float *__restrict__ scores, float thresh)
+                                                     float *__restrict__ scores, float thresh, int *__restrict__ candCount,
+                                                     unsigned long long *__restrict__ candEntries)
 {
     extern __shared__ float sh[];
     const int b = blockIdx.y, c0 = blockIdx.x * kHeadCells, nc = min(kHeadCells, cells - c0);
@@ -113,6 +116,8 @@
         v.x = __fadd_rn(v.x, bb.x); v.y = __fadd_rn(v.y, bb.y); v.z = __fadd_rn(v.z, bb.z); v.w = __fadd_rn(v.w, bb.w);
         *reinterpret_cast<float4 *>(sh + e) = v;
     }
+    __shared__ unsigned sCnt[kCand ? 256 : 1], sBase[kCand ? 256 : 1];
+    if constexpr (kCand) sCnt[threadIdx.x] = 0u;
     __syncthreads();
     __shared__ float sMax[256], sSum[256];
 #define AMOS_HEAD_FOREACH(n, body)                                                             \
@@ -126,7 +131,18 @@
             if (r >= (n)) { r -= (n); cell++; }                                                \
         }                                                                                      \
     }
-    if ((int)threadIdx.x < nc * A) {
+    if constexpr (kCand) {
+        int parts = 1;
+        while (parts * 2 * kHeadCells * A <= 256) parts *= 2;
+        const int prior = (int)threadIdx.x / parts, part = (int)threadIdx.x - prior * parts;
+        const bool have = prior < nc * A;
+        const int cell = have ? prior / A : 0, a = have ? prior - cell * A : 0;
+        const float *v = sh + cell * cpad + nLoc + a * C1;
+        float m = v[min(part, C1 - 1)];
+        for (int c = part + parts; c < C1; c += parts) m = fmaxf(m, v[c]);
+        for (int d = 1; d < parts; d <<= 1) m = fmaxf(m, __shfl_xor(m, d, 64));
+        if (have && part == 0) sMax[prior] = m;
+    } else if ((int)threadIdx.x < nc * A) {
         const int cell = threadIdx.x / A, a = threadIdx.x - cell * A;
         const float *v = sh + cell * cpad + nLoc + a * C1;
         float m = v[0];
@@ -151,11 +167,52 @@
         const int cell = threadIdx.x / A, a = threadIdx.x - cell * A;
         const float *v = sh + cell * cpad + nLoc + a * C1;
         float sum = 0.f;
+#pragma unroll 16
         for (int c = 0; c < C1; c++) sum = __fadd_rn(sum, v[c]);
         sSum[threadIdx.x] = sum;
     }
     __syncthreads();
     const size_t prior0 = (size_t)b * P + pOff + (size_t)c0 * A;
+    if constexpr (kCand) {
+        const int C = C1 - 1;
+        const float pre = thresh * 0.99f;
+        unsigned long long mine = 0ull;
+        int trip = 0;
+        AMOS_HEAD_FOREACH(nConf, {
+            int a = (int)((float)r * invC1);
+            a -= a * C1 > r ? 1 : 0;
+            a += (a + 1) * C1 <= r ? 1 : 0;
+            const int c = r - a * C1;
+            const float ev = sh[cell * cpad + nLoc + r];
+            const float s = sSum[cell * A + a];
+            if (c >= 1 && ev > s * pre && ev / s > thresh) {
+                mine |= 1ull << trip;
+                atomicAdd(&sCnt[c - 1], 1u);
+            }
+            trip++;
+        })
+        __syncthreads();
+        unsigned base = 0u;
+        if ((int)threadIdx.x < C && sCnt[threadIdx.x]) base = (unsigned)atomicAdd(&candCount[(size_t)b * C + threadIdx.x], (int)sCnt[threadIdx.x]);
+        AMOS_HEAD_FOREACH(nLoc, loc[prior0 * 4 + e] = sh[cell * cpad + r])
+        if (nCoef) AMOS_HEAD_FOREACH(nCoef, coef[prior0 * D + e] = sh[cell * cpad + nLoc + nConf + r])
+        if ((int)threadIdx.x < C) {
+            sBase[threadIdx.x] = base;
+            sCnt[threadIdx.x] = 0u;
+        }
+        __syncthreads();
+        while (mine) {
+            const int tr = (int)__builtin_ctzll(mine);
+            mine &= mine - 1ull;
+            const int e = (int)threadIdx.x + 256 * tr, cell = e / nConf, r = e - cell * nConf, a = r / C1, c = r - a * C1;
+            const float q = sh[cell * cpad + nLoc + r] / sSum[cell * A + a];
+            const unsigned slot = sBase[c - 1] + atomicAdd(&sCnt[c - 1], 1u);
+            const unsigned prior = (unsigned)(pOff + (c0 + cell) * A + a);
+            if (slot < (unsigned)P)
+                candEntries[((size_t)b * C + (c - 1)) * P + slot] = ((unsigned long long)topk_key(q) << 32) | (0xffffffffu - prior);
+        }
+        return;
+    }
     AMOS_HEAD_FOREACH(nLoc, loc[prior0 * 4 + e] = sh[cell * cpad + r])
     if (nCoef) AMOS_HEAD_FOREACH(nCoef, coef[prior0 * D + e] = sh[cell * cpad + nLoc + nConf + r])
     if (!scores) {
@@ -650,6 +707,156 @@
     }
 }
 
+constexpr int kListThreads = 256, kListLoads = 16;
+__device__ __forceinline__ void hist_count(unsigned *hist, bool in, unsigned bin, int lane)
+{
+    const unsigned long long m = __ballot(in);
+    if (m) {
+        const int first = (int)__builtin_ctzll(m);
+        const unsigned b0 = __builtin_amdgcn_readlane(bin, first);
+        const bool same = __ballot(in && bin != b0) == 0ull;
+        if (same) {
+            if (lane == first) atomicAdd(&hist[b0], (unsigned)__popcll(m));
+        } else if (in) {
+            atomicAdd(&hist[bin], 1u);
+        }
+    }
+}
+__global__ __launch_bounds__(kListThreads) void k_topk_lists(const int *__restrict__ counts, const unsigned long long *__restrict__ entries, int cap,
+                                                   float *__restrict__ values, long long *__restrict__ indices, int k, int perFrame)
+{
+    const int frames = (int)gridDim.x / perFrame, row = ((int)blockIdx.x % frames) * perFrame + (int)blockIdx.x / frames;
+    __shared__ unsigned long long list[kTopkList];
+    __shared__ unsigned hist[kTopkBins];
+    __shared__ unsigned part[256];
+    __shared__ unsigned long long sel[256];
+    __shared__ unsigned long long sPrefix, sMask;
+    __shared__ unsigned sNeed, sTaken, sDone;
+    const int t = threadIdx.x, lane = t & 63;
+    const int count = min(max(counts[row], 0), cap);
+    const unsigned long long *src = entries + (size_t)row * cap;
+    float *val = values + (size_t)row * k;
+    long long *idx = indices + (size_t)row * k;
+    if (count == 0) {
+        if (t < k) { val[t] = -1.f; idx[t] = 0; }
+        return;
+    }
+    if (count <= kTopkList) {
+        unsigned n2 = 64;
+        while (n2 < (unsigned)count) n2 <<= 1;
+        for (unsigned i = t; i < n2; i += kListThreads) list[i] = i < (unsigned)count ? src[i] : 0ull;
+        __syncthreads();
+        for (unsigned size = 2; size <= n2; size <<= 1)
+            for (unsigned stride = size >> 1; stride > 0; stride >>= 1) {
+                for (unsigned i = t; i < n2 / 2; i += kListThreads) {
+                    const unsigned lo = ((i / stride) * stride * 2) + (i % stride), hi = lo + stride;
+                    const unsigned long long a = list[lo], b = list[hi];
+                    const bool descending = (lo & size) == 0;
+                    if (descending ? a < b : a > b) { list[lo] = b; list[hi] = a; }
+                }
+                __syncthreads();
+            }
+        if (t < k) {
+            const unsigned long long v = t < count ? list[t] : 0ull;
+            val[t] = t < count ? topk_value((unsigned)(v >> 32)) : -1.f;
+            idx[t] = t < count ? (long long)(0xffffffffu - (unsigned)(v & 0xffffffffu)) : 0;
+        }
+        return;
+    }
+    if (t == 0) { sPrefix = 0ull; sMask = 0ull; sNeed = (unsigned)k; sTaken = 0u; sDone = 0u; }
+    __syncthreads();
+    const int shifts[6] = {53, 42, 32, 21, 10, 0}, widths[6] = {11, 11, 10, 11, 11, 10};
+    for (int pass = 0; pass < 6; pass++) {
+        const int shift = shifts[pass];
+        const unsigned bins = 1u << widths[pass];
+        for (int b = t; b < kTopkBins; b += kListThreads) hist[b] = 0;
+        __syncthreads();
+        const unsigned long long prefix = sPrefix, mask = sMask;
+        const unsigned need = sNeed;
+        for (int i0 = 0; i0 < count; i0 += kListThreads * kListLoads) {
+            unsigned long long e[kListLoads];
+#pragma unroll
+            for (int u = 0; u < kListLoads; u++) {
+                const int i = i0 + u * kListThreads + t;
+                e[u] = i < count ? src[i] : 0ull;
+            }
+#pragma unroll
+            for (int u = 0; u < kListLoads; u++) {
+                const int i = i0 + u * kListThreads + t;
+                hist_count(hist, i < count && (e[u] & mask) == prefix, (unsigned)(e[u] >> shift) & (bins - 1u), lane);
+            }
+        }
+        __syncthreads();
+        if (t < 256) {
+            unsigned p = 0;
+            for (int b = 0; b < 8; b++) p += hist[8 * t + b];
+            part[t] = p;
+        }
+        __syncthreads();
+        if (t < 64) {
+            const unsigned q = part[4 * lane] + part[4 * lane + 1] + part[4 * lane + 2] + part[4 * lane + 3];
+            unsigned suffix = q;
+            for (int d = 1; d < 64; d <<= 1) {
+                const unsigned o = __shfl_down(suffix, d, 64);
+                if (lane + d < 64) suffix += o;
+            }
+            const unsigned above = suffix - q;
+            if (above < need && suffix >= need) {
+                unsigned acc = above;
+                int bin = 32 * lane + 31;
+                for (; bin > 32 * lane; bin--) {
+                    const unsigned c = hist[bin];
+                    if (acc + c >= need) break;
+                    acc += c;
+                }
+                sPrefix = prefix | ((unsigned long long)bin << shift);
+                sMask = mask | ((unsigned long long)(bins - 1u) << shift);
+                sNeed = need - acc;
+                sDone = hist[bin] == need - acc ? 1u : 0u;
+            }
+        }
+        __syncthreads();
+        if (sDone) break;
+    }
+    const unsigned long long T = sPrefix;
+    for (int i0 = 0; i0 < count; i0 += kListThreads * kListLoads) {
+        unsigned long long e[kListLoads];
+#pragma unroll
+        for (int u = 0; u < kListLoads; u++) {
+            const int i = i0 + u * kListThreads + t;
+            e[u] = i < count ? src[i] : 0ull;
+        }
+#pragma unroll
+        for (int u = 0; u < kListLoads; u++) {
+            const int i = i0 + u * kListThreads + t;
+            if (i < count && e[u] >= T) {
+                const unsigned slot = atomicAdd(&sTaken, 1u);
+                if (slot < 256u) sel[slot] = e[u];
+            }
+        }
+    }
+    __syncthreads();
+    for (unsigned i = min(sTaken, 256u) + t; i < 256u; i += kListThreads) sel[i] = 0ull;
+    __syncthreads();
+    for (int size = 2; size <= 256; size <<= 1)
+        for (int stride = size >> 1; stride > 0; stride >>= 1) {
+            unsigned long long a = 0ull, b = 0ull;
+            if (t < 256) { a = sel[t]; b = sel[t ^ stride]; }
+            __syncthreads();
+            if (t < 256) {
+                const bool descending = (t & size) == 0, lower = (t & stride) == 0;
+                const unsigned long long hi = a > b ? a : b, lo = a > b ? b : a;
+                sel[t] = (descending == lower) ? hi : lo;
+            }
+            __syncthreads();
+        }
+    if (t < k) {
+        const unsigned long long v = sel[t];
+        val[t] = topk_value((unsigned)(v >> 32));
+        idx[t] = (long long)(0xffffffffu - (unsigned)(v & 0xffffffffu));
+    }
+}
+
 
 
 __global__ __launch_bounds__(256) void k_decode_boxes(const float4 *__restrict__ loc, const float4 *__restrict__ priors, float4 *__restrict__ boxes, int P, int total)
@@ -668,7 +875,12 @@
 {
     __shared__ float4 sb[256];
     __shared__ float sarea[256];
-    const int j = threadIdx.x, list = blockIdx.x, b = list / C;
+    const int frames = (int)gridDim.x / C, list = ((int)blockIdx.x % frames) * C + (int)blockIdx.x / frames;
+    const int j = threadIdx.x, b = list / C;
+    if (scores[(size_t)list * k] <= 0.f) {
+        if (j < k) out[(size_t)list * k + j] = -1.f;
+        return;
+    }
     float4 me = {0.f, 0.f, 0.f, 0.f};
     float myArea = 0.f;
     if (j < k) {
@@ -895,11 +1107,70 @@
         return AMOS_ERR_INVALID;
     }
     if (batch == 0) return AMOS_OK;
-    hipLaunchKernelGGL(k_head_outputs, dim3((cells + kHeadCells - 1) / kHeadCells, batch), dim3(256), (size_t)kHeadCells * channels_padded * sizeof(float),
+    hipLaunchKernelGGL(k_head_outputs<false>, dim3((cells + kHeadCells - 1) / kHeadCells, batch), dim3(256), (size_t)kHeadCells * channels_padded * sizeof(float),
                        (hipStream_t)stream, d_raw, d_bias, d_loc, d_conf, d_coef, cells, channels_padded, anchors, n_classes_with_background, mask_dim,
-                       n_priors_total, prior_offset, d_scores, threshold);
+                       n_priors_total, prior_offset, d_scores, threshold, (int *)nullptr, (unsigned long long *)nullptr);
     AMOS_HIP_CHECK(hipGetLastError());
     return AMOS_OK;
+}
+
+static size_t cand_counts_bytes(int batch, int classes) { return ((size_t)batch * classes * sizeof(int) + 255) & ~(size_t)255; }
+
+size_t amos_mask_candidates_bytes(int batch, int n_priors, int n_classes_with_background)
+{
+    if (batch < 1 || n_priors < 1 || n_classes_with_background < 2) return 0;
+    const int C = n_classes_with_background - 1;
+    return cand_counts_bytes(batch, C) + (size_t)batch * C * n_priors * sizeof(unsigned long long);
+}
+
+int amos_mask_candidates_reset_device(void *stream, void *d_candidates, int batch, int n_classes_with_background)
+{
+    if (!d_candidates || batch < 0 || n_classes_with_background < 2) { set_error("amos_mask_candidates_reset_device: invalid argument"); return AMOS_ERR_INVALID; }
+    if (batch == 0) return AMOS_OK;
+    AMOS_HIP_CHECK(hipMemsetAsync(d_candidates, 0, (size_t)batch * (n_classes_with_background - 1) * sizeof(int), (hipStream_t)stream));
+    return AMOS_OK;
+}
+
+int amos_mask_head_candidates_device(void *stream, const float *d_raw, const float *d_bias, float *d_loc, float *d_coef, void *d_candidates, float threshold,
+                                     int batch, int cells, int channels_padded, int anchors, int n_classes_with_background, int mask_dim, int n_priors_total,
+                                     int prior_offset)
+{
+    const long long used = (long long)anchors * (4 + n_classes_with_background + (d_coef ? mask_dim : 0));
+    if (!d_raw || !d_bias || !d_loc || !d_candidates || !(threshold >= 0.f) || batch < 0 || cells < 1 || anchors < 1 || n_classes_with_background < 2 ||
+        n_classes_with_background > 257 || mask_dim < 1 || channels_padded % 4 != 0 || used > channels_padded || channels_padded > 1000 || prior_offset < 0 ||
+        (long long)prior_offset + (long long)cells * anchors > n_priors_total || batch > 65535 || kHeadCells * anchors > 256 ||
+        ((uintptr_t)d_raw | (uintptr_t)d_bias | (uintptr_t)d_candidates) % 16 != 0) {
+        set_error("amos_mask_head_candidates_device: invalid argument (2 <= classes incl. background <= 257, threshold >= 0)");
+        return AMOS_ERR_INVALID;
+    }
+    if (batch == 0) return AMOS_OK;
+    uint8_t *cand = (uint8_t *)d_candidates;
+    hipLaunchKernelGGL(k_head_outputs<true>, dim3((cells + kHeadCells - 1) / kHeadCells, batch), dim3(256), (size_t)kHeadCells * channels_padded * sizeof(float),
+                       (hipStream_t)stream, d_raw, d_bias, d_loc, (float *)nullptr, d_coef, cells, channels_padded, anchors, n_classes_with_background, mask_dim,
+                       n_priors_total, prior_offset, (float *)nullptr, threshold, (int *)cand,
+                       (unsigned long long *)(cand + cand_counts_bytes(batch, n_classes_with_background - 1)));
+    AMOS_HIP_CHECK(hipGetLastError());
+    return AMOS_OK;
+}
+
+static int launch_topk_lists(hipStream_t stream, const int *d_counts, const unsigned long long *d_entries, int capacity, float *d_values, long long *d_indices, int rows,
+                             int k, int per_frame)
+{
+    hipLaunchKernelGGL(k_topk_lists, dim3(rows), dim3(kListThreads), 0, stream, d_counts, d_entries, capacity, d_values, d_indices, k,
+                       per_frame >= 1 && rows % per_frame == 0 ? per_frame : 1);
+    AMOS_HIP_CHECK(hipGetLastError());
+    return AMOS_OK;
+}
+
+int amos_mask_topk_lists_device(void *stream, const int *d_counts, const unsigned long long *d_entries, int capacity, float *d_values, long long *d_indices,
+                                int rows, int k)
+{
+    if (!d_counts || !d_entries || !d_values || !d_indices || rows < 0 || capacity < 1 || k < 1 || k > 256 || (uintptr_t)d_entries % 8 != 0) {
+        set_error("amos_mask_topk_lists_device: invalid argument (1 <= k <= 256)");
+        return AMOS_ERR_INVALID;
+    }
+    if (rows == 0) return AMOS_OK;
+    return launch_topk_lists((hipStream_t)stream, d_counts, d_entries, capacity, d_values, d_indices, rows, k, 1);
 }
 
 static DeviceOnce g_topk_lds_once;
@@ -978,7 +1249,7 @@
                             const int *level_offsets, int n_levels, int batch, int cin, int anchors, int mask_dim, const float *d_weight, const float *d_bias);
 static int launch_coef_at_priors(hipStream_t st, const CoefLevels &lv, int cin, const float *d_weight, const float *d_bias, const int *d_idx, int batch, int n,
                                  int anchors, int mask_dim, float *d_out);
-static int person_masks(void *stream, const float *d_loc, const float *d_conf, const float *d_scores, const float *d_coef, const LazyCoef *lazy, const float *d_priors,
+static int person_masks(void *stream, const float *d_loc, const float *d_conf, const float *d_scores, const void *d_cand, const float *d_coef, const LazyCoef *lazy, const float *d_priors,
                         const float *d_proto, int batch, int n_priors, int n_classes_with_background, int mask_dim, int proto_h, int proto_w, int out_h, int out_w,
                         void *d_workspace, size_t workspace_bytes, uint8_t *d_masks, uint8_t *d_found);
 
@@ -987,7 +1258,7 @@
                                   void *d_workspace, size_t workspace_bytes, uint8_t *d_masks, uint8_t *d_found)
 {
     if (!d_conf) { set_error("amos_mask_person_masks_device: invalid argument"); return AMOS_ERR_INVALID; }
-    return person_masks(stream, d_loc, d_conf, nullptr, d_coef, nullptr, d_priors, d_proto, batch, n_priors, n_classes_with_background, mask_dim, proto_h, proto_w, out_h, out_w,
+    return person_masks(stream, d_loc, d_conf, nullptr, nullptr, d_coef, nullptr, d_priors, d_proto, batch, n_priors, n_classes_with_background, mask_dim, proto_h, proto_w, out_h, out_w,
                         d_workspace, workspace_bytes, d_masks, d_found);
 }
 
@@ -996,7 +1267,7 @@
                                          void *d_workspace, size_t workspace_bytes, uint8_t *d_masks, uint8_t *d_found)
 {
     if (!d_scores) { set_error("amos_mask_person_masks_scores_device: invalid argument"); return AMOS_ERR_INVALID; }
-    return person_masks(stream, d_loc, nullptr, d_scores, d_coef, nullptr, d_priors, d_proto, batch, n_priors, n_classes_with_background, mask_dim, proto_h, proto_w, out_h, out_w,
+    return person_masks(stream, d_loc, nullptr, d_scores, nullptr, d_coef, nullptr, d_priors, d_proto, batch, n_priors, n_classes_with_background, mask_dim, proto_h, proto_w, out_h, out_w,
                         d_workspace, workspace_bytes, d_masks, d_found);
 }
 
@@ -1060,7 +1331,7 @@
                                     anchors, mask_dim, d_mask_weight, d_mask_bias);
     if (rc != AMOS_OK) return rc;
     lazy.cin = cin; lazy.anchors = anchors; lazy.weight = d_mask_weight; lazy.bias = d_mask_bias;
-    return person_masks(stream, d_loc, d_conf, nullptr, nullptr, &lazy, d_priors, d_proto, batch, n_priors, n_classes_with_background, mask_dim, proto_h, proto_w, out_h,
+    return person_masks(stream, d_loc, d_conf, nullptr, nullptr, nullptr, &lazy, d_priors, d_proto, batch, n_priors, n_classes_with_background, mask_dim, proto_h, proto_w, out_h,
                         out_w, d_workspace, workspace_bytes, d_masks, d_found);
 }
 
@@ -1076,18 +1347,43 @@
                                     cin, anchors, mask_dim, d_mask_weight, d_mask_bias);
     if (rc != AMOS_OK) return rc;
     lazy.cin = cin; lazy.anchors = anchors; lazy.weight = d_mask_weight; lazy.bias = d_mask_bias;
-    return person_masks(stream, d_loc, nullptr, d_scores, nullptr, &lazy, d_priors, d_proto, batch, n_priors, n_classes_with_background, mask_dim, proto_h, proto_w, out_h,
+    return person_masks(stream, d_loc, nullptr, d_scores, nullptr, nullptr, &lazy, d_priors, d_proto, batch, n_priors, n_classes_with_background, mask_dim, proto_h, proto_w, out_h,
                         out_w, d_workspace, workspace_bytes, d_masks, d_found);
 }
 
-static int person_masks(void *stream, const float *d_loc, const float *d_conf, const float *d_scores, const float *d_coef, const LazyCoef *lazy, const float *d_priors,
+int amos_mask_person_masks_candidates_device(void *stream, const float *d_loc, const void *d_candidates, const float *d_coef, const float *d_priors,
+                                             const float *d_proto, int batch, int n_priors, int n_classes_with_background, int mask_dim, int proto_h, int proto_w,
+                                             int out_h, int out_w, void *d_workspace, size_t workspace_bytes, uint8_t *d_masks, uint8_t *d_found)
+{
+    if (!d_candidates) { set_error("amos_mask_person_masks_candidates_device: invalid argument"); return AMOS_ERR_INVALID; }
+    return person_masks(stream, d_loc, nullptr, nullptr, d_candidates, d_coef, nullptr, d_priors, d_proto, batch, n_priors, n_classes_with_background, mask_dim, proto_h, proto_w,
+                        out_h, out_w, d_workspace, workspace_bytes, d_masks, d_found);
+}
+
+int amos_mask_person_masks_candidates_at_priors_device(void *stream, const float *d_loc, const void *d_candidates, const float *const *d_levels, const int *level_h,
+                                                       const int *level_w, const int *level_blocked, const int *level_offsets, int n_levels, int cin, int anchors,
+                                                       const float *d_mask_weight, const float *d_mask_bias, const float *d_priors, const float *d_proto, int batch,
+                                                       int n_priors, int n_classes_with_background, int mask_dim, int proto_h, int proto_w, int out_h, int out_w,
+                                                       void *d_workspace, size_t workspace_bytes, uint8_t *d_masks, uint8_t *d_found)
+{
+    LazyCoef lazy;
+    if (!d_candidates) { set_error("amos_mask_person_masks_candidates_at_priors_device: invalid argument"); return AMOS_ERR_INVALID; }
+    const int rc = fill_coef_levels("amos_mask_person_masks_candidates_at_priors_device", lazy.lv, d_levels, level_h, level_w, level_blocked, level_offsets, n_levels, batch,
+                                    cin, anchors, mask_dim, d_mask_weight, d_mask_bias);
+    if (rc != AMOS_OK) return rc;
+    lazy.cin = cin; lazy.anchors = anchors; lazy.weight = d_mask_weight; lazy.bias = d_mask_bias;
+    return person_masks(stream, d_loc, nullptr, nullptr, d_candidates, nullptr, &lazy, d_priors, d_proto, batch, n_priors, n_classes_with_background, mask_dim, proto_h, proto_w,
+                        out_h, out_w, d_workspace, workspace_bytes, d_masks, d_found);
+}
+
+static int person_masks(void *stream, const float *d_loc, const float *d_conf, const float *d_scores, const void *d_cand, const float *d_coef, const LazyCoef *lazy, const float *d_priors,
                         const float *d_proto, int batch, int n_priors, int n_classes_with_background, int mask_dim, int proto_h, int proto_w, int out_h, int out_w,
                         void *d_workspace, size_t workspace_bytes, uint8_t *d_masks, uint8_t *d_found)
 {
     const int B = batch, P = n_priors, C1 = n_classes_with_background, C = C1 - 1, D = mask_dim, k = AMOS_MASK_NMS_TOP_K, nd = AMOS_MASK_TOP_K_DISPLAY;
-    if (!d_loc || (!d_conf && !d_scores) || (!d_coef && !lazy) || !d_priors || !d_proto || !d_workspace || !d_masks || !d_found || B < 1 || B > 65535 || P < k || C1 < 2 || C1 > 200 ||
+    if (!d_loc || (!d_conf && !d_scores && !d_cand) || (!d_coef && !lazy) || !d_priors || !d_proto || !d_workspace || !d_masks || !d_found || B < 1 || B > 65535 || P < k || C1 < 2 || C1 > 200 ||
         D < 4 || D % 4 != 0 || proto_h < 1 || proto_w < 1 || out_h < 1 || out_w < 1 || (size_t)C * k * 4 > 64 * 1024 ||
-        ((uintptr_t)d_loc | (uintptr_t)d_priors | (uintptr_t)d_proto | (uintptr_t)d_coef | (uintptr_t)d_workspace) % 16 != 0) {
+        ((uintptr_t)d_loc | (uintptr_t)d_priors | (uintptr_t)d_proto | (uintptr_t)d_coef | (uintptr_t)d_workspace | (uintptr_t)d_cand) % 16 != 0) {
         set_error("amos_mask_person_masks_device: invalid argument (16-byte aligned tensors, mask_dim %% 4 == 0, at most %d class lists of %d)", 16384 / k, k);
         return AMOS_ERR_INVALID;
     }
@@ -1109,9 +1405,15 @@
     hipStream_t st = (hipStream_t)stream;
     const int total = B * P;
     hipLaunchKernelGGL(k_decode_boxes, dim3((total + 255) / 256), dim3(256), 0, st, (const float4 *)d_loc, (const float4 *)d_priors, boxes, P, total);
-    int rc = d_scores ? AMOS_OK : amos_mask_class_scores_device(stream, d_conf, (float *)(ws + l.cls), B, P, C1, AMOS_MASK_CONF_THRESH);
-    if (rc != AMOS_OK) return rc;
-    rc = amos_mask_topk_rows_sparse_device(stream, cls, topv, topi, B * C, P, k, -1.f);
+    int rc;
+    if (d_cand) {
+        const uint8_t *cand = (const uint8_t *)d_cand;
+        rc = launch_topk_lists(st, (const int *)cand, (const unsigned long long *)(cand + cand_counts_bytes(B, C)), P, topv, topi, B * C, k, C);
+    } else {
+        rc = d_scores ? AMOS_OK : amos_mask_class_scores_device(stream, d_conf, (float *)(ws + l.cls), B, P, C1, AMOS_MASK_CONF_THRESH);
+        if (rc != AMOS_OK) return rc;
+        rc = amos_mask_topk_rows_sparse_device(stream, cls, topv, topi, B * C, P, k, -1.f);
+    }
     if (rc != AMOS_OK) return rc;
     hipLaunchKernelGGL(k_nms_alive, dim3(B * C), dim3(256), 0, st, boxes, topi, topv, alive, k, P, C, AMOS_MASK_NMS_THRESH);
     int *selPrior = lazy ? (int *)(ws + l.selPrior) : nullptr;
diff --git a/amos-slam_amd/mask/interface.py b/amos-slam_amd/mask/interface.py
--- a/amos-slam_amd/mask/interface.py
+++ b/amos-slam_amd/mask/interface.py
@@ -3,7 +3,7 @@
 import torch
 
 from .detect import detect, detect_batch
-from .net import YolactR50, _stem_eligible, lazy_coef_enabled, stem_kernel_enabled
+from .net import YolactR50, _stem_eligible, candidates_enabled, lazy_coef_enabled, stem_kernel_enabled
 from .post import person_mask, person_mask_batch, person_masks_fused
 from .pre import cxx_marshalling, fast_base_transform, resize_f32_cv
 
@@ -71,10 +71,11 @@
                       and not torch.is_autocast_enabled() and os.environ.get("AMOS_MASK_FUSED_POST", "1") != "0")
         scores_only = fused_post and os.environ.get("AMOS_MASK_HEAD_SCORES", "0") == "1"
         before, self.net.lazy_coef = getattr(self.net, "lazy_coef", False), fused_post and lazy_coef_enabled()
+        before_cand, self.net.candidates = getattr(self.net, "candidates", False), fused_post and candidates_enabled()
         try:
             pred = self._forward(x, scores_only)
         finally:
-            self.net.lazy_coef = before
+            self.net.lazy_coef, self.net.candidates = before, before_cand
         return self._person_masks(pred, width, height)
 
     def _forward(self, x, scores_only=False):
diff --git a/amos-slam_amd/mask/net.py b/amos-slam_amd/mask/net.py
--- a/amos-slam_amd/mask/net.py
+++ b/amos-slam_amd/mask/net.py
@@ -537,13 +537,14 @@
         merged = getattr(self, "merged", None)
         return not (merged is None or not x0.is_cuda or x0.dtype != torch.float32 or torch.is_autocast_enabled() or os.environ.get("AMOS_MASK_FUSED_HEAD", "1") == "0")
 
-    def fused_outputs(self, pyramid, n_priors, br=None, out=None, scores=None, lazy=False):
+    def fused_outputs(self, pyramid, n_priors, br=None, out=None, scores=None, lazy=False, cand=None):
         x0 = pyramid[0]
         if not self.fused_applies(x0):
             return None
         merged = self.scores_boxes if lazy else self.merged
         ups = [None] * len(pyramid)
-        from .. import mask_head_outputs_scores
+        from .. import mask_head_candidates, mask_head_outputs_scores
+        from .post import SCORE_THRESHOLD
         b, dev = x0.shape[0], x0.device
         n_anchor = self.bbox_layer.out_channels // 4
         if out is None:
@@ -569,6 +570,11 @@
             if not raw.is_contiguous(memory_format=torch.channels_last):
                 raw = raw.contiguous(memory_format=torch.channels_last)
             cells = raw.shape[2] * raw.shape[3]
+            if cand is not None:
+                mask_head_candidates(torch.cuda.current_stream(dev).cuda_stream, raw.data_ptr(), merged.bias.data_ptr(), loc.data_ptr(),
+                                     coef.data_ptr() if coef is not None else None, cand.data_ptr(), SCORE_THRESHOLD, b, cells, raw.shape[1], n_anchor,
+                                     NUM_CLASSES, MASK_DIM, n_priors, offs[i])
+                return
             mask_head_outputs_scores(torch.cuda.current_stream(dev).cuda_stream, raw.data_ptr(), merged.bias.data_ptr(), loc.data_ptr(),
                                      conf.data_ptr() if conf is not None else None, coef.data_ptr() if coef is not None else None,
                                      scores.data_ptr() if scores is not None else None,
@@ -594,6 +600,12 @@
 
     def alloc_scores(self, b, n_priors, dev):
         return torch.empty((b, NUM_CLASSES - 1, n_priors), dtype=torch.float32, device=dev)
+
+    def alloc_candidates(self, b, n_priors, dev):
+        from .. import mask_candidates_bytes, mask_candidates_reset
+        cand = torch.empty(mask_candidates_bytes(b, n_priors, NUM_CLASSES), dtype=torch.uint8, device=dev)
+        mask_candidates_reset(torch.cuda.current_stream(dev).cuda_stream, cand.data_ptr(), b, NUM_CLASSES)
+        return cand
 
     def forward(self, x):
         b = x.shape[0]
@@ -637,8 +649,14 @@
     return os.environ.get("AMOS_MASK_LAZY_COEF", "1") != "0"
 
 
-def _outputs(loc, conf, cls, coef, priors, proto, head=None):
+def candidates_enabled():
+    return os.environ.get("AMOS_MASK_CANDIDATES", "1") != "0"
+
+
+def _outputs(loc, conf, cls, coef, priors, proto, head=None, cand=None):
     out = {"loc": loc, "priors": priors, "proto": proto}
+    if cand is not None:
+        out["candidates"] = (cand, NUM_CLASSES)
     if head is None:
         out["mask"] = coef
     else:
@@ -695,6 +713,9 @@
         feats = self.backbone(x)[1:]
         head = self.prediction_layers[0]
         lazy = bool(getattr(self, "lazy_coef", False)) and len(feats) == 3 and head.lazy_applies(feats[0])
+        want_cand = bool(getattr(self, "candidates", False)) and len(feats) == 3 and head.fused_applies(feats[0])
+        if want_cand:
+            scores_only = False
         pn = self.proto_net
 
         def prototypes(p3):
@@ -718,22 +739,24 @@
             for _ in range(2):
                 sizes.append(((sizes[-1][0] - 1) // 2 + 1, (sizes[-1][1] - 1) // 2 + 1))
             n_priors = sum(h * w for h, w in sizes) * (head.bbox_layer.out_channels // 4)
-            out = head.alloc_outputs(x.shape[0], n_priors, x.device, conf=not scores_only, coef=not lazy)
+            out = head.alloc_outputs(x.shape[0], n_priors, x.device, conf=not (scores_only or want_cand), coef=not lazy)
             cls = head.alloc_scores(x.shape[0], n_priors, x.device) if scores_only else None
+            cand = head.alloc_candidates(x.shape[0], n_priors, x.device) if want_cand else None
             pyramid = self.fpn(feats, br, chain)
             priors = priors_of(pyramid)
-            loc, conf, coef = head.fused_outputs(pyramid, priors.shape[0], br, out, cls, lazy)
+            loc, conf, coef = head.fused_outputs(pyramid, priors.shape[0], br, out, cls, lazy, cand)
             proto = prototypes(pyramid[0])
             br.join()
-            return _outputs(loc, conf, cls, coef, priors, proto, head if lazy else None)
+            return _outputs(loc, conf, cls, coef, priors, proto, head if lazy else None, cand)
         pyramid = self.fpn(feats, None, chain)
         proto = prototypes(pyramid[0])
         priors = priors_of(pyramid)
         if head.fused_applies(pyramid[0]):
-            out = head.alloc_outputs(x.shape[0], priors.shape[0], x.device, conf=not scores_only, coef=not lazy)
+            out = head.alloc_outputs(x.shape[0], priors.shape[0], x.device, conf=not (scores_only or want_cand), coef=not lazy)
             cls = head.alloc_scores(x.shape[0], priors.shape[0], x.device) if scores_only else None
-            loc, conf, coef = head.fused_outputs(pyramid, priors.shape[0], None, out, cls, lazy)
-            return _outputs(loc, conf, cls, coef, priors, proto, head if lazy else None)
+            cand = head.alloc_candidates(x.shape[0], priors.shape[0], x.device) if want_cand else None
+            loc, conf, coef = head.fused_outputs(pyramid, priors.shape[0], None, out, cls, lazy, cand)
+            return _outputs(loc, conf, cls, coef, priors, proto, head if lazy else None, cand)
         locs, confs, coefs = zip(*(head(p) for p in pyramid))
         return {"loc": torch.cat(locs, 1), "conf": F.softmax(torch.cat(confs, 1), -1), "mask": torch.cat(coefs, 1),
                 "priors": priors, "proto": proto}
diff --git a/amos-slam_amd/mask/post.py b/amos-slam_amd/mask/post.py
--- a/amos-slam_amd/mask/post.py
+++ b/amos-slam_amd/mask/post.py
@@ -84,8 +84,9 @@
         coef = layer.weight
     cls = pred.get("cls")
     conf = pred.get("conf")
-    scores = cls if cls is not None else conf
-    if scores is None or not (loc.is_cuda and all(t.dtype == torch.float32 for t in (loc, scores, coef, priors, proto))) or proto.dim() != 4:
+    cand, cand_c1 = pred.get("candidates", (None, None))
+    scores = cand if cand is not None else cls if cls is not None else conf
+    if scores is None or not (loc.is_cuda and all(t.dtype == torch.float32 for t in (loc, coef, priors, proto) + (() if cand is not None else (scores,)))) or proto.dim() != 4:
         return None
     import os
     if os.environ.get("AMOS_MASK_FUSED_POST", "1") == "0":
@@ -94,7 +95,7 @@
     loc, scores, priors, proto = (t.contiguous() for t in (loc, scores, priors, proto))
     B, P = loc.shape[:2]
     ph, pw, D = proto.shape[1:]
-    c1 = cls.shape[1] + 1 if cls is not None else conf.shape[2]
+    c1 = cand_c1 if cand is not None else cls.shape[1] + 1 if cls is not None else conf.shape[2]
     if P < 200 or (c1 - 1) * 200 * 4 > 64 * 1024 or D % 4 != 0:
         return None
     nbytes = mask_post_workspace_bytes(B, P, c1, D, ph, pw)
@@ -115,12 +116,13 @@
         data = [u.data if f else u for u, f in zip(ups, blocked)]
         if not all(d.is_contiguous() if f else d.is_contiguous(memory_format=torch.channels_last) for d, f in zip(data, blocked)):
             raise RuntimeError("person_masks_fused: an upfeature tensor is neither channels-last nor channel-blocked")
-        mask_person_masks_at_priors(stream, loc.data_ptr(), scores.data_ptr(), cls is not None, [d.data_ptr() for d in data], [tuple(u.shape[2:]) for u in ups], blocked,
+        mask_person_masks_at_priors(stream, loc.data_ptr(), scores.data_ptr(), "candidates" if cand is not None else cls is not None, [d.data_ptr() for d in data], [tuple(u.shape[2:]) for u in ups], blocked,
                                     layer.in_channels, anchors, weight.data_ptr(), layer.bias.data_ptr(), priors.data_ptr(), proto.data_ptr(), B, P, c1, D, ph, pw,
                                     h, w, ws.data_ptr(), nbytes, out.data_ptr(), found.data_ptr())
         return out, found.bool()
     coef = coef.contiguous()
-    (mask_person_masks_scores if cls is not None else mask_person_masks)(
+    from .. import mask_person_masks_candidates
+    (mask_person_masks_candidates if cand is not None else mask_person_masks_scores if cls is not None else mask_person_masks)(
         stream, loc.data_ptr(), scores.data_ptr(), coef.data_ptr(), priors.data_ptr(), proto.data_ptr(),
         B, P, c1, D, ph, pw, h, w, ws.data_ptr(), nbytes, out.data_ptr(), found.data_ptr())
     return out, found.bool()
diff --git a/include/amos_frontend.h b/include/amos_frontend.h
--- a/include/amos_frontend.h
+++ b/include/amos_frontend.h
@@ -493,6 +493,24 @@
                                                    const float *d_priors, const float *d_proto, int batch, int n_priors,
                                                    int n_classes_with_background, int mask_dim, int proto_h, int proto_w, int out_h, int out_w,
                                                    void *d_workspace, size_t workspace_bytes, uint8_t *d_masks, uint8_t *d_found);
+
+size_t amos_mask_candidates_bytes(int batch, int n_priors, int n_classes_with_background);
+int amos_mask_candidates_reset_device(void *stream, void *d_candidates, int batch, int n_classes_with_background);
+int amos_mask_head_candidates_device(void *stream, const float *d_raw, const float *d_bias, float *d_loc, float *d_coef, void *d_candidates, float threshold,
+                                     int batch, int cells, int channels_padded, int anchors, int n_classes_with_background, int mask_dim,
+                                     int n_priors_total, int prior_offset);
+int amos_mask_topk_lists_device(void *stream, const int *d_counts, const unsigned long long *d_entries, int capacity, float *d_values,
+                                long long *d_indices, int rows, int k);
+int amos_mask_person_masks_candidates_device(void *stream, const float *d_loc, const void *d_candidates, const float *d_coef, const float *d_priors,
+                                             const float *d_proto, int batch, int n_priors, int n_classes_with_background, int mask_dim, int proto_h,
+                                             int proto_w, int out_h, int out_w, void *d_workspace, size_t workspace_bytes, uint8_t *d_masks,
+                                             uint8_t *d_found);
+int amos_mask_person_masks_candidates_at_priors_device(void *stream, const float *d_loc, const void *d_candidates, const float *const *d_levels,
+                                                       const int *level_h, const int *level_w, const int *level_blocked, const int *level_offsets,
+                                                       int n_levels, int cin, int anchors, const float *d_mask_weight, const float *d_mask_bias,
+                                                       const float *d_priors, const float *d_proto, int batch, int n_priors,
+                                                       int n_classes_with_background, int mask_dim, int proto_h, int proto_w, int out_h, int out_w,
+                                                       void *d_workspace, size_t workspace_bytes, uint8_t *d_masks, uint8_t *d_found);
 
 
 
```

Measured after the change: 1655 frames/s (median of 6 runs). +1.7%, better.
